# AlgoLab/PIntron

Measured on AMD Instinct MI355X. Metric: ESTs aligned/sec (whole node) + DP Mcells/s; bit-exact factorizations vs ref, higher is better.
Workload: dtype u8/int32

## Files before the change

include/pintron_gpu.h:

```cpp
#ifndef PINTRON_GPU_H
#define PINTRON_GPU_H

#include <stddef.h>
#include <stdint.h>

#ifdef __cplusplus
extern "C" {
#endif

#define PGPU_OK       0
#define PGPU_EDEVICE (-5)
#define PGPU_ENOMEM  (-12)
#define PGPU_EINVAL  (-22)
#define PGPU_ENOSPC  (-28)
#define PGPU_ERANGE  (-34)
#define PGPU_ENOSYS  (-38)

typedef struct pgpu_ctx pgpu_ctx;
typedef struct pgpu_index pgpu_index;
typedef struct pgpu_dp_plan pgpu_dp_plan;

int pgpu_init(int device, pgpu_ctx** ctx);
int pgpu_destroy(pgpu_ctx* ctx);
const char* pgpu_last_error(const pgpu_ctx* ctx);
// ... 19 lines not shown

int pgpu_index_find(pgpu_ctx* ctx, const pgpu_index* idx,
                    const char* patterns, size_t patterns_len,
                    const pgpu_find_query* queries, size_t n_queries,
                    uint32_t* out, size_t out_cap, uint64_t* out_first, size_t* n_out);
double pgpu_index_find_kernel_ms(int k);

typedef struct { uint32_t start, end; } pgpu_intron;

int pgpu_index_classify(pgpu_ctx* ctx, const pgpu_index* idx, const pgpu_intron* introns, size_t n,
                        uint8_t* out_type);
int pgpu_index_score5(pgpu_ctx* ctx, const pgpu_index* idx, int k, double* out, size_t cap);

#define PGPU_SEXON_MAX_ELEN 64
typedef struct {
  uint64_t e_off;
  uint32_t elen;
  uint32_t allgstart, allglen;
  uint32_t f1slen, f2plen;
  uint32_t min_intron_len;
  uint32_t reserved;
} pgpu_sexon_query;
typedef struct {
  int32_t  status;
  uint32_t len;
  uint32_t offstart, offend;
  uint32_t gpos;
  uint32_t i1type, i2type;
  uint32_t pad;
} pgpu_sexon_result;

int pgpu_index_small_exons(pgpu_ctx* ctx, const pgpu_index* idx, const char* ests, size_t ests_len,
                           const pgpu_sexon_query* q, size_t n, pgpu_sexon_result* out);
double pgpu_index_small_exons_kernel_ms(void);

typedef struct { int32_t EST_start, EST_end, GEN_start, GEN_end; } pgpu_factor;

#define PGPU_REFINE_MAX_DIM 1024
#define PGPU_REFINE_MAX_ED   256
#define PGPU_REFINE_FIRST_INTRON 1u

typedef struct {
  uint64_t est_off;  uint32_t est_len;
  uint32_t flags;
  uint64_t rows_off; uint32_t dim;
  int32_t  factor_cut, intron_start, intron_end, intron_start_on_align, intron_end_on_align;
  pgpu_factor donor, acceptor;
  int32_t  suffpref_length_on_est, suffpref_length_for_intron, suffpref_length_on_gen, min_intron_length;
} pgpu_refine_query;

typedef struct {
  int32_t status;
  int32_t refined;
  int32_t path;
  int32_t pad;
  pgpu_factor donor, acceptor;
} pgpu_refine_result;

int pgpu_index_refine_introns(pgpu_ctx* ctx, const pgpu_index* idx, const char* ests, size_t ests_len,
                              const char* rows, size_t rows_len,
                              const pgpu_refine_query* q, size_t n, pgpu_refine_result* out);
double pgpu_index_refine_introns_kernel_ms(void);

#define PGPU_CHAIN_MAX_EST_WINDOW 192
#define PGPU_CHAIN_MAX_GEN_WINDOW 320
typedef struct {
  uint64_t est_off; uint32_t est_len;
  uint32_t first_exon, n_exons;
  uint32_t reserved;
  int32_t  suffpref_length_on_est, suffpref_length_for_intron, suffpref_length_on_gen, min_intron_length;
} pgpu_chain_query;

typedef struct {
  int32_t  status;
  uint32_t done;
  uint32_t dropped_first;
  uint32_t pad;
} pgpu_chain_result;

int pgpu_index_refine_chains(pgpu_ctx* ctx, const pgpu_index* idx, const char* ests, size_t ests_len,
                             const pgpu_factor* exons, size_t n_exons_total,
                             const pgpu_chain_query* q, size_t n,
                             pgpu_factor* out_exons, uint8_t* out_steps, pgpu_chain_result* out);
double pgpu_index_refine_chains_kernel_ms(void);

typedef struct {
  uint32_t min_factor_len;
  uint32_t reserved;
  double   min_string_depth_rate;
} pgpu_pairing_params;

typedef struct { int32_t p, t, l; } pgpu_pairing;

int pgpu_pairings(pgpu_ctx* ctx, const pgpu_index* idx,
                  const char* patterns, const uint64_t* pat_off, size_t n_pat,
                  const pgpu_pairing_params* params,
                  pgpu_pairing* out, size_t out_cap, uint64_t* out_first, size_t* n_out);

typedef struct pgpu_pairing_plan pgpu_pairing_plan;
int pgpu_pairing_plan_create(pgpu_ctx* ctx, const pgpu_index* idx, const char* patterns,
                             const uint64_t* pat_off, size_t n_pat, pgpu_pairing_plan** plan);
int pgpu_pairing_plan_create_resident(pgpu_ctx* ctx, const pgpu_index* idx, const char* patterns,
                                      const uint64_t* pat_off, size_t n_pat, pgpu_pairing_plan** plan);
int pgpu_pairing_plan_run(pgpu_ctx* ctx, pgpu_pairing_plan* plan, const pgpu_pairing_params* params);
uint64_t pgpu_pairing_plan_count(const pgpu_pairing_plan* plan);
uint64_t pgpu_pairing_plan_positions(const pgpu_pairing_plan* plan);
double pgpu_pairing_plan_kernel_ms(const pgpu_pairing_plan* plan, int k);
int pgpu_pairing_plan_fetch(pgpu_ctx* ctx, pgpu_pairing_plan* plan, pgpu_pairing* out, size_t out_cap,
                            uint64_t* out_first);
int pgpu_pairing_plan_destroy(pgpu_ctx* ctx, pgpu_pairing_plan* plan);

typedef struct {
  uint32_t min_factor_len;
  int32_t  min_intron_length, max_intron_length;
  uint32_t max_pairings_in_MEG;
  double   max_prefix_discarded_rate, max_suffix_discarded_rate, max_freq_shortest_pairing;
  uint32_t trans_red, short_edge_comp;
} pgpu_meg_params;

#define PGPU_MEG_MAX_VERTICES 64
#define PGPU_MEG_MAX_DEGREE   32
#define PGPU_MEG_TOO_COMPLEX  1u
#define PGPU_MEG_UNAVAILABLE  2u
int pgpu_pairing_plan_run_meg(pgpu_ctx* ctx, pgpu_pairing_plan* plan, const pgpu_meg_params* params);
uint64_t pgpu_pairing_plan_meg_bytes(const pgpu_pairing_plan* plan);
int pgpu_pairing_plan_fetch_meg(pgpu_ctx* ctx, pgpu_pairing_plan* plan, void* out, size_t out_cap,
                                uint64_t* rec_first);
double pgpu_pairing_plan_meg_ms(const pgpu_pairing_plan* plan);

int pgpu_host_alloc(pgpu_ctx* ctx, size_t bytes, void** out);
int pgpu_host_free(pgpu_ctx* ctx, void* p);

typedef struct pgpu_comm pgpu_comm;
typedef struct { char bytes[128]; } pgpu_comm_id;
int pgpu_comm_unique_id(pgpu_ctx* ctx, pgpu_comm_id* id);
int pgpu_comm_init(pgpu_ctx* ctx, int rank, int world, const pgpu_comm_id* id, pgpu_comm** comm);
int pgpu_gather(pgpu_ctx* ctx, pgpu_comm* comm, const void* send, uint64_t send_bytes,
                void* recv, uint64_t recv_cap, uint64_t* counts);
int pgpu_allgather(pgpu_ctx* ctx, pgpu_comm* comm, const void* send, uint64_t bytes, void* recv);
int pgpu_comm_destroy(pgpu_ctx* ctx, pgpu_comm* comm);

enum pgpu_dp_kind {
  PGPU_DP_ALIGN = 0,
  PGPU_DP_GAP = 1,
  PGPU_DP_ED = 2,
  PGPU_DP_KBAND = 3,
  PGPU_DP_LCF = 4,
  PGPU_DP_BORDERS = 5,
  PGPU_DP_AFFIX = 6,
  PGPU_DP_NKINDS = 7
};

#define PGPU_JOB_A_GENOMIC 1u
#define PGPU_JOB_B_GENOMIC 2u

typedef struct {
  uint32_t kind;
  uint32_t flags;
  uint64_t a_off, b_off;
  uint32_t a_len, b_len;
  uint32_t p0, p1, p2;
  uint32_t tail;
} pgpu_dp_job;

typedef struct {
  int32_t status;
  int32_t v[6];
  int32_t pad;
  uint64_t str[2];
} pgpu_dp_result;

#define PGPU_MAX_ROWS_LEV     65536u
#define PGPU_MAX_ROWS_BORDERS 4096u
#define PGPU_MAX_ROWS_GAP     2048u
#define PGPU_MAX_GAP_SIDE    16000u
#define PGPU_MAX_GAP_CELLS (1ull << 27)
#define PGPU_MAX_COLS      1048576u

int pgpu_dp_plan_create(pgpu_ctx* ctx, const pgpu_index* idx,
                        const pgpu_dp_job* jobs, size_t n_jobs,
                        const char* arena, size_t arena_len, pgpu_dp_plan** plan);
typedef struct { const pgpu_dp_job* jobs; size_t n_jobs; const char* arena; size_t arena_len; } pgpu_dp_part;
int pgpu_dp_plan_create_parts(pgpu_ctx* ctx, const pgpu_index* idx, const pgpu_dp_part* parts, size_t n_parts,
                              pgpu_dp_plan** plan);
int pgpu_dp_plan_launch(pgpu_ctx* ctx, pgpu_dp_plan* plan);
int pgpu_dp_plan_sync(pgpu_ctx* ctx, pgpu_dp_plan* plan);
size_t pgpu_dp_plan_string_bytes(const pgpu_dp_plan* plan);
int pgpu_dp_plan_fetch(pgpu_ctx* ctx, pgpu_dp_plan* plan, pgpu_dp_result* results,
                       char* strings, size_t strings_cap);
int pgpu_dp_plan_results_to_device(pgpu_ctx* ctx, pgpu_dp_plan* plan, void* device_dst, size_t cap);
int pgpu_dp_plan_destroy(pgpu_ctx* ctx, pgpu_dp_plan* plan);

uint64_t pgpu_dp_plan_cells(const pgpu_dp_plan* plan, int kind);
uint64_t pgpu_dp_plan_algo_bytes(const pgpu_dp_plan* plan, int kind);
double   pgpu_dp_plan_kernel_ms(const pgpu_dp_plan* plan, int kind);
uint64_t pgpu_dp_plan_launches(const pgpu_dp_plan* plan, int kind);

typedef struct {
  char     name[48];
  int32_t  kind;
  int32_t  pad;
  uint64_t jobs, cells, algo_bytes;
  double   ms;
  double   t0_ms;
} pgpu_group_info;
int pgpu_dp_plan_n_groups(const pgpu_dp_plan* plan);
int pgpu_dp_plan_group_info(const pgpu_dp_plan* plan, int i, pgpu_group_info* out);

int pgpu_dp_batch(pgpu_ctx* ctx, const pgpu_index* idx,
                  const pgpu_dp_job* jobs, size_t n_jobs, const char* arena, size_t arena_len,
                  pgpu_dp_result* results, char* strings, size_t strings_cap,
                  size_t* strings_used);

#ifdef __cplusplus
}
#endif
#endif
```

pintron_amd/capi.py:

```python
import ctypes as C
import os

_HERE = os.path.dirname(os.path.abspath(__file__))
LIB_PATH = os.path.join(_HERE, "lib", "libpintron_gpu.so")

PGPU_OK, PGPU_EDEVICE, PGPU_ENOMEM, PGPU_EINVAL, PGPU_ENOSPC, PGPU_ERANGE, PGPU_ENOSYS = \
    0, -5, -12, -22, -28, -34, -38
ALIGN, GAP, ED, KBAND, LCF, BORDERS, AFFIX = range(7)
KIND_NAMES = ["ALIGN", "GAP", "ED", "KBAND", "LCF", "BORDERS", "AFFIX"]
JOB_A_GENOMIC, JOB_B_GENOMIC = 1, 2


class DpJob(C.Structure):
    _fields_ = [("kind", C.c_uint32), ("flags", C.c_uint32), ("a_off", C.c_uint64),
                ("b_off", C.c_uint64), ("a_len", C.c_uint32), ("b_len", C.c_uint32),
                ("p0", C.c_uint32), ("p1", C.c_uint32), ("p2", C.c_uint32), ("tail", C.c_uint32)]


class DpResult(C.Structure):
    _fields_ = [("status", C.c_int32), ("v", C.c_int32 * 6), ("pad", C.c_int32),
                ("str", C.c_uint64 * 2)]


class GroupInfo(C.Structure):
# ... 12 lines not shown


class FindQuery(C.Structure):
    _fields_ = [("pat_off", C.c_uint64), ("pat_len", C.c_uint32), ("reserved", C.c_uint32),
                ("lo", C.c_uint32), ("hi", C.c_uint32)]


class Intron(C.Structure):
    _fields_ = [("start", C.c_uint32), ("end", C.c_uint32)]


class SexonQuery(C.Structure):
    _fields_ = [("e_off", C.c_uint64), ("elen", C.c_uint32), ("allgstart", C.c_uint32), ("allglen", C.c_uint32),
                ("f1slen", C.c_uint32), ("f2plen", C.c_uint32), ("min_intron_len", C.c_uint32), ("reserved", C.c_uint32)]


class SexonResult(C.Structure):
    _fields_ = [("status", C.c_int32), ("len", C.c_uint32), ("offstart", C.c_uint32), ("offend", C.c_uint32),
                ("gpos", C.c_uint32), ("i1type", C.c_uint32), ("i2type", C.c_uint32), ("pad", C.c_uint32)]


class Factor(C.Structure):
    _fields_ = [("EST_start", C.c_int32), ("EST_end", C.c_int32), ("GEN_start", C.c_int32), ("GEN_end", C.c_int32)]


class RefineQuery(C.Structure):
    _fields_ = [("est_off", C.c_uint64), ("est_len", C.c_uint32), ("flags", C.c_uint32), ("rows_off", C.c_uint64),
                ("dim", C.c_uint32), ("factor_cut", C.c_int32), ("intron_start", C.c_int32), ("intron_end", C.c_int32),
                ("intron_start_on_align", C.c_int32), ("intron_end_on_align", C.c_int32), ("donor", Factor), ("acceptor", Factor),
                ("suffpref_length_on_est", C.c_int32), ("suffpref_length_for_intron", C.c_int32),
                ("suffpref_length_on_gen", C.c_int32), ("min_intron_length", C.c_int32)]


class RefineResult(C.Structure):
    _fields_ = [("status", C.c_int32), ("refined", C.c_int32), ("path", C.c_int32), ("pad", C.c_int32),
                ("donor", Factor), ("acceptor", Factor)]


class ChainQuery(C.Structure):
    _fields_ = [("est_off", C.c_uint64), ("est_len", C.c_uint32), ("first_exon", C.c_uint32), ("n_exons", C.c_uint32),
                ("reserved", C.c_uint32), ("suffpref_length_on_est", C.c_int32), ("suffpref_length_for_intron", C.c_int32),
                ("suffpref_length_on_gen", C.c_int32), ("min_intron_length", C.c_int32)]


class ChainResult(C.Structure):
    _fields_ = [("status", C.c_int32), ("done", C.c_uint32), ("dropped_first", C.c_uint32), ("pad", C.c_uint32)]


REFINE_MAX_DIM, REFINE_MAX_ED, REFINE_FIRST_INTRON = 1024, 256, 1
CHAIN_MAX_EST_WINDOW, CHAIN_MAX_GEN_WINDOW = 192, 320
_FACTOR_DTYPE = [("EST_start", "<i4"), ("EST_end", "<i4"), ("GEN_start", "<i4"), ("GEN_end", "<i4")]
REFINE_QUERY_DTYPE = [("est_off", "<u8"), ("est_len", "<u4"), ("flags", "<u4"), ("rows_off", "<u8"), ("dim", "<u4"),
                      ("factor_cut", "<i4"), ("intron_start", "<i4"), ("intron_end", "<i4"), ("intron_start_on_align", "<i4"),
                      ("intron_end_on_align", "<i4"), ("donor", _FACTOR_DTYPE), ("acceptor", _FACTOR_DTYPE),
                      ("suffpref_length_on_est", "<i4"), ("suffpref_length_for_intron", "<i4"), ("suffpref_length_on_gen", "<i4"),
                      ("min_intron_length", "<i4")]
REFINE_RESULT_DTYPE = [("status", "<i4"), ("refined", "<i4"), ("path", "<i4"), ("pad", "<i4"), ("donor", _FACTOR_DTYPE),
                       ("acceptor", _FACTOR_DTYPE)]

CHAIN_QUERY_DTYPE = [("est_off", "<u8"), ("est_len", "<u4"), ("first_exon", "<u4"), ("n_exons", "<u4"), ("reserved", "<u4"),
                     ("suffpref_length_on_est", "<i4"), ("suffpref_length_for_intron", "<i4"), ("suffpref_length_on_gen", "<i4"),
                     ("min_intron_length", "<i4")]
CHAIN_RESULT_DTYPE = [("status", "<i4"), ("done", "<u4"), ("dropped_first", "<u4"), ("pad", "<u4")]
FACTOR_DTYPE = _FACTOR_DTYPE

SEXON_MAX_ELEN = 64
SEXON_QUERY_DTYPE = [("e_off", "<u8"), ("elen", "<u4"), ("allgstart", "<u4"), ("allglen", "<u4"), ("f1slen", "<u4"),
                     ("f2plen", "<u4"), ("min_intron_len", "<u4"), ("reserved", "<u4"), ("_pad", "<u4")]
SEXON_RESULT_DTYPE = [("status", "<i4"), ("len", "<u4"), ("offstart", "<u4"), ("offend", "<u4"), ("gpos", "<u4"),
                      ("i1type", "<u4"), ("i2type", "<u4"), ("pad", "<u4")]

assert C.sizeof(DpJob) == 48 and C.sizeof(DpResult) == 48 and C.sizeof(FindQuery) == 24
assert C.sizeof(Intron) == 8 and C.sizeof(SexonQuery) == 40 and C.sizeof(SexonResult) == 32
assert C.sizeof(Factor) == 16 and C.sizeof(RefineQuery) == 96 and C.sizeof(RefineResult) == 48
assert C.sizeof(ChainQuery) == 40 and C.sizeof(ChainResult) == 16

EXPORTS = [
    "pgpu_init", "pgpu_destroy", "pgpu_last_error", "pgpu_abi_version", "pgpu_set_timing", "pgpu_device_numa_node",
    "pgpu_index_build", "pgpu_index_destroy", "pgpu_index_suffix_array", "pgpu_index_save", "pgpu_index_load", "pgpu_pairings",
    "pgpu_index_find", "pgpu_index_find_kernel_ms",
    "pgpu_index_classify", "pgpu_index_score5", "pgpu_index_small_exons", "pgpu_index_small_exons_kernel_ms",
    "pgpu_index_refine_introns", "pgpu_index_refine_introns_kernel_ms",
    "pgpu_index_refine_chains", "pgpu_index_refine_chains_kernel_ms",
    "pgpu_pairing_plan_create", "pgpu_pairing_plan_create_resident", "pgpu_pairing_plan_run", "pgpu_pairing_plan_count",
    "pgpu_pairing_plan_positions", "pgpu_pairing_plan_kernel_ms", "pgpu_pairing_plan_fetch",
    "pgpu_pairing_plan_destroy",
    "pgpu_pairing_plan_run_meg", "pgpu_pairing_plan_meg_bytes", "pgpu_pairing_plan_fetch_meg",
    "pgpu_pairing_plan_meg_ms", "pgpu_host_alloc", "pgpu_host_free",
    "pgpu_comm_unique_id", "pgpu_comm_init", "pgpu_gather", "pgpu_allgather", "pgpu_comm_destroy",
    "pgpu_range_push", "pgpu_range_pop", "pgpu_build_info",
    "pgpu_dp_plan_create", "pgpu_dp_plan_create_parts", "pgpu_dp_plan_launch", "pgpu_dp_plan_sync",
    "pgpu_dp_plan_string_bytes", "pgpu_dp_plan_fetch", "pgpu_dp_plan_destroy",
    "pgpu_dp_plan_results_to_device",
    "pgpu_dp_plan_cells", "pgpu_dp_plan_algo_bytes", "pgpu_dp_plan_kernel_ms",
    "pgpu_dp_plan_launches", "pgpu_dp_plan_n_groups", "pgpu_dp_plan_group_info", "pgpu_dp_batch",
]

_lib = None


class PgpuError(RuntimeError):
    def __init__(self, code, msg):
        super().__init__("pgpu error %d: %s" % (code, msg))
        self.code = code


def lib():
    global _lib
    if _lib is None:
        if not os.path.exists(LIB_PATH):
            raise ImportError("%s is missing: run `python -c 'import __graft_entry__ as g; "
                              "g.build()'` (hipcc --offload-arch=gfx950)" % LIB_PATH)
        L = C.CDLL(LIB_PATH)
        vp, u64, sz = C.c_void_p, C.c_uint64, C.c_size_t
        L.pgpu_init.argtypes = [C.c_int, C.POINTER(vp)]
        L.pgpu_destroy.argtypes = [vp]
        L.pgpu_set_timing.argtypes = [vp, C.c_int]
        L.pgpu_last_error.argtypes = [vp]
        L.pgpu_last_error.restype = C.c_char_p
        L.pgpu_build_info.restype = C.c_char_p
        L.pgpu_range_push.argtypes = [C.c_char_p]
        L.pgpu_range_push.restype = None
        L.pgpu_range_pop.restype = None
        L.pgpu_allgather.argtypes = [vp, vp, vp, u64, vp]
        L.pgpu_index_build.argtypes = [vp, C.c_char_p, sz, C.POINTER(vp)]
        L.pgpu_index_destroy.argtypes = [vp, vp]
        L.pgpu_index_save.argtypes = [vp, vp, C.c_char_p, C.c_char_p]
        L.pgpu_index_load.argtypes = [vp, C.c_char_p, C.c_char_p, sz, C.POINTER(vp)]
        L.pgpu_index_suffix_array.argtypes = [vp, vp, C.POINTER(C.c_uint32), sz]
        L.pgpu_index_find.argtypes = [vp, vp, C.c_char_p, sz, C.POINTER(FindQuery), sz,
                                      C.POINTER(C.c_uint32), sz, C.POINTER(u64), C.POINTER(sz)]
        L.pgpu_index_find_kernel_ms.argtypes = [C.c_int]
        L.pgpu_index_find_kernel_ms.restype = C.c_double
        L.pgpu_index_classify.argtypes = [vp, vp, C.POINTER(Intron), sz, C.POINTER(C.c_uint8)]
        L.pgpu_index_score5.argtypes = [vp, vp, C.c_int, C.POINTER(C.c_double), sz]
        L.pgpu_index_small_exons.argtypes = [vp, vp, C.c_char_p, sz, C.POINTER(SexonQuery), sz, C.POINTER(SexonResult)]
        L.pgpu_index_small_exons_kernel_ms.argtypes = []
        L.pgpu_index_small_exons_kernel_ms.restype = C.c_double
        L.pgpu_index_refine_introns.argtypes = [vp, vp, C.c_char_p, sz, C.c_char_p, sz, C.POINTER(RefineQuery), sz,
                                                C.POINTER(RefineResult)]
        L.pgpu_index_refine_introns_kernel_ms.argtypes = []
        L.pgpu_index_refine_introns_kernel_ms.restype = C.c_double
        L.pgpu_index_refine_chains.argtypes = [vp, vp, C.c_char_p, sz, C.POINTER(Factor), sz, C.POINTER(ChainQuery), sz,
                                               C.POINTER(Factor), C.POINTER(C.c_uint8), C.POINTER(ChainResult)]
        L.pgpu_index_refine_chains_kernel_ms.argtypes = []
        L.pgpu_index_refine_chains_kernel_ms.restype = C.c_double
        L.pgpu_pairing_plan_run_meg.argtypes = [vp, vp, vp]
        L.pgpu_pairing_plan_meg_bytes.argtypes = [vp]
        L.pgpu_pairing_plan_meg_bytes.restype = u64
        L.pgpu_pairing_plan_meg_ms.argtypes = [vp]
        L.pgpu_pairing_plan_meg_ms.restype = C.c_double
        L.pgpu_pairing_plan_fetch_meg.argtypes = [vp, vp, vp, sz, C.POINTER(u64)]
        L.pgpu_host_alloc.argtypes = [vp, sz, C.POINTER(vp)]
        L.pgpu_host_free.argtypes = [vp, vp]
        L.pgpu_comm_unique_id.argtypes = [vp, vp]
        L.pgpu_comm_init.argtypes = [vp, C.c_int, C.c_int, vp, C.POINTER(vp)]
        L.pgpu_gather.argtypes = [vp, vp, C.c_char_p, u64, vp, u64, C.POINTER(u64)]
        L.pgpu_comm_destroy.argtypes = [vp, vp]
        L.pgpu_pairings.argtypes = [vp, vp, C.c_char_p, C.POINTER(u64), sz,
                                    C.POINTER(PairingParams), C.POINTER(Pairing), sz,
                                    C.POINTER(u64), C.POINTER(sz)]
        L.pgpu_pairing_plan_create.argtypes = [vp, vp, C.c_char_p, C.POINTER(u64), sz, C.POINTER(vp)]
        L.pgpu_pairing_plan_create_resident.argtypes = [vp, vp, C.c_char_p, C.POINTER(u64), sz, C.POINTER(vp)]
        L.pgpu_pairing_plan_run.argtypes = [vp, vp, C.POINTER(PairingParams)]
        L.pgpu_pairing_plan_count.argtypes = [vp]
        L.pgpu_pairing_plan_count.restype = u64
        L.pgpu_pairing_plan_positions.argtypes = [vp]
        L.pgpu_pairing_plan_positions.restype = u64
        L.pgpu_pairing_plan_kernel_ms.argtypes = [vp, C.c_int]
        L.pgpu_pairing_plan_kernel_ms.restype = C.c_double
        L.pgpu_pairing_plan_fetch.argtypes = [vp, vp, C.POINTER(Pairing), sz, C.POINTER(u64)]
        L.pgpu_pairing_plan_destroy.argtypes = [vp, vp]
        L.pgpu_dp_plan_create_parts.argtypes = [vp, vp, vp, sz, C.POINTER(vp)]
        L.pgpu_dp_plan_create.argtypes = [vp, vp, C.POINTER(DpJob), sz, C.c_char_p, sz,
                                          C.POINTER(vp)]
        L.pgpu_dp_plan_launch.argtypes = [vp, vp]
        L.pgpu_dp_plan_sync.argtypes = [vp, vp]
        L.pgpu_dp_plan_string_bytes.argtypes = [vp]
        L.pgpu_dp_plan_string_bytes.restype = sz
        L.pgpu_dp_plan_fetch.argtypes = [vp, vp, C.POINTER(DpResult), C.c_char_p, sz]
        L.pgpu_dp_plan_destroy.argtypes = [vp, vp]
        L.pgpu_dp_plan_results_to_device.argtypes = [vp, vp, vp, sz]
        for nm in ("pgpu_dp_plan_cells", "pgpu_dp_plan_algo_bytes", "pgpu_dp_plan_launches"):
            getattr(L, nm).argtypes = [vp, C.c_int]
            getattr(L, nm).restype = u64
        L.pgpu_dp_plan_kernel_ms.argtypes = [vp, C.c_int]
        L.pgpu_dp_plan_kernel_ms.restype = C.c_double
        L.pgpu_dp_plan_n_groups.argtypes = [vp]
        L.pgpu_dp_plan_group_info.argtypes = [vp, C.c_int, C.POINTER(GroupInfo)]
        L.pgpu_dp_batch.argtypes = [vp, vp, C.POINTER(DpJob), sz, C.c_char_p, sz,
                                    C.POINTER(DpResult), C.c_char_p, sz, C.POINTER(sz)]
        _lib = L
    return _lib


class Context:

    def __init__(self, device=0):
        self.L = lib()
        self.h = C.c_void_p()
        rc = self.L.pgpu_init(device, C.byref(self.h))
        if rc != PGPU_OK:
            raise PgpuError(rc, "pgpu_init(%d) failed (no usable gfx950 device?)" % device)
        self.L.pgpu_set_timing(self.h, 1)

    def check(self, rc):
        if rc != PGPU_OK:
            raise PgpuError(rc, self.L.pgpu_last_error(self.h).decode())

    def close(self):
        if self.h:
            self.L.pgpu_destroy(self.h)
            self.h = C.c_void_p()

    def __enter__(self):
        return self

    def __exit__(self, *a):
        self.close()


class Index:
    def __init__(self, ctx: Context, genomic: bytes, load_from=None):
        self.ctx = ctx
        self.h = C.c_void_p()
        self.n = len(genomic)
        self.genomic = genomic
# ... 46 lines not shown
        if rc == PGPU_ENOSPC:
            out = np.empty(total, dtype=np.uint32)
            rc, first, total = self.find_raw(blob, qs, n, out)
        else:
            out = np.empty(0, dtype=np.uint32)
        self.ctx.check(rc)
        return [out[int(first[i]):int(first[i + 1])] for i in range(n)]

    def find_kernel_ms(self):
        return {"count+scan": self.ctx.L.pgpu_index_find_kernel_ms(0), "fill": self.ctx.L.pgpu_index_find_kernel_ms(1)}

    def classify(self, starts, ends, ctx=None):
        import numpy as np
        ctx = ctx or self.ctx
        iv = np.empty((len(starts), 2), dtype=np.uint32)
        iv[:, 0], iv[:, 1] = starts, ends
        out = np.empty(len(iv), dtype=np.uint8)
        ctx.check(ctx.L.pgpu_index_classify(ctx.h, self.h, iv.ctypes.data_as(C.POINTER(Intron)), len(iv),
                                            out.ctypes.data_as(C.POINTER(C.c_uint8))))
        return out

    def score5(self, k):
        import numpy as np
        out = np.empty(self.n + 1, dtype=np.float64)
        self.ctx.check(self.ctx.L.pgpu_index_score5(self.ctx.h, self.h, k, out.ctypes.data_as(C.POINTER(C.c_double)), len(out)))
        return out

    def small_exons_raw(self, ests: bytes, queries, n: int):
        import numpy as np
        res = np.zeros(n, dtype=np.dtype(SEXON_RESULT_DTYPE))
        qp = queries.ctypes.data_as(C.POINTER(SexonQuery)) if hasattr(queries, "ctypes") else queries
        rc = self.ctx.L.pgpu_index_small_exons(self.ctx.h, self.h, ests, len(ests), qp, n,
                                               res.ctypes.data_as(C.POINTER(SexonResult)))
        return rc, res

    def small_exons(self, ests: bytes, queries):
        import numpy as np
        if not isinstance(queries, np.ndarray):
            rows = list(queries)
            q = np.zeros(len(rows), dtype=np.dtype(SEXON_QUERY_DTYPE))
            for i, r in enumerate(rows):
                q[i] = tuple(r) + (0, 0)
            queries = q
        rc, res = self.small_exons_raw(ests, queries, len(queries))
        self.ctx.check(rc)
        return res

    def small_exons_kernel_ms(self):
        return self.ctx.L.pgpu_index_small_exons_kernel_ms()

    def refine_introns_raw(self, ests: bytes, rows: bytes, queries, n: int):
        import numpy as np
        res = np.zeros(n, dtype=np.dtype(REFINE_RESULT_DTYPE))
        qp = queries.ctypes.data_as(C.POINTER(RefineQuery)) if hasattr(queries, "ctypes") else queries
        rc = self.ctx.L.pgpu_index_refine_introns(self.ctx.h, self.h, ests, len(ests), rows, len(rows), qp, n,
                                                  res.ctypes.data_as(C.POINTER(RefineResult)))
        return rc, res

    def refine_introns(self, ests: bytes, rows: bytes, queries):
        rc, res = self.refine_introns_raw(ests, rows, queries, len(queries))
        self.ctx.check(rc)
        return res

    def refine_introns_kernel_ms(self):
        return self.ctx.L.pgpu_index_refine_introns_kernel_ms()

    def refine_chains_raw(self, ests: bytes, exons, queries, n: int):
        import numpy as np
        out_exons = np.zeros(len(exons), dtype=np.dtype(FACTOR_DTYPE))
        out_steps = np.zeros(len(exons), dtype=np.uint8)
        res = np.zeros(n, dtype=np.dtype(CHAIN_RESULT_DTYPE))
        rc = self.ctx.L.pgpu_index_refine_chains(self.ctx.h, self.h, ests, len(ests), exons.ctypes.data_as(C.POINTER(Factor)),
                                                 len(exons), queries.ctypes.data_as(C.POINTER(ChainQuery)), n,
                                                 out_exons.ctypes.data_as(C.POINTER(Factor)),
                                                 out_steps.ctypes.data_as(C.POINTER(C.c_uint8)),
                                                 res.ctypes.data_as(C.POINTER(ChainResult)))
        return rc, out_exons, out_steps, res

    def refine_chains(self, ests: bytes, exons, queries):
        rc, out_exons, out_steps, res = self.refine_chains_raw(ests, exons, queries, len(queries))
        self.ctx.check(rc)
        return out_exons, out_steps, res

    def refine_chains_kernel_ms(self):
        return self.ctx.L.pgpu_index_refine_chains_kernel_ms()

    def close(self):
        if self.h:
            self.ctx.L.pgpu_index_destroy(self.ctx.h, self.h)
            self.h = C.c_void_p()


class MegParams(C.Structure):
    _fields_ = [("min_factor_len", C.c_uint32), ("min_intron_length", C.c_int32), ("max_intron_length", C.c_int32),
                ("max_pairings_in_MEG", C.c_uint32), ("max_prefix_discarded_rate", C.c_double),
                ("max_suffix_discarded_rate", C.c_double), ("max_freq_shortest_pairing", C.c_double),
                ("trans_red", C.c_uint32), ("short_edge_comp", C.c_uint32)]


def parse_meg_record(rec: bytes):
    import struct
    nv, ne, flags, _ = struct.unpack_from("<4I", rec, 0)
    if flags & 2:
        return dict(flags=flags, vertices=[], adj=[], meg_text=b"", edges_text=b"")
    verts = [struct.unpack_from("<3i", rec, 16 + 12 * k) for k in range(nv)]
    first = struct.unpack_from("<%dH" % (nv + 1), rec, 16 + 12 * nv)
    base = 16 + 12 * nv + 2 * (nv + 1)
    adj = [list(rec[base + first[k]:base + first[k + 1]]) for k in range(nv)]
    graph = (base + ne + 3) & ~3
    ml, el = struct.unpack_from("<2I", rec, graph)
    return dict(flags=flags, vertices=verts, adj=adj, meg_text=rec[graph + 8:graph + 8 + ml],
                edges_text=rec[graph + 8 + ml:graph + 8 + ml + el])


class PairingPlan:
    STAGES = ["locate", "chain", "count+scan", "fill", "cross+scan", "emit"]

    def __init__(self, ctx: Context, index: Index, patterns, resident=False):
        import numpy as np
        self.ctx, self.n_pat = ctx, len(patterns)
        self._blob = b"".join(patterns)
        self._off = np.zeros(len(patterns) + 1, dtype=np.uint64)
        np.cumsum([len(p) for p in patterns], out=self._off[1:])
        self.h = C.c_void_p()
        create = ctx.L.pgpu_pairing_plan_create_resident if resident else ctx.L.pgpu_pairing_plan_create
        ctx.check(create(ctx.h, index.h, self._blob, self._off.ctypes.data_as(C.POINTER(C.c_uint64)),
                         self.n_pat, C.byref(self.h)))

    def run(self, min_factor_len=15, rate=0.2):
        prm = PairingParams(min_factor_len, 0, rate)
        self.ctx.check(self.ctx.L.pgpu_pairing_plan_run(self.ctx.h, self.h, C.byref(prm)))
        return self.ctx.L.pgpu_pairing_plan_count(self.h)

    def stage_ms(self):
        return {s: self.ctx.L.pgpu_pairing_plan_kernel_ms(self.h, k) for k, s in enumerate(self.STAGES)}

    def fetch(self):
        import numpy as np
        n = self.ctx.L.pgpu_pairing_plan_count(self.h)
        out = np.zeros((max(n, 1), 3), dtype=np.int32)
        first = np.zeros(self.n_pat + 1, dtype=np.uint64)
        self.ctx.check(self.ctx.L.pgpu_pairing_plan_fetch(
            self.ctx.h, self.h, out.ctypes.data_as(C.POINTER(Pairing)), n,
            first.ctypes.data_as(C.POINTER(C.c_uint64))))
        return out[:n], first

    def run_meg(self, min_factor_len=15, min_intron_length=40, max_intron_length=0, max_pairings_in_MEG=80,
                max_prefix_discarded_rate=0.6, max_suffix_discarded_rate=0.6, max_freq_shortest_pairing=0.4,
                trans_red=True, short_edge_comp=True):
        prm = MegParams(min_factor_len, min_intron_length, max_intron_length, max_pairings_in_MEG,
                        max_prefix_discarded_rate, max_suffix_discarded_rate, max_freq_shortest_pairing,
                        int(trans_red), int(short_edge_comp))
        self.ctx.check(self.ctx.L.pgpu_pairing_plan_run_meg(self.ctx.h, self.h, C.byref(prm)))
        return self.ctx.L.pgpu_pairing_plan_meg_bytes(self.h)

    def fetch_meg(self):
        import numpy as np
        n = self.ctx.L.pgpu_pairing_plan_meg_bytes(self.h)
        out = np.zeros(max(n, 1), dtype=np.uint8)
        first = np.zeros(self.n_pat + 1, dtype=np.uint64)
        self.ctx.check(self.ctx.L.pgpu_pairing_plan_fetch_meg(
            self.ctx.h, self.h, out.ctypes.data_as(C.c_void_p), n, first.ctypes.data_as(C.POINTER(C.c_uint64))))
        raw = out.tobytes()
        return [raw[int(first[i]):int(first[i + 1])] for i in range(self.n_pat)]

    def close(self):
# ... 139 lines not shown
```

pintron_amd/csrc/pgpu_api.hip:

```cpp
#include <algorithm>
#include <cstdarg>
#include <cstdio>
#include <cstdlib>
#include <cstring>
#include <ctime>
#include <time.h>
#include <new>
#include <mutex>
#include <vector>

#include "pgpu_internal.h"
#include "pgpu_index.h"

struct BufPool {
  static constexpr int SLOTS = 24;
  void* ptr[SLOTS] = {nullptr};
  size_t cap[SLOTS] = {0};
  bool busy = false;
  int sharers = 0;
  const void* owner = nullptr;
};

struct pgpu_ctx {
  int device = 0;
  hipStream_t stream = nullptr;
  char err[512] = {0};
  BufPool pools[2];
  bool timing = false;
  static constexpr int NAUX = 4;
  hipStream_t aux[NAUX] = {nullptr};
  hipEvent_t ev_upload = nullptr;
  hipEvent_t ev_aux[NAUX] = {nullptr};
  hipEvent_t ev_done = nullptr;
  hipEvent_t ev_wait = nullptr;
  long wait_poll_us = 20;
  int poison = -1;
  void* pin[2] = {nullptr, nullptr};
  size_t pin_cap[2] = {0, 0};
  std::vector<hipEvent_t> ev_pool;
};

static int wait_stream(pgpu_ctx* ctx, hipStream_t st) {
  if (hipEventRecord(ctx->ev_done, st) != hipSuccess) return -1;
  if (ctx->wait_poll_us != 0) {
    for (;;) {
      const hipError_t q = hipEventQuery(ctx->ev_done);
      if (q == hipSuccess) return 0;
      if (q != hipErrorNotReady) return -1;
      if (ctx->wait_poll_us > 0) { struct timespec ts = {0, ctx->wait_poll_us * 1000L}; nanosleep(&ts, nullptr); }
    }
  }
  return hipEventSynchronize(ctx->ev_done) == hipSuccess ? 0 : -1;
}

static void* pinned(pgpu_ctx* ctx, int slot, size_t bytes) {
  if (ctx->pin_cap[slot] < bytes) {
    if (ctx->pin[slot]) (void)hipHostFree(ctx->pin[slot]);
    ctx->pin[slot] = nullptr; ctx->pin_cap[slot] = 0;
    const size_t want = std::max<size_t>(bytes + bytes / 2 + 4096, (size_t)2 << 20);
    if (hipHostMalloc(&ctx->pin[slot], want, hipHostMallocDefault) != hipSuccess) return nullptr;
    pgpu_trace_alloc(slot ? "ctx pinned down" : "ctx pinned up", ctx->pin[slot], want);
    ctx->pin_cap[slot] = want;
  }
  return ctx->pin[slot];
}

bool pgpu_ctx_pool_acquire(pgpu_ctx* ctx, int pool) {
  if (ctx->pools[pool].busy) return false;
  ctx->pools[pool].busy = true;
  return true;
}
void pgpu_ctx_pool_release(pgpu_ctx* ctx, int pool) { ctx->pools[pool].busy = false; ctx->pools[pool].owner = nullptr; }
bool pgpu_ctx_pool_share(pgpu_ctx* ctx, int pool) {
  BufPool& p = ctx->pools[pool];
  if (p.busy && p.sharers == 0) return false;
  p.busy = true; ++p.sharers;
  return true;
}
void pgpu_ctx_pool_unshare(pgpu_ctx* ctx, int pool, const void* who) {
  BufPool& p = ctx->pools[pool];
  if (p.owner == who) p.owner = nullptr;
  if (p.sharers > 0 && --p.sharers == 0) p.busy = false;
}
void pgpu_ctx_pool_set_owner(pgpu_ctx* ctx, int pool, const void* who) { ctx->pools[pool].owner = who; }
const void* pgpu_ctx_pool_owner(const pgpu_ctx* ctx, int pool) { return ctx->pools[pool].owner; }
void* pgpu_ctx_pool_get(pgpu_ctx* ctx, int pool, int slot, size_t bytes) {
  BufPool& p = ctx->pools[pool];
  if (bytes == 0) bytes = 16;
  if (p.cap[slot] < bytes) {
    if (p.ptr[slot]) (void)hipFree(p.ptr[slot]);
    p.ptr[slot] = nullptr; p.cap[slot] = 0;
    const size_t want = std::max<size_t>(bytes + bytes / 2 + 4096, pool == 0 ? (size_t)64 << 20 : 0);
    if (hipMalloc(&p.ptr[slot], want) != hipSuccess) {
      if (hipMalloc(&p.ptr[slot], bytes) != hipSuccess) return nullptr;
      p.cap[slot] = bytes;
    } else p.cap[slot] = want;
    pgpu_trace_alloc(pool ? "device pool 1" : "device pool 0", p.ptr[slot], p.cap[slot]);
  }
  return p.ptr[slot];
}
bool pgpu_ctx_timing(const pgpu_ctx* ctx) { return ctx->timing; }

extern "C" int pgpu_device_numa_node(pgpu_ctx* ctx) {
  if (!ctx) return -1;
  char bdf[64] = {0};
  if (hipDeviceGetPCIBusId(bdf, (int)sizeof bdf - 1, ctx->device) != hipSuccess) return -1;
  for (char* c = bdf; *c; ++c) if (*c >= 'A' && *c <= 'F') *c = (char)(*c - 'A' + 'a');
  char path[160];
  snprintf(path, sizeof path, "/sys/bus/pci/devices/%s/numa_node", bdf);
  FILE* f = fopen(path, "r");
  if (!f) return -1;
  int node = -1;
  if (fscanf(f, "%d", &node) != 1) node = -1;
  fclose(f);
  return node;
}

extern "C" int pgpu_set_timing(pgpu_ctx* ctx, int enabled) {
  if (!ctx) return PGPU_EINVAL;
  ctx->timing = enabled != 0;
  return PGPU_OK;
}

static int set_err(pgpu_ctx* ctx, int code, const char* fmt, ...) {
  if (ctx) {
    va_list ap;
    va_start(ap, fmt);
    vsnprintf(ctx->err, sizeof(ctx->err), fmt, ap);
    va_end(ap);
  }
  return code;
}

#define HIP_TRY(ctx, call)                                                                  \
  do {                                                                                      \
    hipError_t e_ = (call);                                                                 \
    if (e_ != hipSuccess)                                                                   \
      return set_err(ctx, e_ == hipErrorOutOfMemory ? PGPU_ENOMEM : PGPU_EDEVICE,           \
                     "%s failed: %s (%s:%d)", #call, hipGetErrorString(e_), __FILE__, __LINE__); \
  } while (0)

hipStream_t pgpu_ctx_stream(pgpu_ctx* ctx) { return ctx->stream; }
hipError_t pgpu_ctx_wait(pgpu_ctx* ctx) {
  if (ctx->wait_poll_us <= 0) return hipStreamSynchronize(ctx->stream);
  hipError_t e = hipEventRecord(ctx->ev_wait, ctx->stream);
  if (e != hipSuccess) return e;
  const struct timespec ts = {0, ctx->wait_poll_us * 5000L};
  for (;;) {
    e = hipEventQuery(ctx->ev_wait);
    if (e != hipErrorNotReady) return e;
    nanosleep(&ts, nullptr);
  }
}
int pgpu_ctx_bind(pgpu_ctx* ctx) {
  const hipError_t e = hipSetDevice(ctx->device);
  return e == hipSuccess ? PGPU_OK : set_err(ctx, PGPU_EDEVICE, "hipSetDevice(%d) failed: %s", ctx->device, hipGetErrorString(e));
}
int pgpu_ctx_fail(pgpu_ctx* ctx, int code, const char* msg) { return set_err(ctx, code, "%s", msg); }

extern "C" int pgpu_abi_version(void) { return 1; }

#include <dlfcn.h>
namespace {
struct Roctx { int state = 0; int (*push)(const char*) = nullptr; int (*pop)() = nullptr; };
Roctx g_roctx;
bool roctx_ready() {
  if (g_roctx.state) return g_roctx.state > 0;
  bool want = false;
  { const char* m = getenv("PGPU_MARKERS"); if (m) want = m[0] != '0'; else {
      const char* t = getenv("ROCP_TOOL_LIBRARIES"); const char* pl = getenv("LD_PRELOAD");
      want = (t && t[0]) || (pl && strstr(pl, "rocprofiler")); } }
  if (want) {
    void* so = nullptr;
    for (const char* n : { "librocprofiler-sdk-roctx.so.1", "librocprofiler-sdk-roctx.so", "libroctx64.so.4", "libroctx64.so" })
      if ((so = dlopen(n, RTLD_NOW | RTLD_GLOBAL)) != nullptr) break;
    if (so) {
      *(void**)(&g_roctx.push) = dlsym(so, "roctxRangePushA");
      *(void**)(&g_roctx.pop) = dlsym(so, "roctxRangePop");
    }
  }
  g_roctx.state = (g_roctx.push && g_roctx.pop) ? 1 : -1;
  return g_roctx.state > 0;
}
}
extern "C" void pgpu_range_push(const char* name) { if (roctx_ready()) g_roctx.push(name ? name : ""); }
extern "C" void pgpu_range_pop(void) { if (roctx_ready()) g_roctx.pop(); }

extern "C" const char* pgpu_build_info(void) {
  static char info[256];
  if (!info[0]) {
    const char* stamp = __DATE__ " " __TIME__ " " __VERSION__;
    unsigned long long h = 1469598103934665603ull;
    for (const char* c = stamp; *c; ++c) { h ^= (unsigned char)*c; h *= 1099511628211ull; }
    snprintf(info, sizeof info, "libpintron_gpu abi %d, gfx950, built %s %s, hip %d.%d.%d, stamp %016llx", pgpu_abi_version(), __DATE__,
             __TIME__, HIP_VERSION_MAJOR, HIP_VERSION_MINOR, HIP_VERSION_PATCH, h);
  }
  return info;
}

static bool aux_stream(pgpu_ctx* ctx, int i) {
  if (!ctx->aux[i] && hipStreamCreateWithFlags(&ctx->aux[i], hipStreamNonBlocking) != hipSuccess) { ctx->aux[i] = nullptr; return false; }
  if (!ctx->ev_aux[i] && hipEventCreateWithFlags(&ctx->ev_aux[i], hipEventDisableTiming) != hipSuccess) { ctx->ev_aux[i] = nullptr; return false; }
  return true;
}

static hipEvent_t g_base_event[64];
static std::mutex g_base_mu;
static hipEvent_t base_event(int device, hipStream_t st) {
  if (device < 0 || device >= 64) return nullptr;
  std::lock_guard<std::mutex> lk(g_base_mu);
  if (!g_base_event[device]) {
    hipEvent_t e = nullptr;
    if (hipEventCreate(&e) == hipSuccess && hipEventRecord(e, st) == hipSuccess && hipEventSynchronize(e) == hipSuccess) g_base_event[device] = e;
    else if (e) hipEventDestroy(e);
  }
  return g_base_event[device];
}

extern "C" int pgpu_init(int device, pgpu_ctx** out) {
  if (!out) return PGPU_EINVAL;
  *out = nullptr;
  int n = 0;
  if (hipGetDeviceCount(&n) != hipSuccess || n <= 0) return PGPU_EDEVICE;
  if (device < 0 || device >= n) return PGPU_EINVAL;
  hipDeviceProp_t prop;
  if (hipGetDeviceProperties(&prop, device) != hipSuccess) return PGPU_EDEVICE;
  if (strncmp(prop.gcnArchName, "gfx950", 6) != 0) return PGPU_EDEVICE;
  if (hipSetDevice(device) != hipSuccess) return PGPU_EDEVICE;
  pgpu_ctx* ctx = new (std::nothrow) pgpu_ctx();
  if (!ctx) return PGPU_ENOMEM;
  ctx->device = device;
  if (hipStreamCreateWithFlags(&ctx->stream, hipStreamNonBlocking) != hipSuccess) {
    delete ctx;
    return PGPU_EDEVICE;
  }
  if (hipEventCreateWithFlags(&ctx->ev_upload, hipEventDisableTiming) != hipSuccess) { delete ctx; return PGPU_EDEVICE; }
  if (hipEventCreateWithFlags(&ctx->ev_done, hipEventDisableTiming | hipEventBlockingSync) != hipSuccess) { delete ctx; return PGPU_EDEVICE; }
  if (hipEventCreateWithFlags(&ctx->ev_wait, hipEventDisableTiming) != hipSuccess) { delete ctx; return PGPU_EDEVICE; }
  { const char* f = getenv("PGPU_WAIT"); if (f) ctx->wait_poll_us = atol(f); }
  { const char* f = getenv("PGPU_POISON"); if (f && f[0]) ctx->poison = atoi(f) & 255; }
  base_event(device, ctx->stream);
  *out = ctx;
  return PGPU_OK;
}

extern "C" int pgpu_destroy(pgpu_ctx* ctx) {
  if (!ctx) return PGPU_EINVAL;
  hipSetDevice(ctx->device);
  hipStreamSynchronize(ctx->stream);
  for (auto& pl : ctx->pools) for (auto& q : pl.ptr) if (q) hipFree(q);
  for (auto& a : ctx->aux) if (a) { hipStreamSynchronize(a); hipStreamDestroy(a); }
  if (ctx->ev_upload) hipEventDestroy(ctx->ev_upload);
  if (ctx->ev_done) hipEventDestroy(ctx->ev_done);
  if (ctx->ev_wait) hipEventDestroy(ctx->ev_wait);
  for (auto& e : ctx->ev_aux) if (e) hipEventDestroy(e);
  for (auto& e : ctx->ev_pool) if (e) hipEventDestroy(e);
  for (auto& q : ctx->pin) if (q) hipHostFree(q);
  hipStreamDestroy(ctx->stream);
  delete ctx;
  return PGPU_OK;
}

extern "C" const char* pgpu_last_error(const pgpu_ctx* ctx) { return ctx ? ctx->err : "null context"; }

namespace {

uint32_t row_class(uint32_t rows) {
  if (rows > 4096u) return ROW_CLASS_STRIPS;
  uint32_t R = 1;
  while (64u * R < rows) R <<= 1;
  return R;
}

enum DpRoute : uint8_t {
  RT_ALIGN_STRIPS, RT_ALIGN_COOP, RT_ALIGN_WAVE, RT_GAP_SLOW, RT_GAP, RT_ED, RT_KBAND, RT_LCF,
  RT_BORDERS_SLOW, RT_BORDERS_COOP, RT_BORDERS_WAVE, RT_AFFIX_STRIPS, RT_AFFIX_COOP, RT_AFFIX_WAVE,
  RT_LCFSA, RT_LCFW, RT_ALIGNB,
  RT_BATCH,
  RT_COUNT
};

enum BatchPlace { OUTSIDE, SEGMENT, ROLE_BORDERS, ROLE_AFFIX, ROLE_ALIGN };

using WsBytes = size_t (*)(uint32_t la, uint32_t lb, uint32_t R);
size_t ws_align_wave(uint32_t, uint32_t lb, uint32_t) { return ((size_t)lb + 64) * 64; }
size_t ws_align_coop(uint32_t, uint32_t lb, uint32_t R) { return ((size_t)lb + 256) * 256 * align_coop_entry_bytes(R); }
size_t ws_align_strips(uint32_t la, uint32_t lb, uint32_t R) {
  return 2 * strip_bnd_bytes(lb) + (size_t)((la + 4095u) / 4096u) * ((size_t)lb + 64) * 64 * align_entry_bytes(R);
}
size_t ws_gap(uint32_t, uint32_t lb, uint32_t R) { return ((size_t)lb + 64) * 64 * gap_entry_bytes(R); }
size_t ws_gap_slow(uint32_t la, uint32_t lb, uint32_t) { return (size_t)9 * ((size_t)la + 1) * 4 + ((size_t)la + 1) * ((size_t)lb + 1); }
size_t ws_borders_slow(uint32_t la, uint32_t, uint32_t) { return (size_t)7 * ((size_t)la + 1) * 4; }
size_t ws_affix_strips(uint32_t, uint32_t lb, uint32_t) { return 2 * strip_bnd_bytes(lb); }
size_t ws_ed_strips(uint32_t la, uint32_t lb, uint32_t R) { return R == ROW_CLASS_STRIPS ? 2 * strip_bnd_bytes(std::max(la, lb)) : 0; }

using AlgoBytes = uint64_t (*)(uint64_t la, uint64_t lb, uint64_t p2);
uint64_t bytes_operands(uint64_t la, uint64_t lb, uint64_t) { return la + lb; }
uint64_t bytes_align(uint64_t la, uint64_t lb, uint64_t) { return la + lb + la * lb + 3 * (la + lb); }
uint64_t bytes_gap(uint64_t la, uint64_t lb, uint64_t) { return la + lb + 3 * la * lb + 3 * (la + lb); }
uint64_t bytes_borders(uint64_t la, uint64_t lb, uint64_t p2) { return la + std::min(lb, 2 * std::min(la + p2, lb)) + 2 * 8 * la; }
uint64_t bytes_lcfsa(uint64_t, uint64_t lb, uint64_t) { return lb + 64u * 96u; }

struct RouteInfo {
  const char* name;
  int kind;
  int family;
  WsBytes ws_bytes;
  bool strings;
  uint32_t cell_factor;
  AlgoBytes algo_bytes;
  BatchPlace place;
  int seg_pos;
  uint32_t big_from;
  long weight; bool by_rows; int lane; DpLauncher launch;
  bool keyed;
};

constexpr RouteInfo ROUTES[] = {
  {"lev_wave<ALIGN,strips>",  PGPU_DP_ALIGN,   KF_ALIGN,   ws_align_strips, true,  1, bytes_align,    OUTSIDE,      0,  0,  5000, false,  2, launch_align_big,    false},
  {"align_coop",              PGPU_DP_ALIGN,   KF_ALIGN,   ws_align_coop,   true,  1, bytes_align,    ROLE_ALIGN,   0,  0,     0, false,  0, nullptr,             false},
  {"lev_wave<ALIGN>",         PGPU_DP_ALIGN,   KF_ALIGN,   ws_align_wave,   true,  1, bytes_align,    SEGMENT,      1,  0,     0, false,  0, nullptr,             false},
  {"gap_slow",                PGPU_DP_GAP,     KF_GAP,     ws_gap_slow,     true,  3, bytes_gap,      OUTSIDE,      0,  0,  4000, false,  3, launch_gap_slow,     false},
  {"gap_wave",                PGPU_DP_GAP,     KF_GAP,     ws_gap,          true,  3, bytes_gap,      SEGMENT,      2,  8,  4000, false,  3, launch_gap_big,      false},
  {"lev_wave<ED>",            PGPU_DP_ED,      KF_ED,      ws_ed_strips,    false, 1, bytes_operands, SEGMENT,      8, 32,  1000, false,  1, launch_ed_big,       false},
  {"lev_wave<KBAND>",         PGPU_DP_KBAND,   KF_KBAND,   ws_ed_strips,    false, 1, bytes_operands, SEGMENT,      3, 32,  2000, false,  2, launch_kband_big,    false},
  {"lcf",                     PGPU_DP_LCF,     KF_LCF,     nullptr,         false, 1, bytes_operands, OUTSIDE,      0,  0,  3000, false,  3, launch_lcf,          true},
  {"borders_slow",            PGPU_DP_BORDERS, KF_BORDERS, ws_borders_slow, false, 2, bytes_borders,  OUTSIDE,      0,  0, 10000, true,   1, launch_borders_slow, false},
  {"borders_coop",            PGPU_DP_BORDERS, KF_BORDERS, nullptr,         false, 2, bytes_borders,  ROLE_BORDERS, 0,  0, 10000, true,   1, launch_borders_coop, false},
  {"lev_wave<BORDERS,R=1>",   PGPU_DP_BORDERS, KF_BORDERS, nullptr,         false, 2, bytes_borders,  SEGMENT,      4,  0,     0, false,  0, nullptr,             false},
  {"lev_wave<AFFIX,strips>",  PGPU_DP_AFFIX,   KF_AFFIX,   ws_affix_strips, false, 1, bytes_operands, OUTSIDE,      0,  0, 10000, true,   0, launch_affix_strips, false},
  {"affix_coop",              PGPU_DP_AFFIX,   KF_AFFIX,   nullptr,         false, 1, bytes_operands, ROLE_AFFIX,   0,  0,     0, false,  0, nullptr,             false},
  {"lev_wave<AFFIX,R=1>",     PGPU_DP_AFFIX,   KF_AFFIX,   nullptr,         false, 1, bytes_operands, SEGMENT,      5,  0,     0, false,  0, nullptr,             false},
// ... 539 lines not shown
```

pintron_amd/csrc/pgpu_chain.hip:

```cpp
#include <stdlib.h>
#include <string.h>

#include "pgpu_internal.h"
#include "pgpu_query_call.h"
#include "pgpu_wave_dp.h"
#include "pgpu_refine_body.h"

namespace {

constexpr int MAX_EW = PGPU_CHAIN_MAX_EST_WINDOW;
constexpr int MAX_GW = PGPU_CHAIN_MAX_GEN_WINDOW;
constexpr uint32_t CHAIN_R = 4;
static_assert(MAX_EW <= 64 * (int)CHAIN_R && MAX_EW + MAX_GW <= MAX_DIM, "the caps fit the sweep and the decision");

constexpr size_t WS_DIRS = ((size_t)MAX_GW + 64) * 64 * CHAIN_R;
constexpr size_t WS_STRS = WS_DIRS;
constexpr size_t WS_STRS_BYTES = (2 * ((size_t)MAX_EW + MAX_GW + 1) + 15) & ~(size_t)15;
constexpr size_t WS_WIN_E = WS_STRS + WS_STRS_BYTES;
constexpr size_t WS_WIN_G = WS_WIN_E + ((MAX_EW + 15) & ~15);
constexpr size_t WS_RES = WS_WIN_G + ((MAX_GW + 15) & ~15);
constexpr size_t WS_WAVE = (WS_RES + sizeof(DevResult) + 255) & ~(size_t)255;

struct ChainLds {
  union {
    struct { __attribute__((aligned(16))) uint8_t win[TB_WIN_BYTES]; uint8_t path[TB_PATH]; } tb;
    RefineLds refine;
  };
};

__device__ __forceinline__ int append_piece(uint8_t* dst, int at, int cap, const Seq& s, int index, int length, int lane) {
  if (at > cap) return at;
  if (index < 0) { length += index; index = 0; }
  if (length > cap - at + 1) length = cap - at + 1;
  const Piece p = substring(s, index, length, lane);
  if (p.len > cap - at) return cap + 1;
  for (int k = lane; k < p.len; k += 64) dst[at + k] = s.p[p.start + k];
  return at + p.len;
}

__global__ __launch_bounds__(64)
void chain_kernel(const uint8_t* __restrict__ T, uint32_t n, const uint8_t* __restrict__ ests, const pgpu_factor* __restrict__ exons,
                  const pgpu_chain_query* __restrict__ queries, uint32_t n_chains, uint8_t* __restrict__ ws,
                  pgpu_factor* __restrict__ out_exons, uint8_t* __restrict__ out_steps, pgpu_chain_result* __restrict__ out) {
  __shared__ ChainLds S;
  const int lane = (int)threadIdx.x;
  uint8_t* const w = ws + (size_t)blockIdx.x * WS_WAVE;
  uint8_t* const win_e = w + WS_WIN_E;
  uint8_t* const win_g = w + WS_WIN_G;
  DevResult* const res = reinterpret_cast<DevResult*>(w + WS_RES);
  for (uint32_t c = blockIdx.x; c < n_chains; c += gridDim.x) {
    const pgpu_chain_query q = queries[c];
    Seq est, gen;
    est.p = ests + q.est_off; est.len = (int)q.est_len;
    gen.p = T; gen.len = (int)n;
    const int sp_est = q.suffpref_length_on_est, sp_int = q.suffpref_length_for_intron, sp_gen = q.suffpref_length_on_gen;
    pgpu_chain_result cr;
    cr.status = PGPU_OK; cr.done = 0; cr.dropped_first = 0; cr.pad = 0;
    pgpu_factor donor = exons[q.first_exon];
    const int first_est_start = donor.EST_start;
    int second_est_start = 0;
    uint32_t i = 0;
    for (; i + 1 < q.n_exons; ++i) {
      const pgpu_factor acceptor = exons[q.first_exon + i + 1];
      int dsl_gen = donor.GEN_start;
      if (donor.GEN_end - sp_gen + 1 >= dsl_gen) dsl_gen = donor.GEN_end - sp_gen + 1;
      int dsl_est = donor.EST_start;
      if (donor.EST_end - sp_est + 1 >= dsl_est) dsl_est = donor.EST_end - sp_est + 1;
      int apr_gen = acceptor.GEN_end;
      if (acceptor.GEN_start + sp_gen - 1 <= apr_gen) apr_gen = acceptor.GEN_start + sp_gen - 1;
      int apr_est = acceptor.EST_end;
      if (acceptor.EST_start + sp_est - 1 <= apr_est) apr_est = acceptor.EST_start + sp_est - 1;
      int le = 0, lg = 0;
      le = append_piece(win_e, le, MAX_EW, est, dsl_est, donor.EST_end - dsl_est + 1, lane);
      if (donor.EST_end != acceptor.EST_start - 1)
        le = append_piece(win_e, le, MAX_EW, est, donor.EST_end + 1, acceptor.EST_start - donor.EST_end - 1, lane);
      le = append_piece(win_e, le, MAX_EW, est, acceptor.EST_start, apr_est - acceptor.EST_start + 1, lane);
      lg = append_piece(win_g, lg, MAX_GW, gen, dsl_gen, donor.GEN_end - dsl_gen + 1, lane);
      lg = append_piece(win_g, lg, MAX_GW, gen, donor.GEN_end + 1, sp_int, lane);
      lg = append_piece(win_g, lg, MAX_GW, gen, acceptor.GEN_start - sp_int, sp_int, lane);
      lg = append_piece(win_g, lg, MAX_GW, gen, acceptor.GEN_start, apr_gen - acceptor.GEN_start + 1, lane);
      if (le > MAX_EW || lg > MAX_GW) { cr.status = PGPU_ERANGE; break; }
      DevJob job;
      job.a = win_e; job.b = win_g; job.la = (uint32_t)le; job.lb = (uint32_t)lg;
      job.p0 = job.p1 = job.p2 = job.tail = 0;
      job.ws_off = 0; job.str_off = WS_STRS; job.out_idx = 0;
      job.r_class = le <= 64 ? 1u : (le <= 128 ? 2u : 4u);
      own_stores_visible();
      switch (job.r_class) {
        case 1:  gap_wave_body<1>(job, res, w, (uint32_t)lane); break;
        case 2:  gap_wave_body<2>(job, res, w, (uint32_t)lane); break;
        default: gap_wave_body<4>(job, res, w, (uint32_t)lane); break;
      }
      own_stores_visible();
      gap_traceback_wave(job, res, w, w, (uint32_t)lane, S.tb.win, S.tb.path);
      own_stores_visible();
      pgpu_refine_query rq;
      rq.est_off = q.est_off; rq.est_len = q.est_len; rq.flags = i == 0 ? PGPU_REFINE_FIRST_INTRON : 0u;
      rq.rows_off = 0; rq.dim = (uint32_t)__builtin_amdgcn_readfirstlane(res->v[0]);
      rq.factor_cut = __builtin_amdgcn_readfirstlane(res->v[1]);
      rq.intron_start = __builtin_amdgcn_readfirstlane(res->v[2]);
      rq.intron_end = __builtin_amdgcn_readfirstlane(res->v[3]);
      rq.intron_start_on_align = __builtin_amdgcn_readfirstlane(res->v[4]);
      rq.intron_end_on_align = __builtin_amdgcn_readfirstlane(res->v[5]);
      rq.donor = donor; rq.acceptor = acceptor;
      rq.suffpref_length_on_est = sp_est; rq.suffpref_length_for_intron = sp_int; rq.suffpref_length_on_gen = sp_gen;
      rq.min_intron_length = q.min_intron_length;
      const int dim = (int)rq.dim;
      const uint8_t* const row_e = w + (uint32_t)__builtin_amdgcn_readfirstlane((int)res->str[0]);
      const uint8_t* const row_g = w + (uint32_t)__builtin_amdgcn_readfirstlane((int)res->str[1]);
      __syncthreads();
      for (int k = lane; k < dim; k += 64) { S.refine.rows[k] = row_e[k]; S.refine.rows[dim + k] = row_g[k]; }
      __syncthreads();
      pgpu_refine_result r;
      r.status = PGPU_OK; r.refined = 0; r.path = 0; r.pad = 0; r.donor = donor; r.acceptor = acceptor;
      refine_decide(S.refine, S.refine.rows, S.refine.rows + dim, dim, rq, T, n, ests, lane, r);
      __syncthreads();
      if (r.status != PGPU_OK) { cr.status = PGPU_ERANGE; break; }
      if (lane == 0) {
        out_exons[q.first_exon + i] = r.donor;
        out_steps[q.first_exon + i + 1] = (uint8_t)((uint32_t)r.path | ((uint32_t)r.refined << 7));
      }
      if (i == 0) second_est_start = r.acceptor.EST_start;
      donor = r.acceptor;
    }
    cr.done = i;
    if (lane == 0) out_exons[q.first_exon + i] = donor;
    if (cr.status == PGPU_OK && q.n_exons > 1 && first_est_start == second_est_start) cr.dropped_first = 1;
    if (lane == 0) out[c] = cr;
  }
}

thread_local double t_chain_ms = 0.0;

constexpr unsigned WAVES_PER_CU = 16;

}

extern "C" double pgpu_index_refine_chains_kernel_ms(void) { return t_chain_ms; }

extern "C" int pgpu_index_refine_chains(pgpu_ctx* ctx, const pgpu_index* idx, const char* ests, size_t ests_len,
                                        const pgpu_factor* exons, size_t n_exons_total,
                                        const pgpu_chain_query* q, size_t n,
                                        pgpu_factor* out_exons, uint8_t* out_steps, pgpu_chain_result* out) {
  t_chain_ms = 0.0;
  static_assert(sizeof(pgpu_chain_query) == 40 && sizeof(pgpu_chain_result) == 16 && sizeof(pgpu_factor) == 16, "ABI layout");
  if (!ctx || !idx || (n && (!q || !out)) || (ests_len && !ests) || (n_exons_total && (!exons || !out_exons || !out_steps)))
    return PGPU_EINVAL;
  if (n > 0x7fffffffull || n_exons_total > 0x7fffffffull)
    return pgpu_ctx_fail(ctx, PGPU_EINVAL, "more than 2^31 - 1 chains or exons in one call");
  const size_t glen = pgpu_index_length(idx);
  struct Freed { uint8_t* p; ~Freed() { free(p); } } named_block{ (uint8_t*)calloc(n_exons_total ? n_exons_total : 1, 1) };
  uint8_t* const named = named_block.p;
  if (!named) return pgpu_ctx_fail(ctx, PGPU_ENOMEM, "no memory for the table of the exons the chains name");
  for (size_t i = 0; i < n; ++i) {
    const pgpu_chain_query& x = q[i];
    bool ok = x.est_off <= ests_len && x.est_len <= ests_len - x.est_off && x.est_len <= 0x7fffffffu && x.reserved == 0 &&
              x.n_exons != 0 && x.first_exon <= n_exons_total && x.n_exons <= n_exons_total - x.first_exon &&
              suffpref_ok(x.suffpref_length_on_est, x.suffpref_length_for_intron, x.suffpref_length_on_gen);
    for (uint32_t k = 0; ok && k < x.n_exons; ++k) {
      const pgpu_factor& f = exons[x.first_exon + k];
      ok = !named[x.first_exon + k] && factor_ok(f, x.est_len, glen);
      named[x.first_exon + k] = 1;
      if (ok && k + 1 < x.n_exons) {
        const pgpu_factor& g = exons[x.first_exon + k + 1];
        ok = f.EST_end < g.EST_start && f.GEN_end < g.GEN_start;
      }
    }
    if (!ok)
      return pgpu_ctx_fail(ctx, PGPU_EINVAL, "bad chain query (a range past its buffer, reserved != 0, no exon, an exon two chains "
                                             "share, a donor that is not in front of its acceptor, or a coordinate outside what it "
                                             "indexes)");
  }
  if (n == 0) {
    if (n_exons_total) { memcpy(out_exons, exons, n_exons_total * sizeof(pgpu_factor)); memset(out_steps, 0, n_exons_total); }
    return PGPU_OK;
  }
  if (pgpu_ctx_bind(ctx) != PGPU_OK) return PGPU_EDEVICE;
  QueryCall call(ctx, "refine chains");
  const hipStream_t st = call.st;
  int dev = 0, cus = 0;
  TRY_HIP(hipGetDevice(&dev));
  TRY_HIP(hipDeviceGetAttribute(&cus, hipDeviceAttributeMultiprocessorCount, dev));
  const size_t waves = n < (size_t)cus * WAVES_PER_CU ? n : (size_t)cus * WAVES_PER_CU;
  const size_t ex_bytes = n_exons_total * sizeof(pgpu_factor);
  const size_t o_ex = up256(ests_len + 64), o_q = o_ex + up256(ex_bytes), o_oex = o_q + up256(n * sizeof(pgpu_chain_query)),
               o_st = o_oex + up256(ex_bytes), o_r = o_st + up256(n_exons_total), o_ws = o_r + up256(n * sizeof(pgpu_chain_result)),
               total = o_ws + waves * WS_WAVE;
  TRY_HIP(hipMalloc((void**)&call.d, total));
  TRY_HIP(call.timing_events(1));
  if (ests_len) TRY_HIP(hipMemcpyAsync(call.d, ests, ests_len, hipMemcpyHostToDevice, st));
  TRY_HIP(hipMemcpyAsync(call.d + o_ex, exons, ex_bytes, hipMemcpyHostToDevice, st));
  TRY_HIP(hipMemcpyAsync(call.d + o_q, q, n * sizeof(pgpu_chain_query), hipMemcpyHostToDevice, st));
  TRY_HIP(hipMemcpyAsync(call.d + o_oex, call.d + o_ex, ex_bytes, hipMemcpyDeviceToDevice, st));
  TRY_HIP(hipMemsetAsync(call.d + o_st, 0, n_exons_total, st));
  TRY_HIP(call.record(0));
  hipLaunchKernelGGL(chain_kernel, dim3((unsigned)waves), dim3(64), 0, st, pgpu_index_genomic(idx), (uint32_t)glen, call.d,
                     (const pgpu_factor*)(call.d + o_ex), (const pgpu_chain_query*)(call.d + o_q), (uint32_t)n, call.d + o_ws,
                     (pgpu_factor*)(call.d + o_oex), call.d + o_st, (pgpu_chain_result*)(call.d + o_r));
  TRY_HIP(call.record(1));
  TRY_HIP(hipMemcpyAsync(out_exons, call.d + o_oex, ex_bytes, hipMemcpyDeviceToHost, st));
  TRY_HIP(hipMemcpyAsync(out_steps, call.d + o_st, n_exons_total, hipMemcpyDeviceToHost, st));
  TRY_HIP(hipMemcpyAsync(out, call.d + o_r, n * sizeof(pgpu_chain_result), hipMemcpyDeviceToHost, st));
  TRY_HIP(pgpu_ctx_wait(ctx));
  TRY_HIP(hipGetLastError());
  call.elapsed_ms(0, &t_chain_ms);
  return PGPU_OK;
}
```

pintron_amd/csrc/pgpu_index.h:

```cpp
#pragma once
#include <stddef.h>
#include <stdint.h>
#include <mutex>
#include <hip/hip_runtime.h>
#include "../../include/pintron_gpu.h"

const uint8_t* pgpu_index_genomic(const pgpu_index* idx);
size_t pgpu_index_length(const pgpu_index* idx);

constexpr uint32_t KTAB = 8;
constexpr uint32_t KTAB_ENTRIES = 1u << (2 * KTAB);

struct LcfIndexView {
  const uint8_t* T; const uint32_t* sa; const uint32_t* klo; const uint32_t* khi; const uint32_t* focc; const uint32_t* rmq;
  uint32_t n, levels, first_bad;
};
LcfIndexView pgpu_index_lcf_view(const pgpu_index* idx);
constexpr uint32_t LCF_FOCC_ENTRIES = 87380;

struct pgpu_index_lazy { std::mutex mu; void* tables = nullptr; void (*release)(void*) = nullptr; };
pgpu_index_lazy* pgpu_index_lazy_slot(const pgpu_index* idx);

hipStream_t pgpu_ctx_stream(pgpu_ctx* ctx);
int pgpu_ctx_bind(pgpu_ctx* ctx);
hipError_t pgpu_ctx_wait(pgpu_ctx* ctx);
int pgpu_ctx_fail(pgpu_ctx* ctx, int code, const char* msg);
bool pgpu_ctx_pool_acquire(pgpu_ctx* ctx, int pool);
void pgpu_ctx_pool_release(pgpu_ctx* ctx, int pool);
void* pgpu_ctx_pool_get(pgpu_ctx* ctx, int pool, int slot, size_t bytes);
bool pgpu_ctx_pool_share(pgpu_ctx* ctx, int pool);
void pgpu_ctx_pool_unshare(pgpu_ctx* ctx, int pool, const void* who);
void pgpu_ctx_pool_set_owner(pgpu_ctx* ctx, int pool, const void* who);
const void* pgpu_ctx_pool_owner(const pgpu_ctx* ctx, int pool);
bool pgpu_ctx_timing(const pgpu_ctx* ctx);

size_t pgpu_scan_tmp_bytes(size_t n);
void pgpu_exclusive_scan_u32(const uint32_t* in, unsigned long long* out, size_t n, void* tmp, hipStream_t st);
size_t pgpu_meg_scratch_bytes(size_t n_pat);
void pgpu_meg_launch_build(const pgpu_pairing* pairs, const unsigned long long* pair_first, const unsigned long long* pat_off,
                           uint32_t n_pat, const pgpu_meg_params* prm, void* scratch, void* info, uint32_t* rec_bytes,
                           hipStream_t st);
void pgpu_meg_launch_emit(uint32_t n_pat, const void* scratch, const void* info, const unsigned long long* rec_off,
                          uint8_t* out, hipStream_t st);
#include <cstdio>
#include <cstdlib>
static inline void pgpu_trace_alloc(const char* what, const void* q, size_t bytes) {
  static int on = -1;
  if (on < 0) { const char* e = getenv("PGPU_TRACE_ALLOC"); on = (e && *e && *e != '0') ? 1 : 0; }
  if (on) fprintf(stderr, "* alloc %-18s %10.1f MB at %p\n", what, bytes / 1048576.0, q);
}
```

pintron_amd/host/ef_config.c:

```c
#include <stdlib.h>
#include <string.h>
#include <unistd.h>

#include "estfact.h"

void ef_config_defaults(ef_config* c) {
  memset(c, 0, sizeof(*c));
  c->min_factor_len = 15; c->min_intron_length = 40; c->max_intron_length = 0;
  c->min_string_depth_rate = 0.2;
  c->max_prefix_discarded_rate = 0.60; c->max_suffix_discarded_rate = 0.60;
  c->max_prefix_discarded = 50; c->max_suffix_discarded = 50;
  c->max_site_difference = 50; c->max_number_of_factorizations = 0;
  c->max_coverage_diff = 0.05; c->max_exonNUM_diff = 5; c->max_gapLength_diff = 20;
  c->retain_externals = 1;
  c->max_pairings_in_MEG = 80; c->max_freq_shortest_pairing = 0.4;
  c->suffpref_length_for_intron = 70; c->suffpref_length_on_est = 30; c->suffpref_length_on_gen = 30;
  c->trans_red = true; c->short_edge_comp = true;
  c->max_single_factorization_time = 900;
  c->complexity_threshold = 20.0;
  strcpy(c->config_file, "config.ini");
}

typedef enum { T_INT, T_DBL, T_STR, T_FLAG, T_BOOLSTR } otype;
typedef struct { const char* name; char shortopt; otype type; size_t off; } optdef;
// ... 29 lines not shown
    case 7: if (iv < 0) return -1; c->max_prefix_discarded = (int)iv; return 0;
    case 8: if (iv < 0) return -1; c->max_suffix_discarded = (int)iv; return 0;
    case 9: if (iv < 0) return -1; c->max_site_difference = (unsigned)iv; return 0;
    case 10: if (iv < 0) return -1; c->max_number_of_factorizations = (int)iv; return 0;
    case 11: if (dv < 0.0 || dv > 1.0) return -1; c->max_coverage_diff = dv; return 0;
    case 12: if (iv < -1) return -1; c->max_exonNUM_diff = (int)iv; return 0;
    case 13: if (iv < -1) return -1; c->max_gapLength_diff = (int)iv; return 0;
    case 14: if (dv <= 0.0) return -1; c->complexity_threshold = dv; return 0;
    case 15:
      if (v && !strcmp(v, "true")) c->retain_externals = 1;
      else if (v && !strcmp(v, "false")) c->retain_externals = 0;
      else return -1;
      return 0;
    case 16: if (iv < 0) return -1; c->max_pairings_in_MEG = (unsigned)iv; return 0;
    case 17: if (dv < 0.0 || dv > 1.0) return -1; c->max_freq_shortest_pairing = dv; return 0;
    case 18: if (iv <= 0) return -1; c->suffpref_length_for_intron = (int)iv; return 0;
    case 19: if (iv <= 0) return -1; c->suffpref_length_on_est = (int)iv; return 0;
    case 20: if (iv <= 0) return -1; c->suffpref_length_on_gen = (int)iv; return 0;
    case 21: c->trans_red = false; return 0;
    case 22: c->short_edge_comp = false; return 0;
    case 23: if (iv < 0) return -1; c->max_single_factorization_time = (unsigned)iv; return 0;
  }
  return -1;
}

static bool is_flag(int k) { return k == 21 || k == 22; }

static int find_long(const char* name, size_t len) {
  for (int k = 0; NAMES[k]; ++k)
    if (strlen(NAMES[k]) == len && !strncmp(NAMES[k], name, len)) return k;
  return -1;
}

static int parse_file(ef_config* c, const char* path, const bool* given) {
  FILE* f = fopen(path, "r");
  if (!f) return 0;
  char line[4096];
  while (fgets(line, sizeof line, f)) {
    char* p = line;
    while (*p == ' ' || *p == '\t') ++p;
    if (*p == '#' || *p == '\n' || *p == '\0') continue;
    char* e = p;
    while (*e && *e != '=' && *e != ' ' && *e != '\t' && *e != '\n') ++e;
    const int k = find_long(p, (size_t)(e - p));
    if (k < 0) { fprintf(stderr, "est-fact: unknown option '%.*s' in %s\n", (int)(e - p), p, path); fclose(f); return -1; }
    while (*e == ' ' || *e == '\t' || *e == '=') ++e;
    char* v = e;
    size_t vl = strlen(v);
    while (vl && (v[vl - 1] == '\n' || v[vl - 1] == '\r' || v[vl - 1] == ' ' || v[vl - 1] == '\t')) v[--vl] = '\0';
    if (vl >= 2 && v[0] == '"' && v[vl - 1] == '"') { v[vl - 1] = '\0'; ++v; }
    if (given[k]) continue;
    if (apply(c, k, is_flag(k) ? NULL : v) != 0) { fprintf(stderr, "est-fact: invalid value for '%s' in %s\n", NAMES[k], path); fclose(f); return -1; }
  }
  fclose(f);
  return 0;
}

static void dump(const ef_config* c) {
  FILE* f = fopen("./config-dump.ini", "w");
  if (!f) return;
  fprintf(f, "# This file was written by est-fact (MI355X build)\n");
  fprintf(f, "config-file=\"%s\"\n", c->config_file);
  fprintf(f, "min-factor-length=\"%u\"\nmin-intron-length=\"%d\"\nmax-intron-length=\"%d\"\n",
          c->min_factor_len, c->min_intron_length, c->max_intron_length);
  fprintf(f, "min-string-depth-rate=\"%g\"\nmax-prefix-discarded-rate=\"%g\"\nmax-suffix-discarded-rate=\"%g\"\n",
          c->min_string_depth_rate, c->max_prefix_discarded_rate, c->max_suffix_discarded_rate);
  fprintf(f, "max-prefix-discarded=\"%d\"\nmax-suffix-discarded=\"%d\"\nmin-distance-of-splice-sites=\"%u\"\n",
          c->max_prefix_discarded, c->max_suffix_discarded, c->max_site_difference);
  fprintf(f, "max-no-of-factorizations=\"%d\"\nmax-difference-of-coverage=\"%g\"\nmax-difference-of-no-of-exons=\"%d\"\n",
          c->max_number_of_factorizations, c->max_coverage_diff, c->max_exonNUM_diff);
  fprintf(f, "max-difference-of-gap-length=\"%d\"\ncomplexity-threshold=\"%g\"\nretain-externals=\"%s\"\n",
          c->max_gapLength_diff, c->complexity_threshold, c->retain_externals ? "true" : "false");
  fprintf(f, "max-pairings-in-CMEG=\"%u\"\nmax-shortest-pairing-frequence=\"%g\"\n",
          c->max_pairings_in_MEG, c->max_freq_shortest_pairing);
  fprintf(f, "suff-pref-length-intron=\"%d\"\nsuff-pref-length-est=\"%d\"\nsuff-pref-length-genomic=\"%d\"\n",
          c->suffpref_length_for_intron, c->suffpref_length_on_est, c->suffpref_length_on_gen);
  if (!c->trans_red) fprintf(f, "no-transitive-reduction\n");
  if (!c->short_edge_comp) fprintf(f, "no-short-edge-compaction\n");
  fprintf(f, "max-single-factorization-time=\"%u\"\n", c->max_single_factorization_time);
  fclose(f);
}

int ef_ahead_on = 1;
int ef_chain_fast_path = 1;
int ef_endpoint_checks = 1;
int ef_prof_on;
_Thread_local ef_prof_state ef_prof;
unsigned long long ef_work_budget_override;

int ef_config_load(ef_config* c, int argc, char** argv) {
  ef_config_defaults(c);
  { const char* e = getenv("PINTRON_ENDPOINT_CHECKS"); ef_endpoint_checks = !(e && e[0] == '0'); }
  { const char* e = getenv("PINTRON_CHAIN"); ef_chain_fast_path = !(e && e[0] == '0' && e[1] == '\0'); }
  { const char* e = getenv("PINTRON_AHEAD"); ef_ahead_on = !(e && e[0] == '0' && e[1] == '\0'); }
  { const char* e = getenv("PINTRON_PROFILE"); ef_prof_on = e && e[0] && !(e[0] == '0' && e[1] == '\0'); }
  { const char* e = getenv("PINTRON_WORK_BUDGET"); ef_work_budget_override = e && atoll(e) > 0 ? (unsigned long long)atoll(e) : 0ull; }
  bool given[32] = { false };
  for (int i = 1; i < argc; ++i) {
    const char* a = argv[i];
    int k = -1;
    const char* v = NULL;
    if (a[0] == '-' && a[1] == '-') {
      const char* eq = strchr(a + 2, '=');
      k = find_long(a + 2, eq ? (size_t)(eq - a - 2) : strlen(a + 2));
      if (eq) v = eq + 1;
    } else if (a[0] == '-' && a[1] && strchr("ClBdpsPSDE", a[1])) {
      for (int q = 0; NAMES[q]; ++q) if (SHORTS[q] == a[1]) k = q;
      if (a[2]) v = a + 2;
    }
    if (k < 0) { fprintf(stderr, "est-fact: unrecognized option '%s'\n", a); return -1; }
    if (!is_flag(k) && !v) {
      if (i + 1 >= argc) { fprintf(stderr, "est-fact: option '%s' requires an argument\n", a); return -1; }
      v = argv[++i];
    }
    if (apply(c, k, is_flag(k) ? NULL : v) != 0) { fprintf(stderr, "est-fact: invalid argument for option '%s'\n", NAMES[k]); return -1; }
    given[k] = true;
  }
  if (access(c->config_file, R_OK) == 0 && parse_file(c, c->config_file, given) != 0) return -1;
  dump(c);
  return 0;
}
```

pintron_amd/host/ef_fact.c:

```c
#include <math.h>
#include <stdlib.h>
#include <string.h>

#include "estfact.h"

typedef struct { int p, t, l; } ptl;

static size_t view_len(const char* s, int index, int length) {
  if (length <= 0) return 0;
  const char* z = (const char*)memchr(s + index, 0, (size_t)length);
  return z ? (size_t)(z - (s + index)) : (size_t)length;
}

char* ef_real_substring(int index, int length, const char* s) {
  if (index < 0) { length += index; index = 0; }
  if (length < 0) length = 0;
  char* r = (char*)malloc((size_t)length + 1);
  strncpy(r, s + index, (size_t)length);
  r[length] = '\0';
  return r;
}

static ef_factor* factor_new(int es, int ee, int gs, int ge) {
  ef_factor* f = (ef_factor*)malloc(sizeof(ef_factor));
// ... 782 lines not shown
  for (size_t v = 0; v < nx; ++v) if (slot[v] >= 0 && rs[slot[v]].v[2] != 0) idx[n++] = (int)v + 1;
  fact = keep_best_run(fact, idx, n);
  if (!efl_empty(fact)) {
    ef_phase(EFP_NOISY);
    n = 0;
    int index = 1;
    size_t v = 0;
    it = efl_begin(fact);
    while (efi_has_next(&it)) {
      const ef_factor* x = (const ef_factor*)efi_next(&it);
      while (v < nx && xs[v] != x) ++v;
      const bool ok = v < nx && slot[v] >= 0 && rs[slot[v]].v[0] != 0;
      if (!ok) idx[n++] = index;
      ++index;
    }
    fact = keep_best_run(fact, idx, n);
  }
  if (!small) { free(xs); free(slot); free(idx); free(rq); free(rs); }
  return fact;
}

static ef_list* clean_candidates(ef_list* cands, ef_list* flist, unsigned est_len, const char* GEN, const char* EST,
                                 const ef_config* cfg, ef_backend* be) {
  ef_iter ci = efl_begin(cands);
  while (efi_has_next(&ci)) {
    ef_list* f = (ef_list*)efi_next(&ci);
    bool ok = not_source_sink(f, (int)est_len);
    if (ok) ok = exon_start_end_ok(f);
    if (ok) { ef_phase(EFP_ENDPOINTS); f = handle_endpoints(f, GEN, EST, cfg, be); if (efl_empty(f)) ok = false; }
    if (ok) { ef_phase(EFP_EXTERNAL); f = ef_clean_external_exons(f, GEN, EST, be); if (efl_empty(f)) ok = false; }
    if (ok) { ef_phase(EFP_DUST); f = clean_complexity_and_noise(f, GEN, EST, cfg, be); if (efl_empty(f)) ok = false; }
    ef_phase(EFP_ADD);
    if (ok) ok = est_coverage_ok(f, EST);
    if (ok) {
      bool added;
      flist = ef_add_if_not_exists(f, flist, cfg, &added);
      if (!added) ef_factorization_free(f);
    } else {
      ef_factorization_free(f);
    }
  }
  efl_free(cands, NULL);
  return flist;
}

static bool chain_embedding(const void* rec, const ef_config* cfg, const char* GEN, ef_work* wk, emb** out) {
  const uint32_t* head = (const uint32_t*)rec;
  const uint32_t nv = head[0];
  if (nv < 2 || nv > 64) return false;
  const int32_t* vt = (const int32_t*)((const char*)rec + 16);
  const uint16_t* first = (const uint16_t*)((const char*)rec + 16 + 12 * (size_t)nv);
  const uint8_t* tgt = (const uint8_t*)rec + 16 + 12 * (size_t)nv + 2 * ((size_t)nv + 1);
  if (vt[0] != EF_SOURCE_START) return false;
  uint8_t path[64];
  uint64_t seen = 0;
  uint32_t k = 0, n = 0;
  for (;;) {
    if (seen >> k & 1u) return false;
    seen |= 1ull << k; path[n++] = (uint8_t)k;
    const uint32_t deg = (uint32_t)first[k + 1] - first[k];
    if (deg == 0) break;
    if (deg != 1) return false;
    k = tgt[first[k]];
    if (k >= nv) return false;
  }
  if (n != nv || vt[3 * (size_t)path[n - 1]] != EF_SINK_START) return false;
  wk->used += nv;
  ef_pairing node;
  memset(&node, 0, sizeof node);
  emb* e = emb_new(1);
  { const int32_t* s3 = vt + 3 * (size_t)path[n - 1]; e->e[0].p = s3[0]; e->e[0].t = s3[1]; e->e[0].l = s3[2]; }
  for (uint32_t q = n - 1; q-- > 0 && e;) {
    const int32_t* v3 = vt + 3 * (size_t)path[q];
    node.p = v3[0]; node.t = v3[1]; node.l = v3[2];
    emb* nx = update_embedding(e, &node, GEN, cfg);
    embedding_free(e);
    e = nx;
    if (e) ++wk->used;
  }
  *out = e;
  return true;
}

ef_est* ef_get_est_factorizations(const ef_seq* est_info, ef_meg* V, const ef_config* cfg,
                                  const ef_seq* gen_info, ef_backend* be) {
  ef_phase(EFP_EMBED);
  ef_est* est = (ef_est*)calloc(1, sizeof(ef_est));
  est->info = est_info;
  const char* GEN = gen_info->seq;
  const char* EST = est_info->seq;
  const unsigned est_len = (unsigned)V->n - 2;
  ef_list* flist = efl_new();
  ef_work wk = { 0, work_limit(cfg) };
  emb* chain = NULL;
  if (V->rec && !V->v && ef_chain_fast_path && chain_embedding(V->rec, cfg, GEN, &wk, &chain)) {
    if (ef_prof_on) ++ef_prof.chain_graphs;
    if (wk.used > wk.limit) {
      if (chain) embedding_free(chain);
      efl_free(flist, ef_factorization_free);
      free(est);
      return NULL;
    }
    if (chain) {
      ef_list* embs = efl_new();
      efl_push_back(embs, chain);
      ef_list* cands = factorizations_from_embeddings(embs, cfg);
      efl_free(embs, embedding_free);
      flist = clean_candidates(cands, flist, est_len, GEN, EST, cfg, be);
    }
  } else {
  if (ef_prof_on) ++ef_prof.other_graphs;
  V = ef_meg_lists(V);
  EF_MEG_FOR_POS(V, i, 0, V->n) {
    ef_iter it = efl_begin(V->v[i]);
    while (efi_has_next(&it)) { ef_pairing* p = (ef_pairing*)efi_next(&it); p->visited = false; p->emb_memo = NULL; }
  }
  EF_MEG_FOR_POS(V, i, 0, V->n) {
    ef_iter it = efl_begin(V->v[i]);
    while (efi_has_next(&it)) {
      ef_pairing* root = (ef_pairing*)efi_next(&it);
      if (root->visited) continue;
      ef_phase(EFP_EMBED);
      ef_list* embs = subtree_embeddings(root, cfg, GEN, &wk);
      if (!embs) {
        EF_MEG_FOR_POS(V, j, 0, V->n) {
          ef_iter jt = efl_begin(V->v[j]);
          while (efi_has_next(&jt)) { ef_pairing* q = (ef_pairing*)efi_next(&jt); if (q->emb_memo) { efl_free(q->emb_memo, embedding_free); q->emb_memo = NULL; } }
        }
        efl_free(flist, ef_factorization_free);
        free(est);
        return NULL;
      }
      flist = clean_candidates(factorizations_from_embeddings(embs, cfg), flist, est_len, GEN, EST, cfg, be);
    }
  }
  EF_MEG_FOR_POS(V, i, 0, V->n) {
    ef_iter it = efl_begin(V->v[i]);
    while (efi_has_next(&it)) { ef_pairing* p = (ef_pairing*)efi_next(&it); if (p->emb_memo) { efl_free(p->emb_memo, embedding_free); p->emb_memo = NULL; } }
  }
  }
  {
    unsigned long long hw = __atomic_load_n(&work_high_water, __ATOMIC_RELAXED);
    while (wk.used > hw && !__atomic_compare_exchange_n(&work_high_water, &hw, wk.used, true, __ATOMIC_RELAXED, __ATOMIC_RELAXED)) { }
  }

  ef_phase(EFP_FILTERS);
  {
    const size_t nf = efl_size(flist);
    double cov_small[32];
    double* cov = nf < 32 ? cov_small : (double*)malloc((nf + 1) * sizeof(double));
    double max_cov = 0.0;
    size_t k = 0;
    ef_iter it = efl_begin(flist);
    while (efi_has_next(&it)) {
      ef_list* f = (ef_list*)efi_next(&it);
      bool src_sink = false;
      if (efl_size(f) == 1) {
        const ef_factor* h = (const ef_factor*)efl_head(f);
        if (h->EST_start < 0 || h->EST_start >= (int)est_len) { cov[k] = -1.0; src_sink = true; }
      }
      if (!src_sink) { cov[k] = coverage_of(f, est_len); if (max_cov < cov[k]) max_cov = cov[k]; }
      ++k;
    }
    k = 0;
    it = efl_begin(flist);
    const int slen = (int)strlen(EST);
    while (efi_has_next(&it)) {
      efi_next(&it);
      const double c = cov[k++];
      if (c == -1.0 || max_cov - c > cfg->max_coverage_diff) efi_remove(&it, ef_factorization_free);
      else if ((max_cov - c) * slen > 100) efi_remove(&it, ef_factorization_free);
    }
    if (cov != cov_small) free(cov);
  }
  {
    const size_t nf = efl_size(flist);
    int gl_small[32];
    int* gl = nf < 32 ? gl_small : (int*)malloc((nf + 1) * sizeof(int));
    int min_gl = -1;
    size_t k = 0;
    ef_iter it = efl_begin(flist);
    while (efi_has_next(&it)) {
      gl[k] = gap_length_of((ef_list*)efi_next(&it));
      if (min_gl == -1 || min_gl > gl[k]) min_gl = gl[k];
      ++k;
    }
    k = 0;
    it = efl_begin(flist);
    while (efi_has_next(&it)) {
      efi_next(&it);
      const int g = gl[k++];
      if (cfg->max_gapLength_diff != -1 && g - min_gl > cfg->max_gapLength_diff) efi_remove(&it, ef_factorization_free);
    }
    if (gl != gl_small) free(gl);
  }
  ef_phase(EFP_GAPERR);
  if (be->ahead) {
    ef_ahead_collect(be, true);
    ef_iter it = efl_begin(flist);
    while (efi_has_next(&it)) check_gap_errors((ef_list*)efi_next(&it), EST, GEN, cfg, be);
    ef_ahead_collect(be, false);
    if (ef_ahead_flush(be) != 0) { fprintf(stderr, "* FATAL dynamic-programming backend failed\n"); abort(); }
  }
  {
    ef_iter it = efl_begin(flist);
    while (efi_has_next(&it)) {
      ef_list* f = (ef_list*)efi_next(&it);
      if (!check_gap_errors(f, EST, GEN, cfg, be)) efi_remove(&it, ef_factorization_free);
    }
  }
  if (cfg->max_number_of_factorizations != 0 && (int)efl_size(flist) > cfg->max_number_of_factorizations) {
    efl_free(flist, ef_factorization_free);
    flist = efl_new();
  }
  ef_phase(EFP_INTRON);
  {
    enum { GAP_AHEAD_MAX = 24 };
    ef_gap_ahead* pre = NULL; size_t n_pre = 0;
    if (be->ahead && be->dp_many) {
      size_t total = 0;
      ef_iter it = efl_begin(flist);
      while (efi_has_next(&it)) { const size_t k = efl_size((ef_list*)efi_next(&it)); total += k ? k - 1 : 0; }
      if (total >= 2 && total <= GAP_AHEAD_MAX) {
        pre = (ef_gap_ahead*)malloc(total * sizeof(ef_gap_ahead));
        ef_dp_req rq[GAP_AHEAD_MAX]; ef_dp_res rs[GAP_AHEAD_MAX];
        it = efl_begin(flist);
        while (efi_has_next(&it)) {
          ef_list* f = (ef_list*)efi_next(&it);
          if (efl_empty(f)) continue;
          ef_iter fi = efl_begin(f);
          const ef_factor* donor = (const ef_factor*)efi_next(&fi);
          while (efi_has_next(&fi)) {
            const ef_factor* acc = (const ef_factor*)efi_next(&fi);
            ef_gap_window_build(cfg, gen_info, est_info, donor, acc, &pre[n_pre].w);
            pre[n_pre].donor = *donor; pre[n_pre].acceptor = *acc;
            const ef_dp_req q = { EF_DP_GAP, pre[n_pre].w.seq_est, pre[n_pre].w.le, pre[n_pre].w.seq_gen, pre[n_pre].w.lg, 0, 0, 0, 0, 1 };
            rq[n_pre++] = q;
            donor = acc;
          }
        }
        memset(rs, 0, n_pre * sizeof(ef_dp_res));
        if (be->dp_many(be->self, rq, rs, n_pre) != 0) { fprintf(stderr, "* FATAL gap alignment backend failed\n"); abort(); }
        for (size_t k = 0; k < n_pre; ++k) pre[k].res = rs[k];
        if (ef_prof_on) ef_prof.ahead_asked += n_pre;
      }
    }
    size_t at = 0;
    ef_iter it = efl_begin(flist);
    while (efi_has_next(&it)) {
      ef_list* f = (ef_list*)efi_next(&it);
      if (efl_empty(f)) continue;
      ef_iter fi = efl_begin(f);
      ef_factor* donor = (ef_factor*)efi_next(&fi);
      bool first = true;
      while (efi_has_next(&fi)) {
        ef_factor* acc = (ef_factor*)efi_next(&fi);
        ef_refine_intron(cfg, gen_info, est_info, donor, acc, first, be, pre && at < n_pre ? &pre[at] : NULL);
        ++at;
        first = false;
        donor = acc;
      }
      fi = efl_begin(f);
      const ef_factor* e1 = (const ef_factor*)efi_next(&fi);
      if (efi_has_next(&fi)) {
        const ef_factor* e2 = (const ef_factor*)efi_next(&fi);
        if (e1->EST_start == e2->EST_start) free(efl_pop_front(f));
      }
    }
    for (size_t k = 0; k < n_pre; ++k) { ef_gap_window_release(&pre[k].w); ef_dp_res_release(&pre[k].res); }
    free(pre);
  }
  ef_phase(EFP_TAIL);
  est->polyA_signals = efl_new();
  est->polyadenil_signals = efl_new();
  {
    ef_iter it = efl_begin(flist);
    while (efi_has_next(&it)) {
      ef_list* f = (ef_list*)efi_next(&it);
      correct_tail(f, GEN, est_info->original_seq);
      bool polyadenil = false;
      const bool polyA = detect_polyA(f, GEN, est_info->original_seq, &polyadenil);
      efl_push_back(est->polyA_signals, polyA ? (void*)1 : (void*)2);
      efl_push_back(est->polyadenil_signals, polyadenil ? (void*)1 : (void*)2);
    }
  }
  est->factorizations = flist;
  return est;
}
```

pintron_amd/host/ef_sched.c:

```c
#define _GNU_SOURCE
#include <malloc.h>
#include <pthread.h>
#include <sys/uio.h>
#include <errno.h>
#include <sys/prctl.h>
#include <sys/syscall.h>
#include <linux/futex.h>
#include <sys/resource.h>
#include <sched.h>
#include <dirent.h>
#include <time.h>
#include <stdlib.h>
#include <string.h>
#include <stdint.h>
#include <ucontext.h>
#include <sys/mman.h>

#if defined(__x86_64__) && !defined(EF_USE_UCONTEXT)
typedef struct { void* sp; } ef_ctx;
void ef_ctx_switch(void** save_sp, void* new_sp);
void ef_ctx_entry(void);
__asm__(
  ".text\n"
  ".globl ef_ctx_switch\n.type ef_ctx_switch,@function\n"
  "ef_ctx_switch:\n"
  "  pushq %rbp\n  pushq %rbx\n  pushq %r12\n  pushq %r13\n  pushq %r14\n  pushq %r15\n"
  "  movq %rsp, (%rdi)\n  movq %rsi, %rsp\n"
  "  popq %r15\n  popq %r14\n  popq %r13\n  popq %r12\n  popq %rbx\n  popq %rbp\n"
  "  ret\n"
  ".size ef_ctx_switch,.-ef_ctx_switch\n"
  ".globl ef_ctx_entry\n.type ef_ctx_entry,@function\n"
  "ef_ctx_entry:\n"
  "  movq %r12, %rdi\n  callq *%r13\n  ud2\n"
  ".size ef_ctx_entry,.-ef_ctx_entry\n");
static inline void ctx_switch(ef_ctx* from, ef_ctx* to) { ef_ctx_switch(&from->sp, to->sp); }
static void ctx_make(ef_ctx* c, char* stack, size_t size, void (*fn)(void*), void* arg) {
  uintptr_t top = ((uintptr_t)stack + size) & ~(uintptr_t)15;
  void** S = (void**)(top - 16);
  S[-1] = (void*)ef_ctx_entry;
  S[-2] = NULL;
  S[-3] = NULL;
  S[-4] = arg;
  S[-5] = (void*)fn;
  S[-6] = NULL;
  S[-7] = NULL;
  c->sp = (void*)(S - 7);
}
#else
typedef struct { ucontext_t uc; } ef_ctx;
static inline void ctx_switch(ef_ctx* from, ef_ctx* to) { swapcontext(&from->uc, &to->uc); }
static void ctx_tramp(unsigned fh, unsigned fl, unsigned ah, unsigned al) {
  void (*fn)(void*) = (void (*)(void*))(((uintptr_t)fh << 32) | (uintptr_t)fl);
  fn((void*)(((uintptr_t)ah << 32) | (uintptr_t)al));
}
static void ctx_make(ef_ctx* c, char* stack, size_t size, void (*fn)(void*), void* arg) {
  getcontext(&c->uc);
  c->uc.uc_stack.ss_sp = stack; c->uc.uc_stack.ss_size = size; c->uc.uc_link = NULL;
  const uintptr_t f = (uintptr_t)fn, a = (uintptr_t)arg;
  makecontext(&c->uc, (void (*)(void))ctx_tramp, 4, (unsigned)(f >> 32), (unsigned)(f & 0xffffffffu), (unsigned)(a >> 32), (unsigned)(a & 0xffffffffu));
}
#endif
#if defined(__SANITIZE_THREAD__)
void* __tsan_get_current_fiber(void);
void* __tsan_create_fiber(unsigned flags);
void __tsan_destroy_fiber(void* fiber);
void __tsan_switch_to_fiber(void* fiber, unsigned flags);
#define EF_TSAN 1
#else
#define EF_TSAN 0
#endif
#include <unistd.h>

#include "estfact.h"
#include "ef_gpu.h"
#include "ef_sched.h"

enum { F_RUNNABLE, F_WAIT_DP, F_WAIT_PAIR, F_DONE };

#if EF_TSAN
static inline void tsan_to(void* fiber) { __tsan_switch_to_fiber(fiber, 0); }
#else
static inline void tsan_to(void* fiber) { (void)fiber; }
#endif

static double now_s(void) { struct timespec ts; clock_gettime(CLOCK_MONOTONIC, &ts); return ts.tv_sec + 1e-9 * ts.tv_nsec; }

struct worker;
#define EF_N_OUT 7

typedef struct fiber {
  ef_ctx ctx;
  void* tsan;
  char* stack; bool guarded;
  struct worker* w;
  int state;
  size_t unit;
  size_t cur_entry;
  int lane;
  int phase;
  const ef_dp_req* reqs; ef_dp_res* ress; size_t nreq;
  ef_dp_req req1; int rc;
  const char* pat; size_t pat_len; unsigned pat_L; double pat_rate; ef_triple** pat_out; size_t* pat_n;
  ef_backend be;
  struct fiber* pool_next;
  ef_sink out[EF_N_OUT];
} fiber;

static const char FIBER_SENTINEL[16] = "pintron-fibre-s";

static inline void fiber_prefetch(const fiber* f) {
#if defined(__x86_64__) && !defined(EF_USE_UCONTEXT)
  const char* sp = (const char*)f->ctx.sp;
  for (int k = 0; k < 12; ++k) __builtin_prefetch(sp + 64 * k, 0, 3);
#endif
  __builtin_prefetch(f->ress, 0, 3);
  __builtin_prefetch(f->reqs, 0, 3);
}

#define EF_GUARD_BYTES 4096u
static char* stack_alloc(size_t size, bool* guarded) {
  void* m = mmap(NULL, size + EF_GUARD_BYTES, PROT_READ | PROT_WRITE, MAP_PRIVATE | MAP_ANONYMOUS | MAP_STACK, -1, 0);
  if (m != MAP_FAILED && mprotect(m, EF_GUARD_BYTES, PROT_NONE) == 0) { *guarded = true; return (char*)m + EF_GUARD_BYTES; }
  if (m != MAP_FAILED) munmap(m, size + EF_GUARD_BYTES);
  *guarded = false;
  return (char*)malloc(size);
}
static void stack_free(char* stack, size_t size, bool guarded) {
  if (!stack) return;
  if (guarded) munmap(stack - EF_GUARD_BYTES, size + EF_GUARD_BYTES); else free(stack);
}

typedef struct {
  size_t first; bool has_sibling;
  char* buf[EF_N_OUT]; size_t len[EF_N_OUT];
} unit;

typedef struct merged_batch {
  pgpu_dp_result* results; char* strings;
  int refs;
} merged_batch;

typedef struct dp_request {
  const pgpu_dp_job* jobs; size_t n; const char* arena; size_t arena_len;
  merged_batch* batch; size_t base;
  int rc;
  uint32_t done;
  uint32_t* wake;
  struct dp_request* next;
} dp_request;

static inline void request_publish(dp_request* rq) {
  uint32_t* wake = rq->wake;
  __atomic_store_n(&rq->done, 1u, __ATOMIC_RELEASE);
  __atomic_add_fetch(wake, 1u, __ATOMIC_RELEASE);
  syscall(SYS_futex, wake, FUTEX_WAKE_PRIVATE, 1, NULL, NULL, 0);
}
static inline void worker_sleep(uint32_t* wake, uint32_t seen) {
  syscall(SYS_futex, wake, FUTEX_WAIT_PRIVATE, seen, NULL, NULL, 0);
}

#define MAX_SERVICES 8
#define EF_MAX_WORKERS 256
typedef struct service_thread {
  pthread_t thread;
  struct service* sv;
  pgpu_ctx* ctx;
  ef_sched_stats stats;
  double* iv; size_t n_iv, cap_iv;
  double phase_s[6];
} service_thread;

typedef struct service {
  pthread_mutex_t mu;
  pthread_cond_t posted, finished;
  dp_request *head, *tail;
  bool stop;
  struct shared* sh;
  int n_threads;
  long coalesce_us;
  service_thread threads[MAX_SERVICES];
} service;

#define PRE_CHUNKS 16
typedef struct shared {
  ef_inputs* in;
  pgpu_index* idx;
  unit* units; size_t n_units; size_t units_cap;
  size_t next_unit;
  pthread_mutex_t mu;
  size_t max_fibers, stack_size;
  int n_pre;
  size_t pre_lo[PRE_CHUNKS + 1];
  pgpu_pairing* pre_tri[PRE_CHUNKS]; uint64_t* pre_first[PRE_CHUNKS];
  bool use_meg;
  pgpu_meg_params meg_prm;
  unsigned char* pre_meg[PRE_CHUNKS]; size_t pre_meg_cap[PRE_CHUNKS]; uint64_t* pre_meg_first[PRE_CHUNKS];
  unsigned char* pre_slab; size_t pre_slab_cap, pre_slab_used;
  bool pre_own[PRE_CHUNKS], pre_first_own[PRE_CHUNKS];
  char* up_stage; size_t up_stage_cap;
  size_t ready_entries;
  pthread_cond_t ready_cv;
  bool kernel_timing;
  size_t gen_len;
  int n_lanes;
  service svc;
  int failed;
  ef_sched_stats stats;
  fiber* fiber_pool;
  fiber* worker_pool[EF_MAX_WORKERS];
  struct out_chunk* chunks;
  struct out_chunk* spare_chunks;
  unsigned long long prof_cyc[EFP_N], prof_susp[EFP_N], prof_jobs[EFP_N];
  unsigned long long prof_ahead[5];
  double prof_t0; double prof_sleep_bins[64];
} shared;

typedef struct out_chunk { struct out_chunk* next; size_t cap, used; char data[]; } out_chunk;

#define MAX_LANES 16
typedef struct lane {
  fiber** fibers; size_t n_fibers;
  ef_jobbuf jb;
  dp_request rq; bool posted;
  fiber** inflight; size_t n_inflight;
} lane;

typedef struct worker {
  shared* sh;
  size_t index;
  double sleep_bins[64];
  size_t suspensions;
  ef_ctx sched;
  void* tsan_sched;
  fiber* free_fibers;
  out_chunk* chunk;
  lane lanes[MAX_LANES];
  uint32_t wake;
  pgpu_ctx* ctx;
  size_t held_unit; bool holding;
  ef_sched_stats stats;
} worker;

static void kstat_add(ef_sched_stats* st, const ef_kernel_stat* k) {
  for (int i = 0; i < st->n_kernels; ++i)
    if (!strcmp(st->kernels[i].name, k->name)) {
      st->kernels[i].ms += k->ms; st->kernels[i].launches += k->launches; st->kernels[i].jobs += k->jobs;
      st->kernels[i].cells += k->cells; st->kernels[i].algo_bytes += k->algo_bytes;
      return;
    }
  if (st->n_kernels < EF_MAX_KERNELS) st->kernels[st->n_kernels++] = *k;
}

static int fiber_dp_many(void* self, const ef_dp_req* reqs, ef_dp_res* res, size_t n) {
  fiber* f = (fiber*)self;
  if (n == 0) return 0;
  f->reqs = reqs; f->ress = res; f->nreq = n; f->state = F_WAIT_DP;
  ++f->w->suspensions;
  if (ef_prof_on) { ef_prof.susp[f->phase]++; ef_prof.jobs[f->phase] += n; }
  if (EF_TSAN) tsan_to(f->w->tsan_sched);
  ctx_switch(&f->ctx, &f->w->sched);
  return f->rc;
}

static int fiber_dp(void* self, const ef_dp_req* q, ef_dp_res* res) {
  fiber* f = (fiber*)self;
  f->req1 = *q;
  return fiber_dp_many(self, &f->req1, res, 1);
}

static int fiber_pairings(void* self, const char* pattern, size_t m, unsigned L, double rate, ef_triple** out, size_t* n) {
  fiber* f = (fiber*)self;
  const shared* sh = f->w->sh;
  int c = 0;
  if (sh->n_pre) while (f->cur_entry >= sh->pre_lo[c + 1]) ++c;
  if (sh->n_pre && sh->pre_tri[c] && L == sh->in->cfg.min_factor_len && rate == sh->in->cfg.min_string_depth_rate &&
      pattern == sh->in->list[f->cur_entry]->seq) {
    const size_t e = f->cur_entry - sh->pre_lo[c];
    const uint64_t a = sh->pre_first[c][e], b = sh->pre_first[c][e + 1];
    ef_triple* t = (ef_triple*)malloc((size_t)(b - a + 1) * sizeof(ef_triple));
    memcpy(t, sh->pre_tri[c] + a, (size_t)(b - a) * sizeof(ef_triple));
    *out = t; *n = (size_t)(b - a);
    return 0;
  }
  f->pat = pattern; f->pat_len = m; f->pat_L = L; f->pat_rate = rate; f->pat_out = out; f->pat_n = n;
  f->state = F_WAIT_PAIR;
  if (EF_TSAN) tsan_to(f->w->tsan_sched);
  ctx_switch(&f->ctx, &f->w->sched);
  return f->rc;
}

static const void* fiber_meg(void* self, const char* pattern, size_t m, const ef_config* cfg) {
  (void)m;
  fiber* f = (fiber*)self;
  const shared* sh = f->w->sh;
  if (!sh->use_meg || !sh->n_pre || cfg->min_factor_len != sh->in->cfg.min_factor_len ||
      cfg->min_string_depth_rate != sh->in->cfg.min_string_depth_rate || pattern != sh->in->list[f->cur_entry]->seq)
    return NULL;
  int c = 0;
  while (f->cur_entry >= sh->pre_lo[c + 1]) ++c;
  if (!sh->pre_meg[c]) return NULL;
  return sh->pre_meg[c] + sh->pre_meg_first[c][f->cur_entry - sh->pre_lo[c]];
}

static char* out_alloc(worker* w, size_t n) {
  out_chunk* c = w->chunk;
  if (!c || c->used + n > c->cap) {
    const size_t cap = n > (1u << 20) ? n : (1u << 20);
    shared* sh = w->sh;
    c = NULL;
    pthread_mutex_lock(&sh->mu);
    if (sh->spare_chunks && sh->spare_chunks->cap >= n) { c = sh->spare_chunks; sh->spare_chunks = c->next; }
    pthread_mutex_unlock(&sh->mu);
    if (!c) { c = (out_chunk*)malloc(sizeof(out_chunk) + cap); c->cap = cap; }
    c->used = 0;
    pthread_mutex_lock(&sh->mu);
    c->next = sh->chunks; sh->chunks = c;
    pthread_mutex_unlock(&sh->mu);
    w->chunk = c;
  }
  char* r = c->data + c->used;
  c->used += n;
  return r;
}

static void fiber_main(void* arg) {
  fiber* f = (fiber*)arg;
  shared* sh = f->w->sh;
  unit* u = &sh->units[f->unit];
  ef_sink* fs = f->out;
  for (int k = 0; k < EF_N_OUT; ++k) { fs[k].f = NULL; fs[k].len = 0; }
  ef_side_files side = { &fs[2], &fs[3], &fs[4], &fs[5] };
  const ef_inputs* in = sh->in;
  for (size_t k = u->first; k <= u->first + (u->has_sibling ? 1 : 0); ++k) {
    f->cur_entry = k;
    ef_est* fe = ef_compute_est_fact(in->gen, in->list[k], &f->be, &in->cfg, &side);
    const bool aligned = !efl_empty(fe->factorizations);
    ef_phase(EFP_OUTPUT);
    if (aligned) {
      ef_write_multifasta_output(in->gen, fe, &fs[0], in->cfg.retain_externals);
      ef_write_factorization_records(in->gen, fe, &fs[6], in->cfg.retain_externals, (uint32_t)f->unit);
      ef_write_single_est_info(&fs[1], fe->info);
    }
    ef_phase(EFP_FREE);
    ef_est_free(fe);
    ef_phase(EFP_OTHER);
    if (aligned) break;
  }
  ef_phase(EFP_OUTPUT);
  for (int k = 0; k < EF_N_OUT; ++k) {
    u->len[k] = fs[k].len;
    u->buf[k] = fs[k].len ? out_alloc(f->w, fs[k].len) : NULL;
    if (fs[k].len) memcpy(u->buf[k], fs[k].mem, fs[k].len);
  }
  f->state = F_DONE;
  if (EF_TSAN) tsan_to(f->w->tsan_sched);
  ctx_switch(&f->ctx, &f->w->sched);
}

static inline bool unit_ready(const shared* sh, size_t u) {
  if (!sh->n_pre) return true;
  const size_t last = sh->units[u].first + (sh->units[u].has_sibling ? 1 : 0);
  return last < __atomic_load_n(&sh->ready_entries, __ATOMIC_ACQUIRE);
}
static void wait_unit_ready(shared* sh, size_t u) {
  const size_t last = sh->units[u].first + (sh->units[u].has_sibling ? 1 : 0);
  const int was = ef_phase(EFP_WAIT_PREFETCH);
  pthread_mutex_lock(&sh->mu);
  while (last >= sh->ready_entries && !sh->failed) pthread_cond_wait(&sh->ready_cv, &sh->mu);
  pthread_mutex_unlock(&sh->mu);
  ef_phase(was);
}
static inline bool worker_has_work(const worker* w) {
  for (int k = 0; k < w->sh->n_lanes; ++k) if (w->lanes[k].n_fibers > 0 || w->lanes[k].posted) return true;
  return false;
}

enum { START_NONE = 0, START_OK = 1, START_LATER = 2 };
static int start_fiber(worker* w, int li) {
  shared* sh = w->sh;
  lane* ln = &w->lanes[li];
  fiber* f = w->free_fibers;
  size_t u;
  if (w->holding) u = w->held_unit;
  else {
    u = __atomic_fetch_add(&sh->next_unit, 1, __ATOMIC_RELAXED);
    if (u >= sh->n_units) return START_NONE;
  }
  if (!unit_ready(sh, u)) {
    if (worker_has_work(w)) { w->held_unit = u; w->holding = true; return START_LATER; }
    wait_unit_ready(sh, u);
  }
  w->holding = false;
  if (__atomic_load_n(&sh->failed, __ATOMIC_RELAXED)) return START_NONE;
  if (f) w->free_fibers = f->pool_next;
  else if (__atomic_load_n(&sh->fiber_pool, __ATOMIC_RELAXED)) {
    pthread_mutex_lock(&sh->mu);
    if (sh->fiber_pool) {
      f = sh->fiber_pool;
      fiber* last = f;
      for (int k = 0; k < 32 && last->pool_next; ++k) last = last->pool_next;
      sh->fiber_pool = last->pool_next;
      last->pool_next = NULL;
      w->free_fibers = f->pool_next; f->pool_next = NULL;
    }
    pthread_mutex_unlock(&sh->mu);
  }
  if (f) {
    char* st = f->stack;
    const bool gd = f->guarded;
    void* ts = f->tsan;
    ef_sink keep[EF_N_OUT];
    memcpy(keep, f->out, sizeof keep);
    memset(f, 0, sizeof(fiber));
    f->stack = st; f->guarded = gd; f->tsan = ts;
    memcpy(f->out, keep, sizeof keep);
  }
  else { f = (fiber*)calloc(1, sizeof(fiber)); f->stack = stack_alloc(sh->stack_size, &f->guarded); }
  f->w = w; f->unit = u; f->state = F_RUNNABLE; f->lane = li;
  f->be.self = f; f->be.pairings = fiber_pairings; f->be.dp = fiber_dp; f->be.dp_many = fiber_dp_many; f->be.meg = fiber_meg;
  memcpy(f->stack, FIBER_SENTINEL, sizeof FIBER_SENTINEL);
#if EF_TSAN
  if (f->tsan) __tsan_destroy_fiber(f->tsan);
  f->tsan = __tsan_create_fiber(0);
  w->tsan_sched = __tsan_get_current_fiber();
#endif
  ctx_make(&f->ctx, f->stack, sh->stack_size, fiber_main, f);
  ln->fibers[ln->n_fibers++] = f;
  return START_OK;
}

static int submit_pairings(worker* w, lane* ln) {
  fiber** wait = (fiber**)malloc((ln->n_fibers + 1) * sizeof(fiber*));
  size_t nw = 0;
  for (size_t i = 0; i < ln->n_fibers; ++i) if (ln->fibers[i]->state == F_WAIT_PAIR) wait[nw++] = ln->fibers[i];
  int rc = 0;
  while (nw > 0 && rc == 0) {
    const unsigned L = wait[0]->pat_L; const double rate = wait[0]->pat_rate;
    size_t ng = 0, total = 0;
    for (size_t i = 0; i < nw; ++i) if (wait[i]->pat_L == L && wait[i]->pat_rate == rate) { ++ng; total += wait[i]->pat_len; }
    char* blob = (char*)malloc(total + 1);
    uint64_t* off = (uint64_t*)malloc((ng + 1) * sizeof(uint64_t));
    fiber** grp = (fiber**)malloc(ng * sizeof(fiber*));
    size_t g = 0, pos = 0, rest = 0;
    for (size_t i = 0; i < nw; ++i) {
      fiber* f = wait[i];
      if (f->pat_L == L && f->pat_rate == rate) { off[g] = pos; memcpy(blob + pos, f->pat, f->pat_len); pos += f->pat_len; grp[g++] = f; }
      else wait[rest++] = f;
    }
    off[ng] = pos;
    pgpu_pairing_plan* plan = NULL;
    pgpu_pairing_params prm = { L, 0, rate };
    if (!w->ctx && pgpu_init(ef_gpu_device_from_env(), &w->ctx) != PGPU_OK) { free(blob); free(off); free(grp); free(wait); return 1; }
    rc = pgpu_pairing_plan_create(w->ctx, w->sh->idx, blob, off, ng, &plan);
    if (rc == PGPU_OK) rc = pgpu_pairing_plan_run(w->ctx, plan, &prm);
    if (rc == PGPU_OK) {
      const size_t cnt = (size_t)pgpu_pairing_plan_count(plan);
      pgpu_pairing* out = (pgpu_pairing*)malloc((cnt + 1) * sizeof(pgpu_pairing));
      uint64_t* first = (uint64_t*)malloc((ng + 1) * sizeof(uint64_t));
      rc = pgpu_pairing_plan_fetch(w->ctx, plan, out, cnt, first);
      if (rc == PGPU_OK) {
        for (size_t i = 0; i < ng; ++i) {
          const size_t n = (size_t)(first[i + 1] - first[i]);
          ef_triple* t = (ef_triple*)malloc((n + 1) * sizeof(ef_triple));
          memcpy(t, out + first[i], n * sizeof(ef_triple));
          *grp[i]->pat_out = t; *grp[i]->pat_n = n;
          grp[i]->rc = 0; grp[i]->state = F_RUNNABLE;
        }
        w->stats.pairing_batches++; w->stats.pairing_requests += ng;
      }
      free(out); free(first);
    }
    if (plan) pgpu_pairing_plan_destroy(w->ctx, plan);
    if (rc != PGPU_OK) fprintf(stderr, "* FATAL pairing batch failed: %s\n", pgpu_last_error(w->ctx));
    free(blob); free(off); free(grp);
    nw = rest;
  }
  free(wait);
  return rc;
}

static void kstat_add(ef_sched_stats* st, const ef_kernel_stat* k);

static void* service_main(void* arg) {
  pthread_setname_np(pthread_self(), "ef-gpu-service");
  prctl(PR_SET_TIMERSLACK, 1000UL, 0, 0, 0);
  service_thread* me = (service_thread*)arg;
  service* sv = me->sv;
  shared* sh = sv->sh;
  pgpu_dp_part* parts = NULL; size_t parts_cap = 0;
  for (;;) {
    pthread_mutex_lock(&sv->mu);
    const double t_idle = now_s();
    while (!sv->head && !sv->stop) pthread_cond_wait(&sv->posted, &sv->mu);
    me->phase_s[0] += now_s() - t_idle;
    if (sv->coalesce_us > 0 && sv->head && !sv->stop) {
      pthread_mutex_unlock(&sv->mu);
      struct timespec ts = { 0, sv->coalesce_us * 1000L };
      nanosleep(&ts, NULL);
      pthread_mutex_lock(&sv->mu);
    }
    dp_request* list = sv->head;
    sv->head = sv->tail = NULL;
    const bool stop = sv->stop;
    pthread_mutex_unlock(&sv->mu);
    if (!list) { if (stop) break; else continue; }
    size_t nj = 0; int nreq = 0;
    for (dp_request* r = list; r; r = r->next) ++nreq;
    if ((size_t)nreq > parts_cap) { parts_cap = (size_t)nreq * 2; parts = (pgpu_dp_part*)realloc(parts, parts_cap * sizeof(pgpu_dp_part)); }
    {
      size_t q = 0;
      for (dp_request* r = list; r; r = r->next, ++q) {
        r->base = nj;
        parts[q].jobs = r->jobs; parts[q].n_jobs = r->n; parts[q].arena = r->arena; parts[q].arena_len = r->arena_len;
        nj += r->n;
      }
    }
    merged_batch* mb = (merged_batch*)calloc(1, sizeof(merged_batch));
    mb->refs = nreq;
    mb->results = (pgpu_dp_result*)malloc((nj + 1) * sizeof(pgpu_dp_result));
    pgpu_dp_plan* plan = NULL;
    const double t_a = now_s();
    me->phase_s[1] += t_a - t_idle - 0;
    pgpu_range_push("dp batch (create, launch, sync, fetch)");
    int rc = pgpu_dp_plan_create_parts(me->ctx, sh->idx, parts, (size_t)nreq, &plan);
    const double t_b = now_s();
    if (rc == PGPU_OK) rc = pgpu_dp_plan_launch(me->ctx, plan);
    const double t_c = now_s();
    if (rc == PGPU_OK) rc = pgpu_dp_plan_sync(me->ctx, plan);
    const double t_d = now_s();
    me->phase_s[2] += t_b - t_a; me->phase_s[3] += t_c - t_b; me->phase_s[4] += t_d - t_c;
    if (rc == PGPU_OK) {
      const size_t sb = pgpu_dp_plan_string_bytes(plan);
      mb->strings = (char*)malloc(sb + 16);
      rc = pgpu_dp_plan_fetch(me->ctx, plan, mb->results, mb->strings, sb + 16);
    }
    if (rc == PGPU_OK && sh->kernel_timing) {
      const int ng = pgpu_dp_plan_n_groups(plan);
      for (int g = 0; g < ng; ++g) {
        pgpu_group_info gi;
        if (pgpu_dp_plan_group_info(plan, g, &gi) != PGPU_OK || gi.jobs == 0) continue;
        ef_kernel_stat ks; memset(&ks, 0, sizeof ks);
        snprintf(ks.name, sizeof ks.name, "%s", gi.name);
        ks.ms = gi.ms; ks.launches = 1; ks.jobs = gi.jobs; ks.cells = gi.cells; ks.algo_bytes = gi.algo_bytes;
        kstat_add(&me->stats, &ks);
        if (gi.t0_ms >= 0 && gi.ms > 0) {
          if (me->n_iv + 2 > me->cap_iv) { me->cap_iv = me->cap_iv ? me->cap_iv * 2 : 4096; me->iv = (double*)realloc(me->iv, me->cap_iv * sizeof(double)); }
          me->iv[me->n_iv++] = gi.t0_ms; me->iv[me->n_iv++] = gi.t0_ms + gi.ms;
        }
      }
    }
    if (plan) pgpu_dp_plan_destroy(me->ctx, plan);
    pgpu_range_pop();
    me->phase_s[5] += now_s() - t_d;
    if (rc != PGPU_OK) fprintf(stderr, "* FATAL DP batch failed: %s\n", pgpu_last_error(me->ctx));
    me->stats.dp_batches++; me->stats.dp_jobs += nj;
    for (dp_request* r = list; r;) { dp_request* nx = r->next; r->batch = mb; r->rc = rc; request_publish(r); r = nx; }
  }
  free(parts);
  return NULL;
}

static int launch_dp(worker* w, lane* ln) {
  shared* sh = w->sh;
  service* sv = &sh->svc;
  const char* gen = sh->in->gen->seq;
  ef_jobbuf_reset(&ln->jb);
  ln->n_inflight = 0;
  for (size_t i = 0; i < ln->n_fibers; ++i) {
    fiber* f = ln->fibers[i];
    if (f->state != F_WAIT_DP) continue;
    for (size_t k = 0; k < f->nreq; ++k) ef_jobbuf_add(&ln->jb, &f->reqs[k], gen, sh->gen_len);
    ln->inflight[ln->n_inflight++] = f;
  }
  if (ln->n_inflight == 0) return 0;
  dp_request* rq = &ln->rq;
  memset(rq, 0, sizeof *rq);
  rq->wake = &w->wake;
  rq->jobs = ln->jb.jobs; rq->n = ln->jb.n; rq->arena = ln->jb.arena; rq->arena_len = ln->jb.arena_len;
  pthread_mutex_lock(&sv->mu);
  if (sv->tail) sv->tail->next = rq; else sv->head = rq;
  sv->tail = rq;
  pthread_cond_signal(&sv->posted);
  pthread_mutex_unlock(&sv->mu);
  ln->posted = true;
  return 0;
}

static int collect_dp(worker* w, lane* ln) {
  if (!ln->posted) return 0;
  dp_request* rq = &ln->rq;
  for (;;) {
    const uint32_t seen = __atomic_load_n(&w->wake, __ATOMIC_ACQUIRE);
    if (__atomic_load_n(&rq->done, __ATOMIC_ACQUIRE)) break;
    ef_phase(EFP_SLEEP);
    worker_sleep(&w->wake, seen);
    ef_phase(EFP_SCHED_COLLECT);
  }
  ln->posted = false;
  const int rc = rq->rc;
  const bool tracing = ef_dp_trace_enabled() != 0;
  if (rc == PGPU_OK) {
    size_t j = rq->base;
    for (size_t i = 0; i < ln->n_inflight; ++i) {
      fiber* f = ln->inflight[i];
      f->rc = 0;
      for (size_t k = 0; k < f->nreq; ++k, ++j) {
        const int drc = ef_decode_result(f->reqs[k].kind, &rq->batch->results[j], rq->batch->strings, &f->ress[k]);
        if (drc != 0) {
          fprintf(stderr, "* FATAL DP job of kind %d (%zu x %zu) exceeds the device limits\n", f->reqs[k].kind, f->reqs[k].la, f->reqs[k].lb);
          f->rc = drc;
        }
        else if (tracing) ef_dp_trace(&f->reqs[k], &f->ress[k], (uint32_t)f->unit);
      }
      f->state = F_RUNNABLE;
    }
  }
  const bool last = __atomic_sub_fetch(&rq->batch->refs, 1, __ATOMIC_ACQ_REL) == 0;
  if (last) { free(rq->batch->results); free(rq->batch->strings); free(rq->batch); }
  ln->n_inflight = 0;
  return rc;
}

static void* worker_main(void* arg) {
  pthread_setname_np(pthread_self(), "ef-worker");
  worker* w = (worker*)arg;
  shared* sh = w->sh;
  const int n_lanes = sh->n_lanes;
  const size_t per_lane = sh->max_fibers / n_lanes ? sh->max_fibers / n_lanes : 1;
  for (int li = 0; li < n_lanes; ++li) {
    lane* ln = &w->lanes[li];
    ln->fibers = (fiber**)malloc(per_lane * sizeof(fiber*));
    ln->inflight = (fiber**)malloc(per_lane * sizeof(fiber*));
    ef_jobbuf_init(&ln->jb);
  }
  if (ef_prof_on) { memset(&ef_prof, 0, sizeof ef_prof); ef_prof.dummy = EFP_SCHED; ef_prof.last = ef_prof_now(); }
  if (w->index < EF_MAX_WORKERS) { w->free_fibers = sh->worker_pool[w->index]; sh->worker_pool[w->index] = NULL; }
  bool more = true;
  int cursor = 0;
  const bool prefetch_on = !getenv("PINTRON_NO_FIBER_PREFETCH");
  while (!sh->failed) {
    int li = -1, first_posted = -1;
    const bool can_start = more && (!w->holding || unit_ready(sh, w->held_unit));
    for (int k = 0; k < n_lanes; ++k) {
      const int idx = (cursor + k) % n_lanes;
      lane* c = &w->lanes[idx];
      if (c->posted) {
        if (__atomic_load_n(&c->rq.done, __ATOMIC_ACQUIRE)) { li = idx; break; }
        if (first_posted < 0) first_posted = idx;
      } else if (c->n_fibers > 0 || can_start) { li = idx; break; }
    }
    if (li < 0 && first_posted < 0 && more && w->holding) {
      wait_unit_ready(sh, w->held_unit);
      if (sh->failed) break;
      continue;
    }
    if (li < 0 && first_posted >= 0) {
      const double tw = now_s();
      ef_phase(EFP_SLEEP);
      for (;;) {
        const uint32_t seen = __atomic_load_n(&w->wake, __ATOMIC_ACQUIRE);
        for (int k = 0; k < n_lanes && li < 0; ++k) {
          const int idx = (cursor + k) % n_lanes;
          if (w->lanes[idx].posted && __atomic_load_n(&w->lanes[idx].rq.done, __ATOMIC_ACQUIRE)) li = idx;
        }
        if (li >= 0 || sh->failed) break;
        worker_sleep(&w->wake, seen);
      }
      w->stats.dp_s += now_s() - tw;
      if (ef_prof_on) {
        const double t1 = now_s();
        int b = (int)((tw - sh->prof_t0) / 0.005); if (b < 0) b = 0; if (b > 63) b = 63;
        w->sleep_bins[b] += t1 - tw;
      }
      ef_phase(EFP_SCHED);
      if (li < 0) break;
    }
    if (li < 0) break;
    cursor = (li + 1) % n_lanes;
    lane* ln = &w->lanes[li];
    double t0 = now_s();
    ef_phase(EFP_SCHED_COLLECT);
    if (collect_dp(w, ln) != 0) { sh->failed = 1; break; }
    w->stats.dp_s += now_s() - t0;
    ef_phase(EFP_SCHED_START);
    while (more && ln->n_fibers < per_lane) {
      const int sr = start_fiber(w, li);
      if (sr == START_LATER) break;
      more = sr == START_OK;
    }
    ef_phase(EFP_SCHED);
    if (ln->n_fibers > 0) {
      t0 = now_s();
      for (size_t i = 0; i < ln->n_fibers; ++i) {
        fiber* f = ln->fibers[i];
        if (prefetch_on && i + 2 < ln->n_fibers) fiber_prefetch(ln->fibers[i + 2]);
        if (f->state == F_RUNNABLE) {
          if (EF_TSAN) tsan_to(f->tsan);
          if (ef_prof_on) { ef_phase(EFP_SCHED); ef_prof.cur = &f->phase; }
          ctx_switch(&w->sched, &f->ctx);
          if (ef_prof_on) { ef_phase(f->phase); ef_prof.cur = NULL; ef_prof.dummy = EFP_SCHED; }
        }
      }
      size_t keep = 0;
      for (size_t i = 0; i < ln->n_fibers; ++i) {
        fiber* f = ln->fibers[i];
        if (f->state == F_DONE) {
          if (memcmp(f->stack, FIBER_SENTINEL, sizeof FIBER_SENTINEL) != 0) {
            fprintf(stderr, "* FATAL fibre stack overflow (raise PINTRON_FIBER_STACK_KB, now %zu)\n", sh->stack_size / 1024);
            abort();
          }
          f->pool_next = w->free_fibers; w->free_fibers = f; w->stats.units++;
        }
        else ln->fibers[keep++] = f;
      }
      ln->n_fibers = keep;
      w->stats.host_s += now_s() - t0;
      t0 = now_s();
      int brc = submit_pairings(w, ln);
      w->stats.pairing_s += now_s() - t0;
      t0 = now_s();
      ef_phase(EFP_SCHED_LAUNCH);
      if (brc == 0) brc = launch_dp(w, ln);
      ef_phase(EFP_SCHED);
      w->stats.dp_s += now_s() - t0;
      if (brc != 0) { sh->failed = 1; break; }
    }
  }
  for (int li = 0; li < n_lanes; ++li) {
    lane* ln = &w->lanes[li];
    collect_dp(w, ln);
    ef_jobbuf_free(&ln->jb);
    free(ln->fibers); free(ln->inflight);
  }
  if (w->ctx) pgpu_destroy(w->ctx);
  if (w->free_fibers && w->index < EF_MAX_WORKERS) { sh->worker_pool[w->index] = w->free_fibers; w->free_fibers = NULL; }
  if (w->free_fibers) {
    fiber* last = w->free_fibers;
    while (last->pool_next) last = last->pool_next;
    pthread_mutex_lock(&sh->mu);
    last->pool_next = sh->fiber_pool; sh->fiber_pool = w->free_fibers;
    pthread_mutex_unlock(&sh->mu);
    w->free_fibers = NULL;
  }
  ef_cell_release_all();
  if (ef_prof_on) {
    ef_phase(EFP_SCHED);
    pthread_mutex_lock(&sh->mu);
    for (int k = 0; k < EFP_N; ++k) { sh->prof_cyc[k] += ef_prof.cyc[k]; sh->prof_susp[k] += ef_prof.susp[k]; sh->prof_jobs[k] += ef_prof.jobs[k]; }
    for (int k = 0; k < 64; ++k) sh->prof_sleep_bins[k] += w->sleep_bins[k];
    sh->prof_ahead[0] += ef_prof.ahead_asked; sh->prof_ahead[1] += ef_prof.ahead_hits; sh->prof_ahead[2] += ef_prof.ahead_misses;
    sh->prof_ahead[3] += ef_prof.chain_graphs; sh->prof_ahead[4] += ef_prof.other_graphs;
    pthread_mutex_unlock(&sh->mu);
  }
  return NULL;
}

static bool env_flag(const char* name) {
  const char* v = getenv(name);
  return v && !(v[0] == '0' && v[1] == '\0');
}

static size_t env_size(const char* name, size_t dflt) {
  const char* v = getenv(name);
  return (v && atol(v) > 0) ? (size_t)atol(v) : dflt;
}

static size_t host_core_share(void) {
  long n = sysconf(_SC_NPROCESSORS_ONLN);
  cpu_set_t set;
  if (sched_getaffinity(0, sizeof set, &set) == 0 && CPU_COUNT(&set) > 0 && CPU_COUNT(&set) < n) n = CPU_COUNT(&set);
  long long quota = -1, period = 0;
  FILE* f = fopen("/sys/fs/cgroup/cpu.max", "r");
  if (f) {
    char q[32];
    if (fscanf(f, "%31s %lld", q, &period) == 2 && strcmp(q, "max") != 0) quota = atoll(q);
    fclose(f);
  } else if ((f = fopen("/sys/fs/cgroup/cpu/cpu.cfs_quota_us", "r")) != NULL) {
    if (fscanf(f, "%lld", &quota) != 1) quota = -1;
    fclose(f);
    if ((f = fopen("/sys/fs/cgroup/cpu/cpu.cfs_period_us", "r")) != NULL) {
      if (fscanf(f, "%lld", &period) != 1) period = 0;
      fclose(f);
    }
  }
  if (quota > 0 && period > 0) {
    const long q = (long)((quota + period - 1) / period);
    if (q < n) n = q;
  }
  const char* lws = getenv("LOCAL_WORLD_SIZE");
  if (lws && atol(lws) > 1) n /= atol(lws);
  if (n > 16) n = 16;
  return n > 0 ? (size_t)n : 1;
}

static size_t default_workers(void) {
  const size_t c = host_core_share();
  return c + c / 8;
}

static cpu_set_t numa_original;
static int numa_bound = -2;
static int open_sessions;

static int guess_gpu_numa_node(int dev) {
  if (getenv("HIP_VISIBLE_DEVICES") || getenv("ROCR_VISIBLE_DEVICES") || getenv("CUDA_VISIBLE_DEVICES")) return -1;
  int minors[64], n = 0;
  DIR* d = opendir("/dev/dri");
  if (!d) return -1;
  for (struct dirent* e; (e = readdir(d)) != NULL && n < 64;)
    if (strncmp(e->d_name, "renderD", 7) == 0) minors[n++] = atoi(e->d_name + 7);
  closedir(d);
  for (int i = 1; i < n; ++i) for (int j = i; j > 0 && minors[j - 1] > minors[j]; --j) { const int t = minors[j]; minors[j] = minors[j - 1]; minors[j - 1] = t; }
  if (dev < 0 || dev >= n) return -1;
  char path[96];
// ... 821 lines not shown
    if (sh->pre_slab && !kept.pre_slab) { kept.pre_slab = sh->pre_slab; kept.pre_slab_cap = sh->pre_slab_cap; sh->pre_slab = NULL; }
    if (sh->up_stage && !kept.up_stage) { kept.up_stage = sh->up_stage; kept.up_stage_cap = sh->up_stage_cap; sh->up_stage = NULL; }
    pthread_mutex_unlock(&kept.mu);
  }
  tq[2] = now_s();
  if (sh->pre_slab) pgpu_host_free(s->ctx0, sh->pre_slab);
  if (sh->up_stage) pgpu_host_free(s->ctx0, sh->up_stage);
  if (s->ctx0 && sh->idx) pgpu_index_destroy(s->ctx0, sh->idx);
  tq[3] = now_s();
  for (int k = 0; k < MAX_SERVICES; ++k) ctx_give(sh->svc.threads[k].ctx, s->device);
  ctx_give(s->ctx0, s->device);
  tq[4] = now_s();
  ef_free_inputs(&s->in);
  tq[5] = now_s();
  if (verbose)
    fprintf(stderr, "* close: unit buffers + fibres %.3fs, pairing plans %.3fs, index + slabs %.3fs, contexts %.3fs, inputs %.3fs\n",
            tq[1] - tq[0], tq[2] - tq[1], tq[3] - tq[2], tq[4] - tq[3], tq[5] - tq[4]);
  pthread_mutex_destroy(&sh->mu); pthread_cond_destroy(&sh->ready_cv);
  pthread_mutex_destroy(&sh->svc.mu); pthread_cond_destroy(&sh->svc.posted); pthread_cond_destroy(&sh->svc.finished);
  free(s);
  if (--open_sessions == 0) restore_affinity();
}

int ef_leave_without_cleanup = 0;

typedef struct { char* p; size_t len; } page_range;
typedef struct { page_range* r; size_t n; size_t next; } page_release;
static void* page_release_main(void* arg) {
  page_release* pr = (page_release*)arg;
  for (;;) {
    const size_t k = __atomic_fetch_add(&pr->next, 1, __ATOMIC_RELAXED);
    if (k >= pr->n) return NULL;
    madvise(pr->r[k].p, pr->r[k].len, MADV_DONTNEED);
  }
}
static void session_release_pages(ef_session* s) {
  shared* sh = &s->sh;
  merge_worker_pools(sh);
  size_t cap = 1024, n = 0;
  for (fiber* f = sh->fiber_pool; f; f = f->pool_next) ++cap;
  for (out_chunk* c = sh->chunks; c; c = c->next) ++cap;
  for (out_chunk* c = sh->spare_chunks; c; c = c->next) ++cap;
  void** ab = (void**)malloc(65536 * sizeof(void*)); size_t* al = (size_t*)malloc(65536 * sizeof(size_t));
  if (!ab || !al) { free(ab); free(al); return; }
  const size_t na = ef_record_arena_regions(s->in.arena, ab, al, 65536);
  page_range* r = (page_range*)malloc((cap + na) * 16 * sizeof(page_range));
  if (!r) { free(ab); free(al); return; }
  const size_t piece = (size_t)8 << 20, room = (cap + na) * 16;
#define ADD_RANGE(ptr, bytes) do { \
    uintptr_t a_ = ((uintptr_t)(ptr) + 4095) & ~(uintptr_t)4095, b_ = ((uintptr_t)(ptr) + (bytes)) & ~(uintptr_t)4095; \
    for (; a_ < b_ && n < room; a_ += piece) { r[n].p = (char*)a_; r[n].len = b_ - a_ < piece ? b_ - a_ : piece; ++n; } } while (0)
  for (size_t k = 0; k < na; ++k) ADD_RANGE(ab[k], al[k]);
  for (out_chunk* c = sh->chunks; c; c = c->next) ADD_RANGE(c->data, c->cap);
  for (out_chunk* c = sh->spare_chunks; c; c = c->next) ADD_RANGE(c->data, c->cap);
  for (fiber* f = sh->fiber_pool; f; f = f->pool_next) if (f->guarded) ADD_RANGE(f->stack, sh->stack_size);
  if (sh->units) ADD_RANGE(sh->units, (sh->n_units + 1) * sizeof(unit));
#undef ADD_RANGE
  page_release pr = { r, n, 0 };
  size_t nth = host_core_share();
  if (nth > 16) nth = 16;
  pthread_t th[16]; size_t started = 0;
  for (size_t t = 1; t < nth; ++t) if (pthread_create(&th[started], NULL, page_release_main, &pr) == 0) ++started;
  page_release_main(&pr);
  for (size_t t = 0; t < started; ++t) pthread_join(th[t], NULL);
  free(r); free(ab); free(al);
}

int ef_run_batched_stats(int argc, char** argv, ef_sched_stats* stats_out) {
  const run_mark m0 = run_mark_now();
  ef_session* s = ef_session_open(argc, argv);
  if (!s) return 1;
  ef_sched_stats st;
  const run_mark m1 = run_mark_now();
  int rc = ef_session_step(s, &st);
  const run_mark m2 = run_mark_now();
  if (rc == 0) rc = ef_session_write_outputs(s);
  const run_mark m3 = run_mark_now();
  if (stats_out) *stats_out = st;
  const bool leave = ef_leave_without_cleanup != 0;
  if (!leave) ef_session_close(s);
  else if (!getenv("PINTRON_NO_PAGE_RELEASE")) session_release_pages(s);
  ef_log_reference_timers(st.index_s, st.prefetch_s, st.workers_s, st.load_s + (m3.wall - m2.wall), now_s() - m0.wall);
  if (getenv("PINTRON_VERBOSE")) {
    fprintf(stderr, "* run: open %.3fs step %.3fs write %.3fs close %.3fs\n", m1.wall - m0.wall, m2.wall - m1.wall, m3.wall - m2.wall, now_s() - m3.wall);
    fprintf(stderr, "* cpu (all threads): open user %.2fs sys %.2fs, %ld page faults; step user %.2fs sys %.2fs, %ld page faults; write user %.2fs sys %.2fs\n",
            m1.user - m0.user, m1.sys - m0.sys, m1.minflt - m0.minflt, m2.user - m1.user, m2.sys - m1.sys, m2.minflt - m1.minflt,
            m3.user - m2.user, m3.sys - m2.sys);
  }
  return rc;
}

int ef_run_batched(int argc, char** argv) {
  ef_sched_stats st;
  const int rc = ef_run_batched_stats(argc, argv, &st);
  if (rc == 0 && getenv("PINTRON_VERBOSE")) {
    fprintf(stderr, "est-fact: %zu ESTs (%zu aligned), %zu threads, %zu pairing batches (%zu requests), %zu DP batches (%zu jobs); "
                    "load %.2fs index %.2fs prefetch %.2fs workers %.2fs [per-thread avg: host %.2fs pairing %.2fs dp %.2fs]\n",
            st.units, st.aligned, st.threads, st.pairing_batches, st.pairing_requests, st.dp_batches, st.dp_jobs,
            st.load_s, st.index_s, st.prefetch_s, st.workers_s, st.host_s / st.threads, st.pairing_s / st.threads, st.dp_s / st.threads);
    for (int k = 0; k < st.n_kernels; ++k)
      fprintf(stderr, "  kernel %-28s launches %6zu jobs %9zu  %9.3f ms  %8.1f algo-GB/s\n", st.kernels[k].name, st.kernels[k].launches,
              st.kernels[k].jobs, st.kernels[k].ms, st.kernels[k].ms > 0 ? st.kernels[k].algo_bytes / (st.kernels[k].ms * 1e-3) / 1e9 : 0.0);
  }
  return rc;
}
```

pintron_amd/host/ef_sched.h:

```cpp
#ifndef EF_SCHED_H
#define EF_SCHED_H
#include <stddef.h>

#define EF_MAX_KERNELS 64
typedef struct {
  char name[48];
  double ms;
  size_t launches, jobs;
  unsigned long long cells, algo_bytes;
} ef_kernel_stat;

typedef struct {
  size_t threads, units, aligned, dp_batches, dp_jobs, pairing_batches, pairing_requests;
  double load_s, index_s, prefetch_s, workers_s;
  double host_s, pairing_s, dp_s;
  int n_kernels;
  ef_kernel_stat kernels[EF_MAX_KERNELS];
  double dp_busy_union_ms;
  double suspensions_per_unit;
} ef_sched_stats;

typedef struct ef_session ef_session;
ef_session* ef_session_open(int argc, char** argv);
int ef_session_step(ef_session* s, ef_sched_stats* stats);
int ef_session_write_outputs(ef_session* s);
char* ef_session_records(ef_session* s, size_t* len);
char* ef_session_output(ef_session* s, int which, size_t* len);
size_t ef_session_n_ests(const ef_session* s);
void ef_session_close(ef_session* s);

int ef_main_multi(int argc, char** argv);
struct pgpu_ctx* ef_session_context(ef_session* s);
const void* ef_session_genomic(ef_session* s);

extern int ef_leave_without_cleanup;
int ef_run_batched(int argc, char** argv);
int ef_run_batched_stats(int argc, char** argv, ef_sched_stats* stats);

#endif
```

pintron_amd/host/estfact.h:

```cpp
#ifndef ESTFACT_H
#define ESTFACT_H

#include <limits.h>
#include <stdbool.h>
#include <stddef.h>
#include <stdint.h>
#include <stdio.h>
#include <string.h>

#include "ef_list.h"

typedef struct {
  unsigned min_factor_len;
  int min_intron_length, max_intron_length;
  double min_string_depth_rate;
  double max_prefix_discarded_rate, max_suffix_discarded_rate;
  int max_prefix_discarded, max_suffix_discarded;
  unsigned max_site_difference;
  int max_number_of_factorizations;
  double max_coverage_diff;
  int max_exonNUM_diff, max_gapLength_diff;
  char retain_externals;
  unsigned max_pairings_in_MEG;
  double max_freq_shortest_pairing;
// ... 140 lines not shown
  ef_sink* s = w->s;
  if (s->f) { efw_flush(w); return; }
  if (w->p) s->len = (size_t)(w->p - s->mem);
  if (s->len + need > s->cap) { s->cap = (s->len + need) * 2 + 256; s->mem = (char*)realloc(s->mem, s->cap); }
  w->p = s->mem + s->len; w->end = s->mem + s->cap;
}
static inline void efw_ch(ef_wbuf* w, char c) { efw_room(w, 1); *w->p++ = c; }
static inline void efw_mem(ef_wbuf* w, const char* s, size_t n) {
  if (w->s->f && n > 2048) { efw_flush(w); fwrite(s, 1, n, w->s->f); return; }
  efw_room(w, n);
  memcpy(w->p, s, n); w->p += n;
}
static inline void efw_str(ef_wbuf* w, const char* s) { efw_mem(w, s, strlen(s)); }
static inline void efw_strn(ef_wbuf* w, const char* s, int prec) {
  if (prec <= 0) return;
  const char* z = (const char*)memchr(s, 0, (size_t)prec);
  efw_mem(w, s, z ? (size_t)(z - s) : (size_t)prec);
}
static inline void efw_int(ef_wbuf* w, long long v) {
  char t[24]; int k = 0;
  unsigned long long u = v < 0 ? 0ull - (unsigned long long)v : (unsigned long long)v;
  do { t[k++] = (char)('0' + u % 10); u /= 10; } while (u);
  efw_room(w, 24);
  if (v < 0) *w->p++ = '-';
  while (k) *w->p++ = t[--k];
}

enum { EFP_OTHER = 0, EFP_MEG, EFP_EMBED, EFP_ENDPOINTS, EFP_EXTERNAL, EFP_DUST, EFP_NOISY, EFP_ADD, EFP_FILTERS,
       EFP_GAPERR, EFP_INTRON, EFP_TAIL, EFP_FACTREF, EFP_OUTPUT, EFP_SIDE, EFP_FREE, EFP_SCHED, EFP_SLEEP,
       EFP_REF_AFFIX, EFP_REF_FALSE_SMALL, EFP_REF_NEW_SMALL, EFP_REF_CLEAN, EFP_SCHED_LAUNCH, EFP_SCHED_COLLECT, EFP_SCHED_START, EFP_WAIT_PREFETCH,
       EFP_NS_PREFIX, EFP_NS_BETWEEN_ASK, EFP_NS_BETWEEN_CLASS, EFP_NS_BETWEEN_SEARCH, EFP_TMP1, EFP_TMP2, EFP_TMP3, EFP_N };
extern int ef_prof_on;
typedef struct { unsigned long long cyc[EFP_N], susp[EFP_N], jobs[EFP_N]; unsigned long long last; int dummy; int* cur;
                 unsigned long long ahead_hits, ahead_misses, ahead_asked, chain_graphs, other_graphs; } ef_prof_state;
extern _Thread_local ef_prof_state ef_prof;
static inline unsigned long long ef_prof_now(void) {
#if defined(__x86_64__)
  unsigned lo, hi; __asm__ volatile("rdtsc" : "=a"(lo), "=d"(hi)); return ((unsigned long long)hi << 32) | lo;
#else
  return 0;
#endif
}
static inline int ef_phase(int id) {
  if (!ef_prof_on) return 0;
  ef_prof_state* p = &ef_prof;
  int* cur = p->cur ? p->cur : &p->dummy;
  const unsigned long long t = ef_prof_now();
  const int was = *cur;
  p->cyc[was] += t - p->last; p->last = t; *cur = id;
  return was;
}

enum { EF_DP_ALIGN = 0, EF_DP_GAP = 1, EF_DP_ED = 2, EF_DP_KBAND = 3, EF_DP_LCF = 4,
       EF_DP_BORDERS = 5, EF_DP_AFFIX = 6 };
typedef struct {
  int kind;
  const char* a; size_t la;
  const char* b; size_t lb;
  uint32_t p0, p1, p2, tail;
  uint32_t temp;
} ef_dp_req;
typedef struct {
  int32_t v[6];
  char* s0; char* s1;
} ef_dp_res;
#define EF_ROW_PAD 64
static inline void ef_dp_res_rows(ef_dp_res* r, size_t cap) {
  r->s0 = (char*)calloc(2 * (cap + EF_ROW_PAD), 1);
  r->s1 = r->s0 + cap + EF_ROW_PAD;
}
static inline void ef_dp_res_release(ef_dp_res* r) { free(r->s0); r->s0 = r->s1 = NULL; }

#define EF_AHEAD_MAX 96
#define EF_DP_PENDING 1
#define EF_AHEAD_SLOTS 256
typedef struct {
  int n, n_pending;
  bool collecting;
  unsigned char slot[EF_AHEAD_SLOTS];
  ef_dp_req q[EF_AHEAD_MAX]; int32_t v[EF_AHEAD_MAX][6];
} ef_ahead;
static inline void ef_ahead_init(ef_ahead* ah) { ah->n = ah->n_pending = 0; ah->collecting = false; memset(ah->slot, 0, sizeof ah->slot); }

typedef struct ef_backend {
  void* self;
  int (*pairings)(void* self, const char* pattern, size_t m, unsigned min_factor_len, double rate,
                  ef_triple** out, size_t* n);
  int (*dp)(void* self, const ef_dp_req* req, ef_dp_res* res);
  int (*dp_many)(void* self, const ef_dp_req* reqs, ef_dp_res* res, size_t n);
  const void* (*meg)(void* self, const char* pattern, size_t m, const ef_config* cfg);
  ef_ahead* ahead;
} ef_backend;

static inline bool ef_req_same(const ef_dp_req* x, const ef_dp_req* y) {
  return x->kind == y->kind && x->a == y->a && x->b == y->b && x->la == y->la && x->lb == y->lb &&
         x->p0 == y->p0 && x->p1 == y->p1 && x->p2 == y->p2 && x->tail == y->tail;
}
static inline bool ef_req_keepable(const ef_dp_req* q) { return q->temp == 0 && q->kind != EF_DP_ALIGN && q->kind != EF_DP_GAP; }
static inline unsigned ef_req_hash(const ef_dp_req* q) {
  uint64_t h = (uint64_t)(uintptr_t)q->a * 0x9E3779B97F4A7C15ull ^ (uint64_t)(uintptr_t)q->b * 0xC2B2AE3D27D4EB4Full;
  h ^= ((uint64_t)q->la << 32 | (uint64_t)q->lb) * 0x165667B19E3779F9ull + (uint64_t)q->kind;
  return (unsigned)(h >> 40) & (EF_AHEAD_SLOTS - 1);
}
static inline const int32_t* ef_ahead_find(const ef_ahead* ah, const ef_dp_req* q) {
  if (ah->n == 0 || !ef_req_keepable(q)) return NULL;
  for (unsigned s = ef_req_hash(q); ah->slot[s]; s = (s + 1) & (EF_AHEAD_SLOTS - 1))
    if (ef_req_same(&ah->q[ah->slot[s] - 1], q)) return ah->v[ah->slot[s] - 1];
  return NULL;
}
static inline unsigned ef_req_hash(const ef_dp_req* q);
static inline void ef_ahead_put(ef_ahead* ah, const ef_dp_req* q, const int32_t* v) {
  if (ah->n_pending || ah->n >= EF_AHEAD_MAX || !ef_req_keepable(q) || ef_ahead_find(ah, q)) return;
  ah->q[ah->n] = *q; memcpy(ah->v[ah->n], v, 6 * sizeof(int32_t));
  unsigned s = ef_req_hash(q);
  while (ah->slot[s]) s = (s + 1) & (EF_AHEAD_SLOTS - 1);
  ah->slot[s] = (unsigned char)(++ah->n);
}
static inline void ef_ahead_keep_next(ef_ahead* ah, const int32_t* v) {
  memcpy(ah->v[ah->n], v, 6 * sizeof(int32_t));
  unsigned s = ef_req_hash(&ah->q[ah->n]);
  while (ah->slot[s]) s = (s + 1) & (EF_AHEAD_SLOTS - 1);
  ah->slot[s] = (unsigned char)(++ah->n);
}
static inline int ef_backend_ask(ef_backend* be, const ef_dp_req* reqs, ef_dp_res* res, size_t n) {
  if (be->dp_many) return be->dp_many(be->self, reqs, res, n);
  for (size_t k = 0; k < n; ++k) { const int rc = be->dp(be->self, &reqs[k], &res[k]); if (rc != 0) return rc; }
  return 0;
}
int ef_dp_many_ahead(ef_backend* be, const ef_dp_req* reqs, ef_dp_res* res, size_t n);
static inline int ef_dp_many(ef_backend* be, const ef_dp_req* reqs, ef_dp_res* res, size_t n) {
  if (n == 0) return 0;
  memset(res, 0, n * sizeof(ef_dp_res));
  if (be->ahead && (be->ahead->n || be->ahead->collecting)) return ef_dp_many_ahead(be, reqs, res, n);
  return ef_backend_ask(be, reqs, res, n);
}
static inline int ef_dp_one(ef_backend* be, const ef_dp_req* req, ef_dp_res* res) { return ef_dp_many(be, req, res, 1); }
static inline void ef_ahead_collect(ef_backend* be, bool on) { if (be->ahead) be->ahead->collecting = on; }
static inline bool ef_collecting(const ef_backend* be) { return be->ahead && be->ahead->collecting; }
int ef_ahead_flush(ef_backend* be);
extern int ef_ahead_on;

typedef struct { int EST_start, EST_end, GEN_start, GEN_end; } ef_factor;

typedef struct {
  const ef_seq* info;
  ef_list* factorizations;
  ef_list* polyA_signals;
  ef_list* polyadenil_signals;
} ef_est;

void ef_factorization_free(void* fact);
void ef_est_free(ef_est* e);

unsigned long long ef_work_high_water(void);
ef_est* ef_get_est_factorizations(const ef_seq* est, ef_meg* V, const ef_config* cfg,
                                  const ef_seq* gen, ef_backend* be);
void ef_refine_est_factorizations(const ef_seq* gen, ef_est* e, const ef_config* cfg, ef_backend* be);
void ef_remove_factorizations_with_very_small_exons(ef_list* facts);
void ef_remove_duplicated_factorizations(ef_list* facts);
typedef struct {
  char* seq_est; char* seq_gen; size_t le, lg;
  int dsl_est, dsl_gen, deleted_intron_dim;
  char buf_e[512], buf_g[512];
} ef_gap_window;
typedef struct { ef_gap_window w; ef_dp_res res; ef_factor donor, acceptor; } ef_gap_ahead;
void ef_gap_window_build(const ef_config* cfg, const ef_seq* gen, const ef_seq* est, const ef_factor* donor,
                         const ef_factor* acceptor, ef_gap_window* w);
void ef_gap_window_release(ef_gap_window* w);
bool ef_refine_intron(const ef_config* cfg, const ef_seq* gen, const ef_seq* est, ef_factor* donor,
                      ef_factor* acceptor, bool first_intron, ef_backend* be, ef_gap_ahead* ahead);
int ef_classify_intron(const ef_seq* gen, int start, int end);
int ef_burset_frequency(const char* donor, const char* acceptor);
int ef_burset_adaptor(const char* t, size_t cut1, size_t cut2);
int ef_check_burset_patterns(const char* gen, int donor_left_on_gen, int acceptor_right_on_gen);
char* ef_real_substring(int index, int length, const char* s);
ef_list* ef_clean_noisy_exons(ef_list* fact, const char* gen, const char* est, bool only_internals, ef_backend* be);
ef_list* ef_clean_external_exons(ef_list* fact, const char* gen, const char* est, ef_backend* be);
ef_list* ef_add_if_not_exists(ef_list* to_add, ef_list* list, const ef_config* cfg, bool* added);
uint32_t ef_edit_distance(ef_backend* be, const char* a, size_t la, const char* b, size_t lb);
uint32_t ef_compute_edit_distance(ef_backend* be, const char* a, size_t la, const char* b, size_t lb);
void ef_write_multifasta_output(const ef_seq* gen, const ef_est* e, ef_sink* f, char retain_externals);
void ef_write_factorization_records(const ef_seq* gen, const ef_est* e, ef_sink* f, char retain_externals, uint32_t est_index);
int ef_raw_text_from_records(const ef_seq* gen, const void* rec, size_t rl, const char* pests, size_t pl, ef_sink* out);
typedef struct { ef_sink *fmeg, *fpmeg, *ftmeg, *fintronic; } ef_side_files;
ef_est* ef_compute_est_fact(const ef_seq* gen, const ef_seq* est, ef_backend* be, const ef_config* cfg,
                            const ef_side_files* side);

ef_meg* ef_build_meg(const ef_seq* est, ef_backend* be, const ef_config* shared_cfg, size_t* inc_pairing_len);

void ef_write_single_est_info(ef_sink* f, const ef_seq* s);

typedef struct { ef_config cfg; ef_seq* gen; ef_seq** list; size_t n; ef_record_arena* arena;
                 bool all_in_arena;
                 unsigned char* has_rev;
} ef_inputs;
typedef struct { FILE* flog; ef_sink fout, fests, fmeg, fpmeg, ftmeg, fintronic; ef_side_files side; } ef_outputs;
int ef_load_inputs(int argc, char** argv, ef_inputs* in);
int ef_load_genomic(int argc, char** argv, ef_inputs* in);
int ef_load_genomic_sequence(int argc, char** argv, ef_inputs* in);
void ef_prepare_genomic_tables(ef_inputs* in);
int ef_load_ests(ef_inputs* in);
extern int ef_shard_rank, ef_shard_world;
void ef_free_inputs(ef_inputs* in);
int ef_open_outputs(ef_outputs* o);
void ef_info_mark(const char* label);
void ef_close_outputs(ef_outputs* o);
void ef_classify_init(void);
void ef_classify_prepare(ef_seq* gen);

void ef_log_reference_timers(double suffix_tree_s, double algorithm_s, double compositions_s, double io_s, double total_s);
int ef_run(int argc, char** argv, ef_backend* (*open_backend)(const ef_seq* gen), void (*close_backend)(ef_backend*));

#endif
```

Measured before the change: 904,000.

## Split chain refinement into async launch/finish and batch it with DP requests

Splits the chain refinement call into an asynchronous launch and a finish step on a dedicated stream. Device, pinned and host buffers are kept per context and grown on demand instead of being allocated on every call. The scheduler now appends each fiber's chain queries to the lane's DP batch, so refinement runs on the GPU next to the DP plan rather than as separate blocking calls. This aims to remove per-call allocation and synchronisation overhead and to overlap chain work with DP. In exchange it adds in-flight state, more buffer management and new per-fiber bookkeeping.

```diff
diff --git a/include/pintron_gpu.h b/include/pintron_gpu.h
--- a/include/pintron_gpu.h
+++ b/include/pintron_gpu.h
@@ -125,6 +125,12 @@
                              const pgpu_factor* exons, size_t n_exons_total,
                              const pgpu_chain_query* q, size_t n,
                              pgpu_factor* out_exons, uint8_t* out_steps, pgpu_chain_result* out);
+int pgpu_index_refine_chains_launch(pgpu_ctx* ctx, const pgpu_index* idx, const char* ests, size_t ests_len,
+                                    const pgpu_factor* exons, size_t n_exons_total,
+                                    const pgpu_chain_query* q, size_t n);
+struct pgpu_group_info;
+int pgpu_index_refine_chains_finish(pgpu_ctx* ctx, pgpu_factor* out_exons, uint8_t* out_steps, pgpu_chain_result* out,
+                                    struct pgpu_group_info* group);
 double pgpu_index_refine_chains_kernel_ms(void);
 
 typedef struct {
@@ -239,7 +245,7 @@
 double   pgpu_dp_plan_kernel_ms(const pgpu_dp_plan* plan, int kind);
 uint64_t pgpu_dp_plan_launches(const pgpu_dp_plan* plan, int kind);
 
-typedef struct {
+typedef struct pgpu_group_info {
   char     name[48];
   int32_t  kind;
   int32_t  pad;
diff --git a/pintron_amd/capi.py b/pintron_amd/capi.py
--- a/pintron_amd/capi.py
+++ b/pintron_amd/capi.py
@@ -118,6 +118,7 @@
     "pgpu_index_classify", "pgpu_index_score5", "pgpu_index_small_exons", "pgpu_index_small_exons_kernel_ms",
     "pgpu_index_refine_introns", "pgpu_index_refine_introns_kernel_ms",
     "pgpu_index_refine_chains", "pgpu_index_refine_chains_kernel_ms",
+    "pgpu_index_refine_chains_launch", "pgpu_index_refine_chains_finish",
     "pgpu_pairing_plan_create", "pgpu_pairing_plan_create_resident", "pgpu_pairing_plan_run", "pgpu_pairing_plan_count",
     "pgpu_pairing_plan_positions", "pgpu_pairing_plan_kernel_ms", "pgpu_pairing_plan_fetch",
     "pgpu_pairing_plan_destroy",
@@ -179,6 +180,9 @@
         L.pgpu_index_refine_introns_kernel_ms.restype = C.c_double
         L.pgpu_index_refine_chains.argtypes = [vp, vp, C.c_char_p, sz, C.POINTER(Factor), sz, C.POINTER(ChainQuery), sz,
                                                C.POINTER(Factor), C.POINTER(C.c_uint8), C.POINTER(ChainResult)]
+        L.pgpu_index_refine_chains_launch.argtypes = [vp, vp, C.c_char_p, sz, C.POINTER(Factor), sz, C.POINTER(ChainQuery), sz]
+        L.pgpu_index_refine_chains_finish.argtypes = [vp, C.POINTER(Factor), C.POINTER(C.c_uint8), C.POINTER(ChainResult),
+                                                      C.POINTER(GroupInfo)]
         L.pgpu_index_refine_chains_kernel_ms.argtypes = []
         L.pgpu_index_refine_chains_kernel_ms.restype = C.c_double
         L.pgpu_pairing_plan_run_meg.argtypes = [vp, vp, vp]
@@ -391,6 +395,28 @@
         self.ctx.check(rc)
         return out_exons, out_steps, res
 
+    def refine_chains_launch_raw(self, ests: bytes, exons, queries, n: int, ctx=None):
+        ctx = ctx or self.ctx
+        rc = ctx.L.pgpu_index_refine_chains_launch(ctx.h, self.h, ests, len(ests), exons.ctypes.data_as(C.POINTER(Factor)),
+                                                   len(exons), queries.ctypes.data_as(C.POINTER(ChainQuery)), n)
+        if rc == PGPU_OK:
+            ctx._chain_sizes = (len(exons), n)
+        return rc
+
+    def refine_chains_finish_raw(self, ctx=None):
+        import numpy as np
+        ctx = ctx or self.ctx
+        n_exons, n = getattr(ctx, "_chain_sizes", (0, 0))
+        out_exons = np.zeros(n_exons, dtype=np.dtype(FACTOR_DTYPE))
+        out_steps = np.zeros(n_exons, dtype=np.uint8)
+        res = np.zeros(n, dtype=np.dtype(CHAIN_RESULT_DTYPE))
+        gi = GroupInfo()
+        rc = ctx.L.pgpu_index_refine_chains_finish(ctx.h, out_exons.ctypes.data_as(C.POINTER(Factor)),
+                                                   out_steps.ctypes.data_as(C.POINTER(C.c_uint8)),
+                                                   res.ctypes.data_as(C.POINTER(ChainResult)), C.byref(gi))
+        group = {"name": gi.name.decode(), "ms": gi.ms, "t0_ms": gi.t0_ms, "jobs": int(gi.jobs)}
+        return rc, out_exons, out_steps, res, group
+
     def refine_chains_kernel_ms(self):
         return self.ctx.L.pgpu_index_refine_chains_kernel_ms()
 
diff --git a/pintron_amd/csrc/pgpu_api.hip b/pintron_amd/csrc/pgpu_api.hip
--- a/pintron_amd/csrc/pgpu_api.hip
+++ b/pintron_amd/csrc/pgpu_api.hip
@@ -38,6 +38,7 @@
   void* pin[2] = {nullptr, nullptr};
   size_t pin_cap[2] = {0, 0};
   std::vector<hipEvent_t> ev_pool;
+  void* chain = nullptr;
 };
 
 static int wait_stream(pgpu_ctx* ctx, hipStream_t st) {
@@ -157,6 +158,15 @@
   return e == hipSuccess ? PGPU_OK : set_err(ctx, PGPU_EDEVICE, "hipSetDevice(%d) failed: %s", ctx->device, hipGetErrorString(e));
 }
 int pgpu_ctx_fail(pgpu_ctx* ctx, int code, const char* msg) { return set_err(ctx, code, "%s", msg); }
+void** pgpu_ctx_chain_slot(pgpu_ctx* ctx) { return &ctx->chain; }
+hipError_t pgpu_ctx_wait_event(pgpu_ctx* ctx, hipEvent_t ev) {
+  if (ctx->wait_poll_us == 0) return hipEventSynchronize(ev);
+  for (;;) {
+    const hipError_t e = hipEventQuery(ev);
+    if (e != hipErrorNotReady) return e;
+    if (ctx->wait_poll_us > 0) { struct timespec ts = {0, ctx->wait_poll_us * 1000L}; nanosleep(&ts, nullptr); }
+  }
+}
 
 extern "C" int pgpu_abi_version(void) { return 1; }
 
@@ -216,6 +226,11 @@
   }
   return g_base_event[device];
 }
+float pgpu_ctx_t0_ms(pgpu_ctx* ctx, hipEvent_t ev) {
+  hipEvent_t b = base_event(ctx->device, ctx->stream);
+  float t0 = 0.f;
+  return (b && hipEventElapsedTime(&t0, b, ev) == hipSuccess) ? t0 : -1.f;
+}
 
 extern "C" int pgpu_init(int device, pgpu_ctx** out) {
   if (!out) return PGPU_EINVAL;
@@ -248,6 +263,7 @@
   if (!ctx) return PGPU_EINVAL;
   hipSetDevice(ctx->device);
   hipStreamSynchronize(ctx->stream);
+  pgpu_chain_state_release(ctx->chain);
   for (auto& pl : ctx->pools) for (auto& q : pl.ptr) if (q) hipFree(q);
   for (auto& a : ctx->aux) if (a) { hipStreamSynchronize(a); hipStreamDestroy(a); }
   if (ctx->ev_upload) hipEventDestroy(ctx->ev_upload);
diff --git a/pintron_amd/csrc/pgpu_chain.hip b/pintron_amd/csrc/pgpu_chain.hip
--- a/pintron_amd/csrc/pgpu_chain.hip
+++ b/pintron_amd/csrc/pgpu_chain.hip
@@ -1,5 +1,7 @@
+#include <stdio.h>
 #include <stdlib.h>
 #include <string.h>
+#include <new>
 
 #include "pgpu_internal.h"
 #include "pgpu_query_call.h"
@@ -134,24 +136,102 @@
 
 constexpr unsigned WAVES_PER_CU = 16;
 
+struct ChainState {
+  hipStream_t st = nullptr;
+  hipEvent_t ev_done = nullptr, ev[2] = {nullptr, nullptr};
+  int cus = 0;
+  uint8_t* d = nullptr;   size_t d_cap = 0;
+  uint8_t* ws = nullptr;  size_t ws_cap = 0;
+  uint8_t* pin = nullptr; size_t pin_cap = 0;
+  uint8_t* named = nullptr; size_t named_cap = 0;
+  bool in_flight = false, timed = false;
+  size_t n = 0, n_exons = 0;
+  size_t p_oex = 0, p_st = 0, p_r = 0;
+};
+
+template <class Alloc, class Free>
+hipError_t grow(uint8_t*& p, size_t& cap, size_t bytes, Alloc alloc, Free release) {
+  if (cap >= bytes) return hipSuccess;
+  if (p) (void)release(p);
+  p = nullptr; cap = 0;
+  const size_t want = bytes + bytes / 2 + 4096;
+  const hipError_t e = alloc((void**)&p, want);
+  if (e != hipSuccess) { p = nullptr; return e; }
+  cap = want;
+  return hipSuccess;
+}
+hipError_t device_block(uint8_t*& p, size_t& cap, size_t bytes) {
+  return grow(p, cap, bytes, [](void** q, size_t b) { return hipMalloc(q, b); }, [](void* q) { return hipFree(q); });
+}
+hipError_t pinned_block(uint8_t*& p, size_t& cap, size_t bytes) {
+  return grow(p, cap, bytes, [](void** q, size_t b) { return hipHostMalloc(q, b, hipHostMallocDefault); },
+              [](void* q) { return hipHostFree(q); });
+}
+
+ChainState* chain_state(pgpu_ctx* ctx, hipError_t* err) {
+  void** slot = pgpu_ctx_chain_slot(ctx);
+  if (*slot) return (ChainState*)*slot;
+  ChainState* s = new (std::nothrow) ChainState();
+  if (!s) { *err = hipErrorOutOfMemory; return nullptr; }
+  int dev = 0;
+  hipError_t e = hipGetDevice(&dev);
+  if (e == hipSuccess) e = hipDeviceGetAttribute(&s->cus, hipDeviceAttributeMultiprocessorCount, dev);
+  if (e == hipSuccess) e = hipStreamCreateWithFlags(&s->st, hipStreamNonBlocking);
+  if (e == hipSuccess) e = hipEventCreateWithFlags(&s->ev_done, hipEventDisableTiming);
+  if (e != hipSuccess) { pgpu_chain_state_release(s); *err = e; return nullptr; }
+  *slot = s;
+  return s;
+}
+
+#define TRY_CHAIN(expr)                                                          \
+  do {                                                                           \
+    const hipError_t e_ = (expr);                                                \
+    if (e_ != hipSuccess) {                                                      \
+      (void)hipStreamSynchronize(s->st);                                         \
+      s->in_flight = false;                                                      \
+      return pgpu_ctx_fail(ctx, pgpu_code_of(e_), hipGetErrorString(e_));        \
+    }                                                                            \
+  } while (0)
+
+}
+
+void pgpu_chain_state_release(void* state) {
+  ChainState* s = (ChainState*)state;
+  if (!s) return;
+  if (s->st) (void)hipStreamSynchronize(s->st);
+  for (hipEvent_t e : { s->ev_done, s->ev[0], s->ev[1] }) if (e) (void)hipEventDestroy(e);
+  if (s->d) (void)hipFree(s->d);
+  if (s->ws) (void)hipFree(s->ws);
+  if (s->pin) (void)hipHostFree(s->pin);
+  free(s->named);
+  if (s->st) (void)hipStreamDestroy(s->st);
+  delete s;
 }
 
 extern "C" double pgpu_index_refine_chains_kernel_ms(void) { return t_chain_ms; }
 
-extern "C" int pgpu_index_refine_chains(pgpu_ctx* ctx, const pgpu_index* idx, const char* ests, size_t ests_len,
-                                        const pgpu_factor* exons, size_t n_exons_total,
-                                        const pgpu_chain_query* q, size_t n,
-                                        pgpu_factor* out_exons, uint8_t* out_steps, pgpu_chain_result* out) {
+extern "C" int pgpu_index_refine_chains_launch(pgpu_ctx* ctx, const pgpu_index* idx, const char* ests, size_t ests_len,
+                                               const pgpu_factor* exons, size_t n_exons_total,
+                                               const pgpu_chain_query* q, size_t n) {
   t_chain_ms = 0.0;
   static_assert(sizeof(pgpu_chain_query) == 40 && sizeof(pgpu_chain_result) == 16 && sizeof(pgpu_factor) == 16, "ABI layout");
-  if (!ctx || !idx || (n && (!q || !out)) || (ests_len && !ests) || (n_exons_total && (!exons || !out_exons || !out_steps)))
-    return PGPU_EINVAL;
+  if (!ctx || !idx || (n && !q) || (ests_len && !ests) || (n_exons_total && !exons)) return PGPU_EINVAL;
   if (n > 0x7fffffffull || n_exons_total > 0x7fffffffull)
     return pgpu_ctx_fail(ctx, PGPU_EINVAL, "more than 2^31 - 1 chains or exons in one call");
+  if (pgpu_ctx_bind(ctx) != PGPU_OK) return PGPU_EDEVICE;
+  hipError_t se = hipSuccess;
+  ChainState* const s = chain_state(ctx, &se);
+  if (!s) return pgpu_ctx_fail(ctx, pgpu_code_of(se), hipGetErrorString(se));
+  if (s->in_flight) return pgpu_ctx_fail(ctx, PGPU_EINVAL, "a chain call is in flight on this context: finish it first");
   const size_t glen = pgpu_index_length(idx);
-  struct Freed { uint8_t* p; ~Freed() { free(p); } } named_block{ (uint8_t*)calloc(n_exons_total ? n_exons_total : 1, 1) };
-  uint8_t* const named = named_block.p;
-  if (!named) return pgpu_ctx_fail(ctx, PGPU_ENOMEM, "no memory for the table of the exons the chains name");
+  if (s->named_cap < n_exons_total) {
+    free(s->named);
+    s->named_cap = n_exons_total + n_exons_total / 2 + 64;
+    s->named = (uint8_t*)malloc(s->named_cap);
+    if (!s->named) { s->named_cap = 0; return pgpu_ctx_fail(ctx, PGPU_ENOMEM, "no memory for the table of the exons the chains name"); }
+  }
+  uint8_t* const named = s->named;
+  if (n_exons_total) memset(named, 0, n_exons_total);
   for (size_t i = 0; i < n; ++i) {
     const pgpu_chain_query& x = q[i];
     bool ok = x.est_off <= ests_len && x.est_len <= ests_len - x.est_off && x.est_len <= 0x7fffffffu && x.reserved == 0 &&
@@ -171,38 +251,86 @@
                                              "share, a donor that is not in front of its acceptor, or a coordinate outside what it "
                                              "indexes)");
   }
+  const size_t ex_bytes = n_exons_total * sizeof(pgpu_factor), q_bytes = n * sizeof(pgpu_chain_query),
+               r_bytes = n * sizeof(pgpu_chain_result);
+  const size_t p_ex = up256(ests_len + 64), p_q = p_ex + up256(ex_bytes), p_oex = p_q + up256(q_bytes),
+               p_st = p_oex + up256(ex_bytes), p_r = p_st + up256(n_exons_total), p_total = p_r + up256(r_bytes);
+  TRY_CHAIN(pinned_block(s->pin, s->pin_cap, p_total));
+  s->n = n; s->n_exons = n_exons_total; s->p_oex = p_oex; s->p_st = p_st; s->p_r = p_r;
+  s->timed = false;
   if (n == 0) {
-    if (n_exons_total) { memcpy(out_exons, exons, n_exons_total * sizeof(pgpu_factor)); memset(out_steps, 0, n_exons_total); }
+    if (ex_bytes) memcpy(s->pin + p_oex, exons, ex_bytes);
+    if (n_exons_total) memset(s->pin + p_st, 0, n_exons_total);
+    s->in_flight = true;
     return PGPU_OK;
   }
+  const size_t waves = n < (size_t)s->cus * WAVES_PER_CU ? n : (size_t)s->cus * WAVES_PER_CU;
+  TRY_CHAIN(device_block(s->d, s->d_cap, p_total));
+  TRY_CHAIN(device_block(s->ws, s->ws_cap, waves * WS_WAVE));
+  if (pgpu_ctx_timing(ctx)) {
+    for (auto& e : s->ev) if (!e) TRY_CHAIN(hipEventCreate(&e));
+    s->timed = true;
+  }
+  if (ests_len) memcpy(s->pin, ests, ests_len);
+  memcpy(s->pin + p_ex, exons, ex_bytes);
+  memcpy(s->pin + p_q, q, q_bytes);
+  pgpu_range_push("refine chains (launch)");
+  struct Pop { ~Pop() { pgpu_range_pop(); } } pop;
+  const hipStream_t st = s->st;
+  uint8_t* const d = s->d;
+  TRY_CHAIN(hipMemcpyAsync(d, s->pin, p_oex, hipMemcpyHostToDevice, st));
+  TRY_CHAIN(hipMemcpyAsync(d + p_oex, d + p_ex, ex_bytes, hipMemcpyDeviceToDevice, st));
+  TRY_CHAIN(hipMemsetAsync(d + p_st, 0, n_exons_total, st));
+  if (s->timed) TRY_CHAIN(hipEventRecord(s->ev[0], st));
+  hipLaunchKernelGGL(chain_kernel, dim3((unsigned)waves), dim3(64), 0, st, pgpu_index_genomic(idx), (uint32_t)glen, d,
+                     (const pgpu_factor*)(d + p_ex), (const pgpu_chain_query*)(d + p_q), (uint32_t)n, s->ws,
+                     (pgpu_factor*)(d + p_oex), d + p_st, (pgpu_chain_result*)(d + p_r));
+  TRY_CHAIN(hipGetLastError());
+  if (s->timed) TRY_CHAIN(hipEventRecord(s->ev[1], st));
+  TRY_CHAIN(hipMemcpyAsync(s->pin + p_oex, d + p_oex, p_total - p_oex, hipMemcpyDeviceToHost, st));
+  TRY_CHAIN(hipEventRecord(s->ev_done, st));
+  s->in_flight = true;
+  return PGPU_OK;
+}
+
+extern "C" int pgpu_index_refine_chains_finish(pgpu_ctx* ctx, pgpu_factor* out_exons, uint8_t* out_steps,
+                                               pgpu_chain_result* out, pgpu_group_info* group) {
+  t_chain_ms = 0.0;
+  if (group) { memset(group, 0, sizeof *group); group->t0_ms = -1.0; }
+  if (!ctx) return PGPU_EINVAL;
+  ChainState* const s = (ChainState*)*pgpu_ctx_chain_slot(ctx);
+  if (!s || !s->in_flight) return pgpu_ctx_fail(ctx, PGPU_EINVAL, "no chain call is in flight on this context");
   if (pgpu_ctx_bind(ctx) != PGPU_OK) return PGPU_EDEVICE;
-  QueryCall call(ctx, "refine chains");
-  const hipStream_t st = call.st;
-  int dev = 0, cus = 0;
-  TRY_HIP(hipGetDevice(&dev));
-  TRY_HIP(hipDeviceGetAttribute(&cus, hipDeviceAttributeMultiprocessorCount, dev));
-  const size_t waves = n < (size_t)cus * WAVES_PER_CU ? n : (size_t)cus * WAVES_PER_CU;
-  const size_t ex_bytes = n_exons_total * sizeof(pgpu_factor);
-  const size_t o_ex = up256(ests_len + 64), o_q = o_ex + up256(ex_bytes), o_oex = o_q + up256(n * sizeof(pgpu_chain_query)),
-               o_st = o_oex + up256(ex_bytes), o_r = o_st + up256(n_exons_total), o_ws = o_r + up256(n * sizeof(pgpu_chain_result)),
-               total = o_ws + waves * WS_WAVE;
-  TRY_HIP(hipMalloc((void**)&call.d, total));
-  TRY_HIP(call.timing_events(1));
-  if (ests_len) TRY_HIP(hipMemcpyAsync(call.d, ests, ests_len, hipMemcpyHostToDevice, st));
-  TRY_HIP(hipMemcpyAsync(call.d + o_ex, exons, ex_bytes, hipMemcpyHostToDevice, st));
-  TRY_HIP(hipMemcpyAsync(call.d + o_q, q, n * sizeof(pgpu_chain_query), hipMemcpyHostToDevice, st));
-  TRY_HIP(hipMemcpyAsync(call.d + o_oex, call.d + o_ex, ex_bytes, hipMemcpyDeviceToDevice, st));
-  TRY_HIP(hipMemsetAsync(call.d + o_st, 0, n_exons_total, st));
-  TRY_HIP(call.record(0));
-  hipLaunchKernelGGL(chain_kernel, dim3((unsigned)waves), dim3(64), 0, st, pgpu_index_genomic(idx), (uint32_t)glen, call.d,
-                     (const pgpu_factor*)(call.d + o_ex), (const pgpu_chain_query*)(call.d + o_q), (uint32_t)n, call.d + o_ws,
-                     (pgpu_factor*)(call.d + o_oex), call.d + o_st, (pgpu_chain_result*)(call.d + o_r));
-  TRY_HIP(call.record(1));
-  TRY_HIP(hipMemcpyAsync(out_exons, call.d + o_oex, ex_bytes, hipMemcpyDeviceToHost, st));
-  TRY_HIP(hipMemcpyAsync(out_steps, call.d + o_st, n_exons_total, hipMemcpyDeviceToHost, st));
-  TRY_HIP(hipMemcpyAsync(out, call.d + o_r, n * sizeof(pgpu_chain_result), hipMemcpyDeviceToHost, st));
-  TRY_HIP(pgpu_ctx_wait(ctx));
-  TRY_HIP(hipGetLastError());
-  call.elapsed_ms(0, &t_chain_ms);
+  if (s->n) TRY_CHAIN(pgpu_ctx_wait_event(ctx, s->ev_done));
+  s->in_flight = false;
+  if ((s->n && !out) || (s->n_exons && (!out_exons || !out_steps))) return PGPU_EINVAL;
+  if (s->n_exons) {
+    memcpy(out_exons, s->pin + s->p_oex, s->n_exons * sizeof(pgpu_factor));
+    memcpy(out_steps, s->pin + s->p_st, s->n_exons);
+  }
+  if (s->n) memcpy(out, s->pin + s->p_r, s->n * sizeof(pgpu_chain_result));
+  if (s->n && s->timed) {
+    float ms = 0.f;
+    if (hipEventElapsedTime(&ms, s->ev[0], s->ev[1]) == hipSuccess) t_chain_ms = ms;
+    if (group) {
+      snprintf(group->name, sizeof group->name, "chain");
+      group->kind = -1;
+      size_t settled = 0;
+      for (size_t i = 0; i < s->n; ++i) settled += out[i].done;
+      group->jobs = settled; group->ms = ms; group->t0_ms = pgpu_ctx_t0_ms(ctx, s->ev[0]);
+    }
+  }
   return PGPU_OK;
 }
+
+extern "C" int pgpu_index_refine_chains(pgpu_ctx* ctx, const pgpu_index* idx, const char* ests, size_t ests_len,
+                                        const pgpu_factor* exons, size_t n_exons_total,
+                                        const pgpu_chain_query* q, size_t n,
+                                        pgpu_factor* out_exons, uint8_t* out_steps, pgpu_chain_result* out) {
+  t_chain_ms = 0.0;
+  if (!ctx || !idx || (n && (!q || !out)) || (ests_len && !ests) || (n_exons_total && (!exons || !out_exons || !out_steps)))
+    return PGPU_EINVAL;
+  const int rc = pgpu_index_refine_chains_launch(ctx, idx, ests, ests_len, exons, n_exons_total, q, n);
+  if (rc != PGPU_OK) return rc;
+  return pgpu_index_refine_chains_finish(ctx, out_exons, out_steps, out, nullptr);
+}
diff --git a/pintron_amd/csrc/pgpu_index.h b/pintron_amd/csrc/pgpu_index.h
--- a/pintron_amd/csrc/pgpu_index.h
+++ b/pintron_amd/csrc/pgpu_index.h
@@ -33,6 +33,10 @@
 void pgpu_ctx_pool_set_owner(pgpu_ctx* ctx, int pool, const void* who);
 const void* pgpu_ctx_pool_owner(const pgpu_ctx* ctx, int pool);
 bool pgpu_ctx_timing(const pgpu_ctx* ctx);
+hipError_t pgpu_ctx_wait_event(pgpu_ctx* ctx, hipEvent_t ev);
+float pgpu_ctx_t0_ms(pgpu_ctx* ctx, hipEvent_t ev);
+void** pgpu_ctx_chain_slot(pgpu_ctx* ctx);
+void pgpu_chain_state_release(void* state);
 
 size_t pgpu_scan_tmp_bytes(size_t n);
 void pgpu_exclusive_scan_u32(const uint32_t* in, unsigned long long* out, size_t n, void* tmp, hipStream_t st);
diff --git a/pintron_amd/host/ef_config.c b/pintron_amd/host/ef_config.c
--- a/pintron_amd/host/ef_config.c
+++ b/pintron_amd/host/ef_config.c
@@ -135,6 +135,11 @@
 }
 
 int ef_ahead_on = 1;
+int ef_refine_chains_on = 0;
+unsigned long long ef_chain_counts[6];
+void ef_refine_chain_counters(unsigned long long out[6]) {
+  for (int k = 0; k < 6; ++k) out[k] = __atomic_load_n(&ef_chain_counts[k], __ATOMIC_RELAXED);
+}
 int ef_chain_fast_path = 1;
 int ef_endpoint_checks = 1;
 int ef_prof_on;
@@ -146,6 +151,7 @@
   { const char* e = getenv("PINTRON_ENDPOINT_CHECKS"); ef_endpoint_checks = !(e && e[0] == '0'); }
   { const char* e = getenv("PINTRON_CHAIN"); ef_chain_fast_path = !(e && e[0] == '0' && e[1] == '\0'); }
   { const char* e = getenv("PINTRON_AHEAD"); ef_ahead_on = !(e && e[0] == '0' && e[1] == '\0'); }
+  { const char* e = getenv("PINTRON_REFINE_CHAINS"); if (e && e[0]) ef_refine_chains_on = !(e[0] == '0' && e[1] == '\0'); }
   { const char* e = getenv("PINTRON_PROFILE"); ef_prof_on = e && e[0] && !(e[0] == '0' && e[1] == '\0'); }
   { const char* e = getenv("PINTRON_WORK_BUDGET"); ef_work_budget_override = e && atoll(e) > 0 ? (unsigned long long)atoll(e) : 0ull; }
   bool given[32] = { false };
diff --git a/pintron_amd/host/ef_fact.c b/pintron_amd/host/ef_fact.c
--- a/pintron_amd/host/ef_fact.c
+++ b/pintron_amd/host/ef_fact.c
@@ -888,6 +888,91 @@
   return true;
 }
 
+static bool refine_introns_chained(ef_list* flist, const ef_config* cfg, const ef_seq* gen_info, const ef_seq* est_info,
+                                   ef_backend* be) {
+  if (!be->refine_chains || !ef_refine_chains_on) return false;
+  size_t n_chains = 0, n_exons = 0, n_introns = 0;
+  {
+    ef_iter it = efl_begin(flist);
+    while (efi_has_next(&it)) {
+      const size_t k = efl_size((ef_list*)efi_next(&it));
+      if (k) { ++n_chains; n_exons += k; n_introns += k - 1; }
+    }
+  }
+  if (n_introns == 0) return false;
+  const int sp[3] = { cfg->suffpref_length_on_est, cfg->suffpref_length_for_intron, cfg->suffpref_length_on_gen };
+  for (int k = 0; k < 3; ++k) if (sp[k] < 0 || sp[k] > (1 << 24)) return false;
+  const size_t est_len = strlen(est_info->seq), gen_len = strlen(gen_info->seq);
+  if (est_len > 0x7fffffffu) return false;
+  enum { SMALL_EXONS = 64, SMALL_CHAINS = 8 };
+  ef_factor ex_small[SMALL_EXONS]; ef_chain ch_small[SMALL_CHAINS];
+  ef_factor* ex = n_exons <= SMALL_EXONS ? ex_small : (ef_factor*)malloc(n_exons * sizeof(ef_factor));
+  ef_chain* ch = n_chains <= SMALL_CHAINS ? ch_small : (ef_chain*)malloc(n_chains * sizeof(ef_chain));
+  bool ok = true;
+  {
+    size_t e = 0, c = 0;
+    ef_iter it = efl_begin(flist);
+    while (efi_has_next(&it) && ok) {
+      ef_list* f = (ef_list*)efi_next(&it);
+      if (efl_empty(f)) continue;
+      ch[c].first_exon = (uint32_t)e; ch[c].n_exons = (uint32_t)efl_size(f); ch[c].refused = 0; ch[c].done = 0; ch[c].dropped_first = 0;
+      ++c;
+      const size_t first = e;
+      ef_iter fi = efl_begin(f);
+      while (efi_has_next(&fi)) {
+        const ef_factor* x = (const ef_factor*)efi_next(&fi);
+        const long long v[4] = { x->EST_start, x->EST_end, x->GEN_start, x->GEN_end };
+        if (v[0] < -1 || v[0] > (long long)est_len || v[1] < -1 || v[1] > (long long)est_len ||
+            v[2] < -1 || v[2] > (long long)gen_len || v[3] < -1 || v[3] > (long long)gen_len) ok = false;
+        if (e > first && !(ex[e - 1].EST_end < x->EST_start && ex[e - 1].GEN_end < x->GEN_start)) ok = false;
+        ex[e++] = *x;
+      }
+    }
+  }
+  if (ok && be->refine_chains(be->self, est_info->seq, est_len, ex, n_exons, ch, n_chains, cfg) != 0) {
+    fprintf(stderr, "* FATAL intron refinement backend failed\n"); abort();
+  }
+  if (ok) {
+    size_t c = 0;
+    ef_iter it = efl_begin(flist);
+    while (efi_has_next(&it)) {
+      ef_list* f = (ef_list*)efi_next(&it);
+      if (efl_empty(f)) continue;
+      const ef_chain* q = &ch[c++];
+      size_t e = q->first_exon;
+      ef_iter fi = efl_begin(f);
+      while (efi_has_next(&fi)) *(ef_factor*)efi_next(&fi) = ex[e++];
+      bool drop = q->dropped_first != 0;
+      if (q->refused) {
+        fi = efl_begin(f);
+        ef_factor* donor = (ef_factor*)efi_next(&fi);
+        for (uint32_t k = 0; k < q->done; ++k) donor = (ef_factor*)efi_next(&fi);
+        bool first = q->done == 0;
+        while (efi_has_next(&fi)) {
+          ef_factor* acc = (ef_factor*)efi_next(&fi);
+          ef_refine_intron(cfg, gen_info, est_info, donor, acc, first, be, NULL);
+          first = false;
+          donor = acc;
+        }
+        fi = efl_begin(f);
+        const ef_factor* e1 = (const ef_factor*)efi_next(&fi);
+        drop = false;
+        if (efi_has_next(&fi)) { const ef_factor* e2 = (const ef_factor*)efi_next(&fi); drop = e1->EST_start == e2->EST_start; }
+      }
+      if (drop) free(efl_pop_front(f));
+    }
+  }
+  {
+    unsigned long long add[6] = { 0, 0, 0, 0, 0, n_introns };
+    if (!ok) add[4] = 1;
+    else for (size_t c = 0; c < n_chains; ++c) { ++add[0]; add[1] += ch[c].done; add[2] += ch[c].refused != 0; add[3] += !ch[c].refused && ch[c].dropped_first; }
+    for (int k = 0; k < 6; ++k) if (add[k]) __atomic_fetch_add(&ef_chain_counts[k], add[k], __ATOMIC_RELAXED);
+  }
+  if (ex != ex_small) free(ex);
+  if (ch != ch_small) free(ch);
+  return ok;
+}
+
 ef_est* ef_get_est_factorizations(const ef_seq* est_info, ef_meg* V, const ef_config* cfg,
                                   const ef_seq* gen_info, ef_backend* be) {
   ef_phase(EFP_EMBED);
@@ -1020,7 +1105,7 @@
     flist = efl_new();
   }
   ef_phase(EFP_INTRON);
-  {
+  if (!refine_introns_chained(flist, cfg, gen_info, est_info, be)) {
     enum { GAP_AHEAD_MAX = 24 };
     ef_gap_ahead* pre = NULL; size_t n_pre = 0;
     if (be->ahead && be->dp_many) {
diff --git a/pintron_amd/host/ef_sched.c b/pintron_amd/host/ef_sched.c
--- a/pintron_amd/host/ef_sched.c
+++ b/pintron_amd/host/ef_sched.c
@@ -77,6 +77,10 @@
 
 enum { F_RUNNABLE, F_WAIT_DP, F_WAIT_PAIR, F_DONE };
 
+extern __typeof__(pgpu_index_refine_chains_launch) pgpu_index_refine_chains_launch __attribute__((weak));
+extern __typeof__(pgpu_index_refine_chains_finish) pgpu_index_refine_chains_finish __attribute__((weak));
+static inline bool chains_linked(void) { return pgpu_index_refine_chains_launch && pgpu_index_refine_chains_finish; }
+
 #if EF_TSAN
 static inline void tsan_to(void* fiber) { __tsan_switch_to_fiber(fiber, 0); }
 #else
@@ -100,6 +104,7 @@
   int phase;
   const ef_dp_req* reqs; ef_dp_res* ress; size_t nreq;
   ef_dp_req req1; int rc;
+  const char* ch_est; size_t ch_est_len; ef_factor* ch_exons; size_t ch_n_exons; ef_chain* chains; size_t n_chains; const ef_config* ch_cfg;
   const char* pat; size_t pat_len; unsigned pat_L; double pat_rate; ef_triple** pat_out; size_t* pat_n;
   ef_backend be;
   struct fiber* pool_next;
@@ -137,12 +142,15 @@
 
 typedef struct merged_batch {
   pgpu_dp_result* results; char* strings;
+  pgpu_factor* ch_exons; pgpu_chain_result* ch_res;
   int refs;
 } merged_batch;
 
 typedef struct dp_request {
   const pgpu_dp_job* jobs; size_t n; const char* arena; size_t arena_len;
+  const pgpu_chain_query* cq; size_t n_cq; const pgpu_factor* cex; size_t n_cex; const char* cests; size_t cests_len;
   merged_batch* batch; size_t base;
+  size_t cq_base, cex_base;
   int rc;
   uint32_t done;
   uint32_t* wake;
@@ -167,6 +175,7 @@
   pgpu_ctx* ctx;
   ef_sched_stats stats;
   double* iv; size_t n_iv, cap_iv;
+  pgpu_chain_query* m_cq; size_t m_cq_cap; pgpu_factor* m_cex; size_t m_cex_cap; char* m_cests; size_t m_cests_cap;
   double phase_s[6];
 } service_thread;
 
@@ -221,6 +230,7 @@
 typedef struct lane {
   fiber** fibers; size_t n_fibers;
   ef_jobbuf jb;
+  pgpu_chain_query* cq; size_t n_cq, cq_cap; pgpu_factor* cex; size_t n_cex, cex_cap; char* cests; size_t cests_len, cests_cap;
   dp_request rq; bool posted;
   fiber** inflight; size_t n_inflight;
 } lane;
@@ -257,6 +267,20 @@
   f->reqs = reqs; f->ress = res; f->nreq = n; f->state = F_WAIT_DP;
   ++f->w->suspensions;
   if (ef_prof_on) { ef_prof.susp[f->phase]++; ef_prof.jobs[f->phase] += n; }
+  if (EF_TSAN) tsan_to(f->w->tsan_sched);
+  ctx_switch(&f->ctx, &f->w->sched);
+  return f->rc;
+}
+
+static int fiber_refine_chains(void* self, const char* est, size_t est_len, ef_factor* exons, size_t n_exons,
+                               ef_chain* chains, size_t n_chains, const ef_config* cfg) {
+  fiber* f = (fiber*)self;
+  if (n_chains == 0) return 0;
+  f->ch_est = est; f->ch_est_len = est_len; f->ch_exons = exons; f->ch_n_exons = n_exons; f->chains = chains; f->n_chains = n_chains;
+  f->ch_cfg = cfg;
+  f->nreq = 0; f->state = F_WAIT_DP;
+  ++f->w->suspensions;
+  if (ef_prof_on) ef_prof.susp[f->phase]++;
   if (EF_TSAN) tsan_to(f->w->tsan_sched);
   ctx_switch(&f->ctx, &f->w->sched);
   return f->rc;
@@ -418,6 +442,7 @@
   else { f = (fiber*)calloc(1, sizeof(fiber)); f->stack = stack_alloc(sh->stack_size, &f->guarded); }
   f->w = w; f->unit = u; f->state = F_RUNNABLE; f->lane = li;
   f->be.self = f; f->be.pairings = fiber_pairings; f->be.dp = fiber_dp; f->be.dp_many = fiber_dp_many; f->be.meg = fiber_meg;
+  f->be.refine_chains = chains_linked() ? fiber_refine_chains : NULL;
   memcpy(f->stack, FIBER_SENTINEL, sizeof FIBER_SENTINEL);
 #if EF_TSAN
   if (f->tsan) __tsan_destroy_fiber(f->tsan);
@@ -504,8 +529,8 @@
     const bool stop = sv->stop;
     pthread_mutex_unlock(&sv->mu);
     if (!list) { if (stop) break; else continue; }
-    size_t nj = 0; int nreq = 0;
-    for (dp_request* r = list; r; r = r->next) ++nreq;
+    size_t nj = 0, n_cq = 0, n_cex = 0, n_cests = 0; int nreq = 0;
+    for (dp_request* r = list; r; r = r->next) { ++nreq; n_cq += r->n_cq; n_cex += r->n_cex; n_cests += r->cests_len; }
     if ((size_t)nreq > parts_cap) { parts_cap = (size_t)nreq * 2; parts = (pgpu_dp_part*)realloc(parts, parts_cap * sizeof(pgpu_dp_part)); }
     {
       size_t q = 0;
@@ -519,22 +544,60 @@
     mb->refs = nreq;
     mb->results = (pgpu_dp_result*)malloc((nj + 1) * sizeof(pgpu_dp_result));
     pgpu_dp_plan* plan = NULL;
+    int rc = PGPU_OK;
+    bool chains_up = false;
+    if (n_cq) {
+      if (n_cq > me->m_cq_cap) { me->m_cq_cap = n_cq * 2; me->m_cq = (pgpu_chain_query*)realloc(me->m_cq, me->m_cq_cap * sizeof(pgpu_chain_query)); }
+      if (n_cex > me->m_cex_cap) { me->m_cex_cap = n_cex * 2; me->m_cex = (pgpu_factor*)realloc(me->m_cex, me->m_cex_cap * sizeof(pgpu_factor)); }
+      if (n_cests > me->m_cests_cap) { me->m_cests_cap = n_cests * 2; me->m_cests = (char*)realloc(me->m_cests, me->m_cests_cap); }
+      size_t qb = 0, eb = 0, sb = 0;
+      for (dp_request* r = list; r; r = r->next) {
+        r->cq_base = qb; r->cex_base = eb;
+        for (size_t k = 0; k < r->n_cq; ++k) {
+          pgpu_chain_query x = r->cq[k];
+          x.est_off += sb; x.first_exon += (uint32_t)eb;
+          me->m_cq[qb + k] = x;
+        }
+        if (r->n_cex) memcpy(me->m_cex + eb, r->cex, r->n_cex * sizeof(pgpu_factor));
+        if (r->cests_len) memcpy(me->m_cests + sb, r->cests, r->cests_len);
+        qb += r->n_cq; eb += r->n_cex; sb += r->cests_len;
+      }
+      mb->ch_exons = (pgpu_factor*)malloc((n_cex + 1) * sizeof(pgpu_factor) + n_cex);
+      mb->ch_res = (pgpu_chain_result*)malloc((n_cq + 1) * sizeof(pgpu_chain_result));
+      rc = pgpu_index_refine_chains_launch(me->ctx, sh->idx, me->m_cests, n_cests, me->m_cex, n_cex, me->m_cq, n_cq);
+      chains_up = rc == PGPU_OK;
+    }
     const double t_a = now_s();
     me->phase_s[1] += t_a - t_idle - 0;
     pgpu_range_push("dp batch (create, launch, sync, fetch)");
-    int rc = pgpu_dp_plan_create_parts(me->ctx, sh->idx, parts, (size_t)nreq, &plan);
+    if (rc == PGPU_OK && nj) rc = pgpu_dp_plan_create_parts(me->ctx, sh->idx, parts, (size_t)nreq, &plan);
     const double t_b = now_s();
-    if (rc == PGPU_OK) rc = pgpu_dp_plan_launch(me->ctx, plan);
+    if (rc == PGPU_OK && plan) rc = pgpu_dp_plan_launch(me->ctx, plan);
     const double t_c = now_s();
-    if (rc == PGPU_OK) rc = pgpu_dp_plan_sync(me->ctx, plan);
+    if (rc == PGPU_OK && plan) rc = pgpu_dp_plan_sync(me->ctx, plan);
+    if (chains_up) {
+      pgpu_group_info gi;
+      const int crc = pgpu_index_refine_chains_finish(me->ctx, mb->ch_exons, (uint8_t*)(mb->ch_exons + n_cex + 1), mb->ch_res, &gi);
+      if (rc == PGPU_OK) rc = crc;
+      if (crc == PGPU_OK && sh->kernel_timing && gi.ms > 0) {
+        ef_kernel_stat ks; memset(&ks, 0, sizeof ks);
+        snprintf(ks.name, sizeof ks.name, "%s", gi.name);
+        ks.ms = gi.ms; ks.launches = 1; ks.jobs = gi.jobs;
+        kstat_add(&me->stats, &ks);
+        if (gi.t0_ms >= 0) {
+          if (me->n_iv + 2 > me->cap_iv) { me->cap_iv = me->cap_iv ? me->cap_iv * 2 : 4096; me->iv = (double*)realloc(me->iv, me->cap_iv * sizeof(double)); }
+          me->iv[me->n_iv++] = gi.t0_ms; me->iv[me->n_iv++] = gi.t0_ms + gi.ms;
+        }
+      }
+    }
     const double t_d = now_s();
     me->phase_s[2] += t_b - t_a; me->phase_s[3] += t_c - t_b; me->phase_s[4] += t_d - t_c;
-    if (rc == PGPU_OK) {
+    if (rc == PGPU_OK && plan) {
       const size_t sb = pgpu_dp_plan_string_bytes(plan);
       mb->strings = (char*)malloc(sb + 16);
       rc = pgpu_dp_plan_fetch(me->ctx, plan, mb->results, mb->strings, sb + 16);
     }
-    if (rc == PGPU_OK && sh->kernel_timing) {
+    if (rc == PGPU_OK && plan && sh->kernel_timing) {
       const int ng = pgpu_dp_plan_n_groups(plan);
       for (int g = 0; g < ng; ++g) {
         pgpu_group_info gi;
@@ -557,7 +620,27 @@
     for (dp_request* r = list; r;) { dp_request* nx = r->next; r->batch = mb; r->rc = rc; request_publish(r); r = nx; }
   }
   free(parts);
+  free(me->m_cq); free(me->m_cex); free(me->m_cests);
+  me->m_cq = NULL; me->m_cex = NULL; me->m_cests = NULL; me->m_cq_cap = me->m_cex_cap = me->m_cests_cap = 0;
   return NULL;
+}
+
+static void lane_add_chains(lane* ln, const fiber* f) {
+  if (ln->n_cq + f->n_chains > ln->cq_cap) { ln->cq_cap = (ln->n_cq + f->n_chains) * 2 + 64; ln->cq = (pgpu_chain_query*)realloc(ln->cq, ln->cq_cap * sizeof(pgpu_chain_query)); }
+  if (ln->n_cex + f->ch_n_exons > ln->cex_cap) { ln->cex_cap = (ln->n_cex + f->ch_n_exons) * 2 + 256; ln->cex = (pgpu_factor*)realloc(ln->cex, ln->cex_cap * sizeof(pgpu_factor)); }
+  if (ln->cests_len + f->ch_est_len > ln->cests_cap) { ln->cests_cap = (ln->cests_len + f->ch_est_len) * 2 + 4096; ln->cests = (char*)realloc(ln->cests, ln->cests_cap); }
+  const ef_config* cfg = f->ch_cfg;
+  for (size_t k = 0; k < f->n_chains; ++k) {
+    pgpu_chain_query* q = &ln->cq[ln->n_cq + k];
+    q->est_off = ln->cests_len; q->est_len = (uint32_t)f->ch_est_len;
+    q->first_exon = (uint32_t)(ln->n_cex + f->chains[k].first_exon); q->n_exons = f->chains[k].n_exons; q->reserved = 0;
+    q->suffpref_length_on_est = cfg->suffpref_length_on_est; q->suffpref_length_for_intron = cfg->suffpref_length_for_intron;
+    q->suffpref_length_on_gen = cfg->suffpref_length_on_gen; q->min_intron_length = cfg->min_intron_length;
+  }
+  _Static_assert(sizeof(ef_factor) == sizeof(pgpu_factor), "a factor goes to the device as it is");
+  memcpy(ln->cex + ln->n_cex, f->ch_exons, f->ch_n_exons * sizeof(pgpu_factor));
+  memcpy(ln->cests + ln->cests_len, f->ch_est, f->ch_est_len);
+  ln->n_cq += f->n_chains; ln->n_cex += f->ch_n_exons; ln->cests_len += f->ch_est_len;
 }
 
 static int launch_dp(worker* w, lane* ln) {
@@ -566,10 +649,12 @@
   const char* gen = sh->in->gen->seq;
   ef_jobbuf_reset(&ln->jb);
   ln->n_inflight = 0;
+  ln->n_cq = ln->n_cex = ln->cests_len = 0;
   for (size_t i = 0; i < ln->n_fibers; ++i) {
     fiber* f = ln->fibers[i];
     if (f->state != F_WAIT_DP) continue;
     for (size_t k = 0; k < f->nreq; ++k) ef_jobbuf_add(&ln->jb, &f->reqs[k], gen, sh->gen_len);
+    if (f->n_chains) lane_add_chains(ln, f);
     ln->inflight[ln->n_inflight++] = f;
   }
   if (ln->n_inflight == 0) return 0;
@@ -577,6 +662,7 @@
   memset(rq, 0, sizeof *rq);
   rq->wake = &w->wake;
   rq->jobs = ln->jb.jobs; rq->n = ln->jb.n; rq->arena = ln->jb.arena; rq->arena_len = ln->jb.arena_len;
+  rq->cq = ln->cq; rq->n_cq = ln->n_cq; rq->cex = ln->cex; rq->n_cex = ln->n_cex; rq->cests = ln->cests; rq->cests_len = ln->cests_len;
   pthread_mutex_lock(&sv->mu);
   if (sv->tail) sv->tail->next = rq; else sv->head = rq;
   sv->tail = rq;
@@ -600,10 +686,19 @@
   const int rc = rq->rc;
   const bool tracing = ef_dp_trace_enabled() != 0;
   if (rc == PGPU_OK) {
-    size_t j = rq->base;
+    size_t j = rq->base, cq = rq->cq_base, ce = rq->cex_base;
     for (size_t i = 0; i < ln->n_inflight; ++i) {
       fiber* f = ln->inflight[i];
       f->rc = 0;
+      if (f->n_chains) {
+        memcpy(f->ch_exons, rq->batch->ch_exons + ce, f->ch_n_exons * sizeof(pgpu_factor));
+        for (size_t k = 0; k < f->n_chains; ++k) {
+          const pgpu_chain_result* r = &rq->batch->ch_res[cq + k];
+          f->chains[k].refused = r->status != PGPU_OK; f->chains[k].done = r->done; f->chains[k].dropped_first = r->dropped_first;
+        }
+        cq += f->n_chains; ce += f->ch_n_exons;
+        f->n_chains = 0;
+      }
       for (size_t k = 0; k < f->nreq; ++k, ++j) {
         const int drc = ef_decode_result(f->reqs[k].kind, &rq->batch->results[j], rq->batch->strings, &f->ress[k]);
         if (drc != 0) {
@@ -616,7 +711,7 @@
     }
   }
   const bool last = __atomic_sub_fetch(&rq->batch->refs, 1, __ATOMIC_ACQ_REL) == 0;
-  if (last) { free(rq->batch->results); free(rq->batch->strings); free(rq->batch); }
+  if (last) { free(rq->batch->results); free(rq->batch->strings); free(rq->batch->ch_exons); free(rq->batch->ch_res); free(rq->batch); }
   ln->n_inflight = 0;
   return rc;
 }
@@ -730,6 +825,7 @@
     lane* ln = &w->lanes[li];
     collect_dp(w, ln);
     ef_jobbuf_free(&ln->jb);
+    free(ln->cq); free(ln->cex); free(ln->cests);
     free(ln->fibers); free(ln->inflight);
   }
   if (w->ctx) pgpu_destroy(w->ctx);
@@ -1717,6 +1813,10 @@
   else if (!getenv("PINTRON_NO_PAGE_RELEASE")) session_release_pages(s);
   ef_log_reference_timers(st.index_s, st.prefetch_s, st.workers_s, st.load_s + (m3.wall - m2.wall), now_s() - m0.wall);
   if (getenv("PINTRON_VERBOSE")) {
+    unsigned long long cc[EF_CHAIN_COUNTERS];
+    ef_refine_chain_counters(cc);
+    fprintf(stderr, "* refine chains: sent %llu, introns settled on the device %llu of %llu, refused mid-way %llu, first exons dropped %llu, "
+                    "ESTs on the host path after the pre-check %llu\n", cc[0], cc[1], cc[5], cc[2], cc[3], cc[4]);
     fprintf(stderr, "* run: open %.3fs step %.3fs write %.3fs close %.3fs\n", m1.wall - m0.wall, m2.wall - m1.wall, m3.wall - m2.wall, now_s() - m3.wall);
     fprintf(stderr, "* cpu (all threads): open user %.2fs sys %.2fs, %ld page faults; step user %.2fs sys %.2fs, %ld page faults; write user %.2fs sys %.2fs\n",
             m1.user - m0.user, m1.sys - m0.sys, m1.minflt - m0.minflt, m2.user - m1.user, m2.sys - m1.sys, m2.minflt - m1.minflt,
diff --git a/pintron_amd/host/ef_sched.h b/pintron_amd/host/ef_sched.h
--- a/pintron_amd/host/ef_sched.h
+++ b/pintron_amd/host/ef_sched.h
@@ -20,6 +20,9 @@
   double suspensions_per_unit;
 } ef_sched_stats;
 
+#define EF_CHAIN_COUNTERS 6
+void ef_refine_chain_counters(unsigned long long out[EF_CHAIN_COUNTERS]);
+
 typedef struct ef_session ef_session;
 ef_session* ef_session_open(int argc, char** argv);
 int ef_session_step(ef_session* s, ef_sched_stats* stats);
diff --git a/pintron_amd/host/estfact.h b/pintron_amd/host/estfact.h
--- a/pintron_amd/host/estfact.h
+++ b/pintron_amd/host/estfact.h
@@ -246,6 +246,9 @@
 } ef_ahead;
 static inline void ef_ahead_init(ef_ahead* ah) { ah->n = ah->n_pending = 0; ah->collecting = false; memset(ah->slot, 0, sizeof ah->slot); }
 
+typedef struct { uint32_t first_exon, n_exons; int refused; uint32_t done, dropped_first; } ef_chain;
+struct ef_factor_s;
+
 typedef struct ef_backend {
   void* self;
   int (*pairings)(void* self, const char* pattern, size_t m, unsigned min_factor_len, double rate,
@@ -254,6 +257,8 @@
   int (*dp_many)(void* self, const ef_dp_req* reqs, ef_dp_res* res, size_t n);
   const void* (*meg)(void* self, const char* pattern, size_t m, const ef_config* cfg);
   ef_ahead* ahead;
+  int (*refine_chains)(void* self, const char* est, size_t est_len, struct ef_factor_s* exons, size_t n_exons,
+                       ef_chain* chains, size_t n_chains, const ef_config* cfg);
 } ef_backend;
 
 static inline bool ef_req_same(const ef_dp_req* x, const ef_dp_req* y) {
@@ -303,8 +308,10 @@
 static inline bool ef_collecting(const ef_backend* be) { return be->ahead && be->ahead->collecting; }
 int ef_ahead_flush(ef_backend* be);
 extern int ef_ahead_on;
-
-typedef struct { int EST_start, EST_end, GEN_start, GEN_end; } ef_factor;
+extern unsigned long long ef_chain_counts[6];
+extern int ef_refine_chains_on;
+
+typedef struct ef_factor_s { int EST_start, EST_end, GEN_start, GEN_end; } ef_factor;
 
 typedef struct {
   const ef_seq* info;
```

Result: slower. 832,900 (-7.9%).
